# zhouzypaul/fql

Hardware: NVIDIA B200
Metric: fql_update_samples_per_sec (higher is better)
Workload: dtype bf16

## Files before the change

fql_b200/_lib.py:

```python
from __future__ import annotations

import ctypes as C
import os

_HERE = os.path.dirname(os.path.abspath(__file__))
LIB_PATH = os.path.join(_HERE, 'libfql_b200.so')

NUM_INFO = 13
NUM_RAW = 16
NET_NAMES = ('actor_bc_flow', 'actor_onestep_flow', 'critic', 'target_critic')
NET_ACTOR_BC_FLOW, NET_ACTOR_ONESTEP_FLOW, NET_CRITIC, NET_TARGET_CRITIC = 0, 1, 2, 3
LEAF_KINDS = ('kernel', 'bias', 'scale', 'bias', 'kernel', 'bias', 'kernel', 'bias')
PRECISION_FP32, PRECISION_BF16_TC, PRECISION_BF16_ENC = 0, 1, 2


class FqlDims(C.Structure):
    _fields_ = [(n, C.c_int32) for n in (
        'batch', 'global_batch', 'obs_dim', 'action_dim', 'hidden', 'num_hidden', 'critic_layer_norm', 'actor_layer_norm',
        'q_agg_min', 'normalize_q_loss', 'flow_steps', 'num_seeds', 'precision')] + [('reserved', C.c_int32 * 3)]


class FqlHparams(C.Structure):
    _fields_ = [(n, C.c_float) for n in ('lr', 'beta1', 'beta2', 'eps', 'discount', 'tau', 'alpha', 'one_minus_beta1',
                                         'one_minus_beta2', 'one_minus_tau')] + [('reserved', C.c_float * 2)]


class FqlLeaf(C.Structure):
    _fields_ = [('net', C.c_int32), ('layer', C.c_int32), ('kind', C.c_int32), ('ens', C.c_int32), ('rows', C.c_int32),
                ('cols', C.c_int32), ('offset', C.c_int64)]


class FqlBatch(C.Structure):
    _fields_ = [(n, C.c_void_p) for n in ('observations', 'actions', 'next_observations', 'rewards', 'masks', 'z_next', 'x0',
                                          't', 'z', 'z_metric')]


class FqlState(C.Structure):
    _fields_ = [(n, C.c_void_p) for n in ('params', 'mu', 'nu', 'grads', 'count', 'shadow')]


DP_MAX_RANKS = 8


class FqlDpComm(C.Structure):
    _fields_ = [('rank', C.c_int32), ('world', C.c_int32), ('base', C.c_void_p * DP_MAX_RANKS), ('base_mc', C.c_void_p)]


class FqlTestOperand(C.Structure):
    _fields_ = [('ptr', C.c_void_p), ('inner', C.c_int32), ('rows', C.c_int32), ('ld', C.c_int64), ('g0', C.c_int32), ('s0', C.c_int64),
                ('g1', C.c_int32), ('s1', C.c_int64)]


class FqlTestPtr(C.Structure):
    _fields_ = [('base', C.c_void_p), ('s0', C.c_int64), ('s1', C.c_int64), ('ld', C.c_int32)]


TEST_GEMM_PTRS = ('bias', 'out_f', 'out_h', 'out_z', 'zin', 'act', 'xb', 'target', 'ln_s', 'ln_b', 'dbias', 'wmaster', 'dln_s', 'dln_b')


class FqlTestGemm(C.Structure):
    _fields_ = ([(n, C.c_int32) for n in ('mode', 'M', 'N', 'K', 'G0', 'G1', 'a_mn', 'b_mn', 'ksplit')] +
                [('A', FqlTestOperand), ('B', FqlTestOperand)] + [(n, FqlTestPtr) for n in TEST_GEMM_PTRS] +
                [(n, C.c_int32) for n in ('F', 'Adim', 'step', 'n_steps', 'clip')])


TC_MODE_STORE_F32, TC_MODE_FWD_HIDDEN, TC_MODE_DGRAD_GELU, TC_MODE_EULER, TC_MODE_WGRAD_LN = 0, 1, 2, 3, 4


class FqlError(RuntimeError):
    pass


_lib = None

_SIGS = {
    'fql_version': (C.c_int, []),
    'fql_last_error': (C.c_char_p, []),
    'fql_info_name': (C.c_char_p, [C.c_int]),
    'fql_context_create': (C.c_int, [C.POINTER(C.c_void_p)]),
    'fql_context_destroy': (C.c_int, [C.c_void_p]),
    'fql_launch_count': (C.c_longlong, [C.c_void_p]),
    'fql_arena_floats': (C.c_int64, [C.POINTER(FqlDims)]),
    'fql_layout': (C.c_int, [C.POINTER(FqlDims), C.POINTER(FqlLeaf), C.c_int32, C.POINTER(C.c_int32)]),
    'fql_workspace_bytes': (C.c_size_t, [C.POINTER(FqlDims)]),
    'fql_shadow_bytes': (C.c_size_t, [C.POINTER(FqlDims)]),
    'fql_forward_workspace_bytes': (C.c_size_t, [C.POINTER(FqlDims), C.c_int32]),
    'fql_update_step': (C.c_int, [C.c_void_p, C.POINTER(FqlDims), C.POINTER(FqlHparams), C.POINTER(FqlBatch), C.POINTER(FqlState),
                                  C.c_void_p, C.c_void_p, C.c_size_t, C.c_void_p]),
    'fql_step_grads': (C.c_int, [C.c_void_p, C.POINTER(FqlDims), C.POINTER(FqlHparams), C.POINTER(FqlBatch), C.POINTER(FqlState),
                                 C.c_void_p, C.c_void_p, C.c_size_t, C.c_void_p]),
    'fql_step_apply': (C.c_int, [C.c_void_p, C.POINTER(FqlDims), C.POINTER(FqlHparams), C.POINTER(FqlState), C.c_void_p,
                                 C.c_void_p, C.c_void_p, C.c_size_t, C.c_void_p]),
    'fql_step_apply_gathered': (C.c_int, [C.c_void_p, C.POINTER(FqlDims), C.POINTER(FqlHparams), C.POINTER(FqlState), C.c_void_p, C.c_int32,
                                          C.c_void_p, C.c_void_p, C.c_size_t, C.c_void_p]),
    'fql_dp_symmetric_bytes': (C.c_size_t, [C.POINTER(FqlDims), C.c_int32]),
    'fql_dp_attach': (C.c_int, [C.c_void_p, C.POINTER(FqlDims), C.POINTER(FqlDpComm)]),
    'fql_dp_allreduce': (C.c_int, [C.c_void_p, C.c_int32, C.c_int64, C.c_int64, C.c_void_p]),
    'fql_conv3x3_workspace_bytes': (C.c_size_t, []),
    'fql_conv3x3_bf16': (C.c_int, [C.c_void_p, C.c_void_p, C.c_void_p, C.c_int32, C.c_int32, C.c_int32, C.c_int32, C.c_int32, C.c_int32,
                                   C.c_void_p, C.c_void_p, C.c_int32, C.c_void_p, C.c_void_p, C.c_size_t, C.c_void_p]),
    'fql_conv3x3_wgrad_bf16': (C.c_int, [C.c_void_p, C.c_void_p, C.c_int32, C.c_int32, C.c_int32, C.c_int32, C.c_int32, C.c_void_p,
                                         C.c_void_p, C.c_void_p, C.c_size_t, C.c_void_p]),
    'fql_test_tc_gemm': (C.c_int, [C.POINTER(FqlTestGemm), C.c_void_p]),
    'fql_test_act_ln_bf16': (C.c_int, [C.c_void_p, C.c_void_p, C.c_void_p, C.c_int64, C.c_int64, C.c_void_p, C.c_void_p, C.c_void_p,
                                       C.c_int32, C.c_int32, C.c_int32, C.c_int32, C.c_int32, C.c_void_p]),
    'fql_test_ln_bwd_bf16': (C.c_int, [C.c_void_p, C.c_void_p, C.c_void_p, C.c_int64, C.c_int64, C.c_void_p, C.c_void_p, C.c_int32,
                                       C.c_int32, C.c_int32, C.c_int32, C.c_int64, C.c_int64, C.c_void_p]),
    'fql_test_gelu_bwd_bf16': (C.c_int, [C.c_void_p, C.c_void_p, C.c_void_p, C.c_void_p, C.c_int32, C.c_int32, C.c_int32, C.c_int32,
                                         C.c_int64, C.c_int64, C.c_void_p]),
    'fql_test_colsum_bf16': (C.c_int, [C.c_void_p, C.c_int64, C.c_int64, C.c_int32, C.c_void_p, C.c_int64, C.c_int32, C.c_int64,
                                       C.c_void_p]),
    'fql_set_early_grads_event':(C.c_int, [C.c_void_p, C.c_void_p]),
    'fql_early_grads_floats': (C.c_int64, [C.POINTER(FqlDims)]),
    'fql_total_loss': (C.c_int, [C.c_void_p, C.POINTER(FqlDims), C.POINTER(FqlHparams), C.POINTER(FqlBatch), C.POINTER(FqlState),
                                 C.c_void_p, C.c_void_p, C.c_size_t, C.c_void_p]),
    'fql_sample_actions': (C.c_int, [C.c_void_p, C.POINTER(FqlDims), C.c_void_p, C.c_void_p, C.c_void_p, C.c_void_p, C.c_void_p,
                                     C.c_int32, C.c_void_p, C.c_size_t, C.c_void_p]),
    'fql_compute_flow_actions': (C.c_int, [C.c_void_p, C.POINTER(FqlDims), C.c_void_p, C.c_void_p, C.c_void_p, C.c_void_p,
                                           C.c_void_p, C.c_int32, C.c_void_p, C.c_size_t, C.c_void_p]),
    'fql_mlp_forward': (C.c_int, [C.c_void_p, C.POINTER(FqlDims), C.c_int32, C.c_void_p, C.c_void_p, C.c_void_p, C.c_int32,
                                  C.c_void_p, C.c_size_t, C.c_void_p]),
    'fql_target_update': (C.c_int, [C.POINTER(FqlDims), C.POINTER(FqlHparams), C.c_void_p, C.c_void_p, C.c_void_p]),
    'fql_debug_stamps': (C.c_int, [C.c_void_p, C.c_void_p, C.c_int]),
    'fql_refresh_shadow': (C.c_int, [C.POINTER(FqlDims), C.c_void_p, C.c_void_p, C.c_void_p]),
    'fql_gather_rows': (C.c_int, [C.c_void_p, C.c_void_p, C.c_void_p, C.c_int64, C.c_int64, C.c_void_p]),
    'fql_gather_frames': (C.c_int, [C.c_void_p, C.c_void_p, C.c_void_p, C.c_void_p, C.c_void_p, C.c_void_p, C.c_void_p, C.c_int64,
                                    C.c_int32, C.c_int32, C.c_int32, C.c_int32, C.c_int32, C.c_void_p]),
    'fql_fill_noise': (C.c_int, [C.POINTER(FqlDims), C.c_uint64, C.c_uint64, C.c_void_p, C.c_void_p, C.c_void_p, C.c_void_p,
                                 C.c_void_p, C.c_void_p]),
    'fql_fill_noise_rows': (C.c_int, [C.POINTER(FqlDims), C.c_uint64, C.c_uint64, C.c_int64, C.c_void_p, C.c_void_p, C.c_void_p,
                                      C.c_void_p, C.c_void_p, C.c_void_p]),
}
EXPORTS = tuple(_SIGS)


def lib():
    global _lib
    if _lib is None:
        if not os.path.exists(LIB_PATH):
            raise FqlError(f'{LIB_PATH} is missing: build it with `python -c "import __graft_entry__ as g; g.build()"` '
                           f'or `make -C fql_b200/csrc`. fql_b200 has no CPU or PyTorch fallback.')
        l = C.CDLL(LIB_PATH)
        for name, (res, args) in _SIGS.items():
            fn = getattr(l, name)
            fn.restype, fn.argtypes = res, args
        _lib = l
    return _lib


def check(rc, what=''):
    if rc != 0:
        raise FqlError(f'{what}: {lib().fql_last_error().decode()}')


def make_dims(batch, obs_dim, action_dim, *, global_batch=None, hidden=512, num_hidden=4, critic_layer_norm=True,
              actor_layer_norm=False, q_agg='mean', normalize_q_loss=False, flow_steps=10, num_seeds=1, precision=PRECISION_FP32,
              image=None):
    d = FqlDims()
    d.batch, d.global_batch = int(batch), int(global_batch if global_batch is not None else batch)
    d.obs_dim, d.action_dim, d.hidden, d.num_hidden = int(obs_dim), int(action_dim), int(hidden), int(num_hidden)
    d.critic_layer_norm, d.actor_layer_norm = int(bool(critic_layer_norm)), int(bool(actor_layer_norm))
    d.q_agg_min, d.normalize_q_loss = int(q_agg == 'min'), int(bool(normalize_q_loss))
    d.flow_steps, d.num_seeds, d.precision = int(flow_steps), int(num_seeds), int(precision)
    if image is not None:
        d.reserved[0], d.reserved[1], d.reserved[2] = int(image[0]), int(image[1]), int(image[2])
    return d


def make_hparams(lr=3e-4, discount=0.99, tau=0.005, alpha=300.0, beta1=0.9, beta2=0.999, eps=1e-8):
    h = FqlHparams()
    h.lr, h.beta1, h.beta2, h.eps, h.discount, h.tau, h.alpha = lr, beta1, beta2, eps, discount, tau, alpha
    h.one_minus_beta1, h.one_minus_beta2, h.one_minus_tau = 1.0 - beta1, 1.0 - beta2, 1.0 - tau
    return h


def layout(dims):
    l = lib()
    n = C.c_int32(0)
    check(l.fql_layout(C.byref(dims), None, 0, C.byref(n)), 'fql_layout')
    arr = (FqlLeaf * n.value)()
    check(l.fql_layout(C.byref(dims), arr, n.value, C.byref(n)), 'fql_layout')
    out = []
    for lf in arr:
        if lf.kind < 4:
            path = (('LayerNorm' if lf.kind >= 2 else 'Dense') + f'_{lf.layer}',)
        elif lf.kind < 6:
            path = ('encoder', f'stack_blocks_{lf.layer // 3}', f'Conv_{lf.layer % 3}')
        else:
            path = ('encoder', 'MLP_0', 'Dense_0')
        shape = None
        if lf.kind == 4:
            shape = (3, 3, lf.rows // 9, lf.cols)
        out.append(dict(net=NET_NAMES[lf.net], module=path[-1], path=path, name=LEAF_KINDS[lf.kind], ens=lf.ens, rows=lf.rows, cols=lf.cols,
                        offset=lf.offset, is_kernel=lf.kind in (0, 4, 6), shape=shape, kind=lf.kind))
    return out, int(l.fql_arena_floats(C.byref(dims)))
```

fql_b200/csrc/euler_cluster.cu:

```cuda
#include "step.cuh"
#include "tc_prims.cuh"

using namespace tc;

namespace {

constexpr int TILE_M = 128;
constexpr int KB = 64;
constexpr int A_BLK = TILE_M * 128;
constexpr int SUB = 32;
constexpr int A_SUB = TILE_M * SUB * 2;
constexpr int NSUB = 16;
constexpr int MAX_A = 32;
constexpr int NMMA = 4;
#ifndef FQL_EULER_NISS
#define FQL_EULER_NISS 2
#endif
constexpr int NISS = FQL_EULER_NISS;
static_assert(NISS == 1 || NISS == 2 || NISS == 4, "NISS");
constexpr int NEPI = 4;
constexpr int NTHREADS = 32 * (1 + NMMA + NEPI);
constexpr int EPI0 = 32 * (1 + NMMA);

struct EulerArgs {
  int H, K0, K0pad, A, F, n_steps, NL;
  int S, M, tiles;
  int x_rows_s;
  int x_row0;
  int w_row[FQL_MAXL];
  int w_rows_s;
  int wl_row, wl_rows_s;
  const float* params;
  long long arena;
  long long off_b[FQL_MAXL];
  const float* c0;
  const float* a0;
  float* target;
  __nv_bfloat16* hx;
  long long hx_buf_elems;
  float* state;
  __nv_bfloat16* Hsave[FQL_MAXL];
  __nv_bfloat16* Zsave[FQL_MAXL];
  float* out;
  int rows_cap, r0;
  float* Fsave[FQL_MAXL];
  int z_rows_cap, z_r0;
  unsigned long long* dbg;
  unsigned long long* t_start;
  int dbg_it;
};

struct HMaps {
  CUtensorMap m[4];
};
constexpr int MODE_EULER = 0, MODE_FWD = 1, MODE_DGRAD = 2;

__device__ __forceinline__ unsigned long long gtime() {
  unsigned long long t;
  asm volatile("mov.u64 %0, %globaltimer;" : "=l"(t));
  return t;
}

__device__ __forceinline__ float gelu_fast(float x) {
  const float u = FQL_GELU_C * (x + FQL_GELU_A * x * x * x);
  return 0.5f * x * (1.0f + tanh_approx(u));
}
__device__ __forceinline__ float gelu_grad_fast(float x) {
  const float x2 = x * x;
  const float u = FQL_GELU_C * (x + FQL_GELU_A * x2 * x);
  const float th = tanh_approx(u);
  const float du = FQL_GELU_C * (1.0f + 3.0f * FQL_GELU_A * x2);
  return 0.5f * (1.0f + th) + 0.5f * x * (1.0f - th * th) * du;
}
__device__ __forceinline__ uint32_t pack2(float a, float b) {
  __nv_bfloat162 v = __floats2bfloat162_rn(a, b);
  return *reinterpret_cast<uint32_t*>(&v);
}

template <int NC, int AMAX, int MODE>
__global__ void __launch_bounds__(NTHREADS, 1) euler_cluster_kernel(const __grid_constant__ CUtensorMap mapX,
                                                               const __grid_constant__ CUtensorMap mapW,
                                                               const __grid_constant__ CUtensorMap mapWL,
                                                               const __grid_constant__ HMaps mapsH, const EulerArgs a) {
  constexpr int NCOL = 512 / NC;
  constexpr int HALVES = NCOL / SUB;
  constexpr int B_ROWB = NCOL * 2;
  constexpr int B_BLK = KB * B_ROWB;
  constexpr int ACC_SET = NMMA * NCOL;
  constexpr uint16_t MASK = (uint16_t)((1u << NC) - 1u);
  extern __shared__ uint8_t smem_raw[];
  uint8_t* smem = reinterpret_cast<uint8_t*>((reinterpret_cast<uintptr_t>(smem_raw) + 1023) & ~(uintptr_t)1023);
  const int nkb = a.H / KB, nkb_x = a.K0pad / KB;
  uint8_t* sA = smem;
  uint8_t* sB = sA + NSUB * A_SUB;
  uint8_t* sX = sB + nkb * B_BLK;
  float* sBias = reinterpret_cast<float*>(sX + nkb_x * A_BLK);
  float* sT = sBias + a.NL * 64;
  uint64_t* bars = reinterpret_cast<uint64_t*>(sT + 64);
  uint64_t* full_a = bars;
  uint64_t* full_b = bars + 16;
  uint64_t* acc_full = bars + 17;
  uint64_t* free_a = bars + 18;
  uint64_t* a_ready = bars + 19;
  uint64_t* x_full = bars + 20;
  uint64_t* half_ready = bars + 21;
  uint32_t* tmem_slot = reinterpret_cast<uint32_t*>(bars + 24);

  const int warp = __shfl_sync(0xffffffffu, (int)(threadIdx.x >> 5), 0), lane = threadIdx.x & 31;
  const uint32_t j = __shfl_sync(0xffffffffu, cluster_ctarank(), 0);
  const int cl = blockIdx.x / NC;
  const int tile = cl % a.tiles, s = cl / a.tiles;
  const int NL = a.NL;
  const int total = a.n_steps * NL;
  const int hx_row = (s * a.tiles + tile) * TILE_M;
  unsigned long long* dbg = a.dbg ? a.dbg + blockIdx.x * 16 : nullptr;
  const int DBG_IT = a.dbg_it;

  if (warp == 0 && lane == 0) {
    tma_prefetch_desc(&mapX);
    tma_prefetch_desc(&mapW);
    tma_prefetch_desc(&mapWL);
    for (int i = 0; i < (MODE == MODE_EULER ? 1 : NL - 1); i++) tma_prefetch_desc(&mapsH.m[i]);
    for (int i = 0; i < NSUB; i++) mbar_init(&full_a[i], 1);
    mbar_init(&half_ready[0], NEPI);
    mbar_init(&half_ready[1], NEPI);
    mbar_init(full_b, 1);
    mbar_init(acc_full, NISS);
    mbar_init(free_a, NC * NISS);
    mbar_init(a_ready, NEPI);
    mbar_init(x_full, 1);
    fence_barrier_init();
  }
  if (warp == 1) tmem_alloc(tmem_slot, 2 * ACC_SET);
  for (int i = threadIdx.x; i < (MODE == MODE_DGRAD ? 0 : NL * 64); i += NTHREADS) {
    const int l = i >> 6, c = i & 63;
    const bool lastl = (l == NL - 1);
    const int N = lastl ? a.A : a.H;
    const int col = lastl ? c : (int)j * NCOL + c;
    sBias[i] = (c < NCOL && col < N && !(l == 0 && a.c0)) ? a.params[(int64_t)s * a.arena + a.off_b[l] + col] : 0.f;
  }
  if (threadIdx.x <= a.n_steps) sT[threadIdx.x] = (float)((double)threadIdx.x / (double)a.n_steps);
  tc_fence_before();
  __syncthreads();
  tc_fence_after();
  cluster_sync_all();
  const uint32_t tmem_base = *tmem_slot;
  if (a.t_start && blockIdx.x == 0 && threadIdx.x == 0) a.t_start[0] = gtime();

  if (warp == 0) {
    const bool el = elect_one();
    {
      if (el) mbar_expect_tx(x_full, nkb_x * A_BLK);
      const int xrow = s * a.x_rows_s + a.x_row0 + tile * TILE_M;
      for (int kb = 0; kb < nkb_x; kb++)
        if (el) tma_load_2d(sX + kb * A_BLK, &mapX, x_full, kb * KB, xrow);
      int n_pub = 0;
      int l = 0;
      for (int it = 0; it < total; it++, l = (l + 1 == NL) ? 0 : l + 1) {
        const bool last = (l == NL - 1);
        const int K = (l == 0) ? a.K0 : a.H;
        const int kblocks = (K + KB - 1) / KB;
        if (it > 0) mbar_wait_u(acc_full, (it - 1) & 1);
        if (el) mbar_expect_tx(full_b, kblocks * B_BLK);
        for (int kb = 0; kb < kblocks; kb++) {
          if (!el) continue;
          if constexpr (MODE == MODE_DGRAD) {
            if (l == 0) tma_load_2d(sB, &mapWL, full_b, 0, a.wl_row + s * a.wl_rows_s + (int)j * NCOL);
            else tma_load_2d(sB + kb * B_BLK, &mapW, full_b, kb * KB, a.w_row[l] + s * a.w_rows_s + (int)j * NCOL);
          } else {
            if (!last) tma_load_2d(sB + kb * B_BLK, &mapW, full_b, (int)j * NCOL, a.w_row[l] + s * a.w_rows_s + kb * KB);
            else tma_load_2d(sB + kb * B_BLK, &mapWL, full_b, 0, a.wl_row + s * a.wl_rows_s + kb * KB);
          }
        }
        if (l >= 1) {
          for (int sbk = 0; sbk < NSUB; sbk++)
            if (el) mbar_expect_tx(&full_a[sbk], A_SUB);
          const int buf = n_pub & 1;
          for (int h = 0; h < HALVES; h++) {
            mbar_wait_u(&half_ready[h], n_pub & 1);
            asm volatile("fence.proxy.async.global;" ::: "memory");
            if (h == 0) mbar_wait_cluster_u(free_a, (it - 1) & 1);
            if (dbg && el && it == DBG_IT) dbg[3 + h] = gtime();
            const int sbk = (int)j * HALVES + h;
            if (el)
              asm volatile(
                  "cp.async.bulk.tensor.2d.shared::cluster.global.mbarrier::complete_tx::bytes.multicast::cluster [%0], [%1, {%3, %4}], [%2], %5;"
                  ::"r"(smem_u32(sA + sbk * A_SUB)), "l"(reinterpret_cast<uint64_t>(MODE != MODE_EULER ? &mapsH.m[l - 1] : &mapsH.m[0])),
                  "r"(smem_u32(&full_a[sbk])), "r"(sbk * SUB),
                  "r"(MODE != MODE_EULER ? s * a.rows_cap + a.r0 + tile * TILE_M : buf * (a.S * a.tiles * TILE_M) + hx_row), "h"(MASK)
                  : "memory");
          }
          n_pub++;
        }
      }
    }
  } else if (warp <= NMMA) {
    const bool el = elect_one();
    if (warp <= NISS) {
      const int mw = warp - 1;
      const uint32_t tmem_u = __shfl_sync(0xffffffffu, tmem_base, 0);
      const uint32_t idesc = make_idesc_bf16(TILE_M, NCOL, false, MODE != MODE_DGRAD);
      const uint64_t ax_t = make_smem_desc(0, 16, 1024);
      const uint64_t a64_t0 = make_smem_desc_sw64(0, 16, 512);
      const uint64_t b_t0 = (MODE == MODE_DGRAD) ? make_smem_desc(0, 16, 1024)
                                                 : ((NC == 8) ? make_smem_desc(0, B_BLK, 1024) : make_smem_desc_sw64(0, B_BLK, 512));
      constexpr uint64_t B_KSTEP = (MODE == MODE_DGRAD) ? 2 : ((16 * B_ROWB) >> 4);
      constexpr uint64_t B_SUBH = (MODE == MODE_DGRAD) ? 4 : ((32 * B_ROWB) >> 4);
      const uint32_t sa0 = smem_u32(sA) >> 4, sx0 = smem_u32(sX) >> 4, sb0 = smem_u32(sB) >> 4;
      int n_a = 0;
      int n_step = 0;
      int l = 0;
      for (int it = 0; it < total; it++, l = (l + 1 == NL) ? 0 : l + 1) {
        const int K = (l == 0) ? a.K0 : a.H;
        const int kblocks = (K + KB - 1) / KB;
        const uint32_t tacc = tmem_u + (it & 1) * ACC_SET + mw * NCOL;
        if (l == 0) {
          if (it == 0) mbar_wait_u(x_full, 0);
          else { mbar_wait_u(a_ready, (n_step - 1) & 1); }
          n_step++;
          if (dbg && el && mw == 0 && it == DBG_IT) dbg[8] = gtime();
        }
        mbar_wait_u(full_b, it & 1);
        tc_fence_after();
        if (dbg && el && mw == 0 && it == DBG_IT && l == 0) dbg[9] = gtime();
        if (l >= 1) {
          constexpr int PER = NSUB / NISS;
          for (int i = 0; i < PER; i++) {
            const int sbk = (NC == 8) ? (mw * (PER / 2) + (i % (PER / 2))) * 2 + (i / (PER / 2)) : mw * PER + i;
            mbar_wait_u(&full_a[sbk], n_a & 1);
            tc_fence_after();
            if (dbg && el && mw == 0 && it == DBG_IT && i == 0) dbg[5] = gtime();
            if (dbg && el && mw == NISS - 1 && it == DBG_IT && i == PER - 1) dbg[6] = gtime();
            if (el)
              umma_bf16_x2(tacc, a64_t0 + (uint64_t)(sa0 + sbk * (A_SUB >> 4)),
                           b_t0 + (uint64_t)(sb0 + (sbk >> 1) * (B_BLK >> 4) + (sbk & 1) * B_SUBH), 2, B_KSTEP, idesc, i != 0);
          }
        } else {
          for (int kb = 0; kb < kblocks; kb++)
            for (int ks = mw; ks < 4; ks += NISS)
              if (el && ks < (a.K0 - kb * KB + 15) / 16)
                umma_bf16(tacc, ax_t + (uint64_t)(sx0 + kb * (A_BLK >> 4) + ks * 2), b_t0 + (uint64_t)(sb0 + kb * (B_BLK >> 4) + ks * B_KSTEP), idesc,
                          !(kb == 0 && ks == mw));
        }
        if (l >= 1) n_a++;
        if (dbg && el && mw == 0 && it == DBG_IT && l == 0) dbg[10] = gtime();
        if (el) {
          umma_commit(acc_full);
          asm volatile("tcgen05.commit.cta_group::1.mbarrier::arrive::one.shared::cluster.multicast::cluster.b64 [%0], %1;" ::"r"(smem_u32(free_a)),
                       "h"(MASK)
                       : "memory");
        }
      }
    }
  } else {
    const int q = warp & 3;
    const int row = q * 32 + lane;
    const int grow = tile * TILE_M + row;
    const bool valid = grow < a.M;
    const uint32_t t_lane0 = tmem_base + ((uint32_t)(q * 32) << 16);
    const int et = threadIdx.x - EPI0;
    float* st_row = a.state + (int64_t)blockIdx.x * MAX_A * TILE_M + row;
    int n_exch = 0;
    int l = 0, step = 0;
    for (int it = 0; it < total; it++, l = (l + 1 == NL) ? 0 : l + 1, step += (l == 0)) {
      const bool last = (l == NL - 1);
      const float* sb = sBias + l * 64;
      uint4 zq[4];
      if constexpr (MODE == MODE_DGRAD) {
        static_assert(MODE != MODE_DGRAD || HALVES == 1, "the dgrad chain is built for clusters of 16");
        if (valid) {
          const uint4* zp = reinterpret_cast<const uint4*>(a.Zsave[l] + ((int64_t)s * a.z_rows_cap + a.z_r0 + grow) * a.H + j * NCOL);
#pragma unroll
          for (int c = 0; c < 4; c++) zq[c] = __ldg(zp + c);
        }
      }
      float ac[AMAX];
      if (MODE == MODE_EULER && last) {
#pragma unroll
        for (int c = 0; c < AMAX; c++)
          if (c < a.A) ac[c] = (step == 0) ? (valid ? __ldg(a.a0 + ((int64_t)s * a.M + grow) * a.A + c) : 0.f) : __ldcg(st_row + c * TILE_M);
      }
      mbar_wait(acc_full, it & 1);
      tc_fence_after();
      if (dbg && et == 0 && it == DBG_IT - 1) dbg[0] = gtime();
      if (dbg && et == 0 && it == DBG_IT) dbg[7] = gtime();
      const int live = (l == 0 && (a.K0 + 15) / 16 < NISS) ? (a.K0 + 15) / 16 : NISS;
      const int buf = n_exch & 1;
      if (!last) n_exch++;
#pragma unroll 1
      for (int half = 0; half < HALVES; half++) {
        const uint32_t t_lane = t_lane0 + (it & 1) * ACC_SET + half * 32;
        uint32_t r0[32];
        if (!last || half == 0) {
          uint32_t t1[32];
          tmem_ld32(t_lane, r0);
          if (live > 1) tmem_ld32(t_lane + NCOL, t1);
          tmem_wait_ld();
          if (live > 1) {
#pragma unroll
            for (int i = 0; i < 32; i++) r0[i] = __float_as_uint(__uint_as_float(r0[i]) + __uint_as_float(t1[i]));
          }
          if (live > 2) {
            uint32_t t2[32];
            tmem_ld32(t_lane + 2 * NCOL, t1);
            if (live > 3) tmem_ld32(t_lane + 3 * NCOL, t2);
            tmem_wait_ld();
#pragma unroll
            for (int i = 0; i < 32; i++) {
              float v = __uint_as_float(r0[i]) + __uint_as_float(t1[i]);
              if (live > 3) v += __uint_as_float(t2[i]);
              r0[i] = __float_as_uint(v);
            }
          }
        }
        if constexpr (MODE == MODE_DGRAD) {
          if (valid) {
            const int64_t e0 = ((int64_t)s * a.rows_cap + a.r0 + grow) * a.H + j * NCOL;
            uint4* dh = reinterpret_cast<uint4*>(a.Hsave[l] + e0);
            float4* df = reinterpret_cast<float4*>(a.Fsave[l] + e0);
#pragma unroll
            for (int c = 0; c < 4; c++) {
              const uint32_t zw[4] = {zq[c].x, zq[c].y, zq[c].z, zq[c].w};
              float dv[8];
#pragma unroll
              for (int i = 0; i < 4; i++) {
                const __nv_bfloat162 zb = *reinterpret_cast<const __nv_bfloat162*>(&zw[i]);
                dv[2 * i] = __uint_as_float(r0[c * 8 + 2 * i]) * gelu_grad_fast(__low2float(zb));
                dv[2 * i + 1] = __uint_as_float(r0[c * 8 + 2 * i + 1]) * gelu_grad_fast(__high2float(zb));
              }
              dh[c] = make_uint4(pack2(dv[0], dv[1]), pack2(dv[2], dv[3]), pack2(dv[4], dv[5]), pack2(dv[6], dv[7]));
              df[2 * c] = make_float4(dv[0], dv[1], dv[2], dv[3]);
              df[2 * c + 1] = make_float4(dv[4], dv[5], dv[6], dv[7]);
            }
          }
          if (!last) {
            __syncwarp();
            if (lane == 0) mbar_arrive(&half_ready[half]);
          }
        } else if (!last) {
          if constexpr (MODE == MODE_EULER) {
            uint4* dst = reinterpret_cast<uint4*>(a.hx + (int64_t)buf * a.hx_buf_elems + (int64_t)(hx_row + row) * a.H + j * NCOL + half * 32);
            if (l == 0 && a.c0) {
              const float4* cp = reinterpret_cast<const float4*>(a.c0 + ((int64_t)s * a.M + (valid ? grow : 0)) * a.H + j * NCOL + half * 32);
#pragma unroll
              for (int c = 0; c < 8; c++) {
                const float4 cv = __ldg(cp + c);
                r0[c * 4 + 0] = __float_as_uint(__uint_as_float(r0[c * 4 + 0]) + cv.x);
                r0[c * 4 + 1] = __float_as_uint(__uint_as_float(r0[c * 4 + 1]) + cv.y);
                r0[c * 4 + 2] = __float_as_uint(__uint_as_float(r0[c * 4 + 2]) + cv.z);
                r0[c * 4 + 3] = __float_as_uint(__uint_as_float(r0[c * 4 + 3]) + cv.w);
              }
            }
#pragma unroll
            for (int c = 0; c < 4; c++) {
              float h[8];
#pragma unroll
              for (int i = 0; i < 8; i++) h[i] = gelu_fast(__uint_as_float(r0[c * 8 + i]) + sb[half * 32 + c * 8 + i]);
              dst[c] = make_uint4(pack2(h[0], h[1]), pack2(h[2], h[3]), pack2(h[4], h[5]), pack2(h[6], h[7]));
            }
          } else if (valid) {
            const int64_t e0 = ((int64_t)s * a.rows_cap + a.r0 + grow) * a.H + j * NCOL + half * 32;
            uint4* dh = reinterpret_cast<uint4*>(a.Hsave[l] + e0);
            uint4* dz = reinterpret_cast<uint4*>(a.Zsave[l] + e0);
#pragma unroll
            for (int c = 0; c < 4; c++) {
              float z[8], h[8];
#pragma unroll
              for (int i = 0; i < 8; i++) {
                z[i] = __uint_as_float(r0[c * 8 + i]) + sb[half * 32 + c * 8 + i];
                h[i] = gelu_fast(z[i]);
              }
              dh[c] = make_uint4(pack2(h[0], h[1]), pack2(h[2], h[3]), pack2(h[4], h[5]), pack2(h[6], h[7]));
              dz[c] = make_uint4(pack2(z[0], z[1]), pack2(z[2], z[3]), pack2(z[4], z[5]), pack2(z[6], z[7]));
            }
          }
          __syncwarp();
          if (lane == 0) mbar_arrive(&half_ready[half]);
          if (dbg && et == 0 && it == DBG_IT - 1) dbg[1 + half] = gtime();
        } else if (MODE == MODE_FWD) {
          if (half == 0 && j == 0 && valid) {
            float* o = a.out + ((int64_t)s * a.rows_cap + a.r0 + grow) * a.A;
#pragma unroll
            for (int c = 0; c < AMAX; c++)
              if (c < a.A) o[c] = __uint_as_float(r0[c]) + sb[c];
          }
        } else if (half == 0) {
          if (dbg && et == 0 && it == DBG_IT - 1) dbg[13] = gtime();
          const float inv = (float)a.n_steps;
          const bool final_step = (step == a.n_steps - 1);
#pragma unroll
          for (int c = 0; c < AMAX; c++)
            if (c < a.A) {
              ac[c] += (__uint_as_float(r0[c]) + sb[c]) / inv;
              const int col = a.F + c;
              *reinterpret_cast<__nv_bfloat16*>(sX + (col >> 6) * A_BLK + sw128_off(row, (col & 63) >> 3) + (col & 7) * 2) = __float2bfloat16(ac[c]);
            }
          {
            const int col = a.F + a.A;
            *reinterpret_cast<__nv_bfloat16*>(sX + (col >> 6) * A_BLK + sw128_off(row, (col & 63) >> 3) + (col & 7) * 2) =
                __float2bfloat16(sT[step + 1]);
          }
          if (dbg && et == 0 && it == DBG_IT - 1) dbg[11] = gtime();
          fence_proxy_async_smem();
          tc_fence_before();
          __syncwarp();
          if (lane == 0) mbar_arrive(a_ready);
          if (dbg && et == 0 && it == DBG_IT - 1) dbg[12] = gtime();
#pragma unroll
          for (int c = 0; c < AMAX; c++)
            if (c < a.A) {
              if (!final_step) __stcg(st_row + c * TILE_M, ac[c]);
              else if (valid && j == 0) a.target[((int64_t)s * a.M + grow) * a.A + c] = fminf(fmaxf(ac[c], -1.0f), 1.0f);
            }
        }
      }
      if (!last) tc_fence_before();
    }
  }
  tc_fence_before();
  __syncthreads();
  cluster_sync_all();
  if (a.t_start && blockIdx.x == 0 && threadIdx.x == 0) a.t_start[1] = gtime();
  if (warp == 1) tmem_dealloc(tmem_base, 2 * ACC_SET);
}

}

size_t tc_euler_scratch_elems(const FqlDims* d, int M) {
  const int tiles = (M + TILE_M - 1) / TILE_M;
  return (size_t)2 * d->num_seeds * tiles * TILE_M * d->hidden + (size_t)2 * d->num_seeds * tiles * 16 * MAX_A * TILE_M;
}

namespace {
template <int NC, int AMAX, int MODE>
int launch_euler(const EulerArgs& a, const TcEulerSpec& f, cudaStream_t st, bool query_only, int* max_clusters) {
  constexpr int NCOL = 512 / NC;
  const FqlDims* d = f.d;
  const int smem = NSUB * A_SUB + (a.H / KB) * (KB * NCOL * 2) + (a.K0pad / KB) * A_BLK + a.NL * 64 * 4 + 64 * 4 + 256 + 1024;
  FQL_REQUIRE(smem <= 232448, "euler_cluster_kernel: shared memory %d > 227 KB", smem);
  auto kern = euler_cluster_kernel<NC, AMAX, MODE>;
  static bool attr_set[FQL_MAX_DEVICES] = {};
  const int dev = fql_current_device();
  if (!attr_set[dev]) {
    FQL_CHECK_CUDA(cudaFuncSetAttribute(kern, cudaFuncAttributeMaxDynamicSharedMemorySize, 232448));
    if (NC > 8) FQL_CHECK_CUDA(cudaFuncSetAttribute(kern, cudaFuncAttributeNonPortableClusterSizeAllowed, 1));
    attr_set[dev] = true;
  }
  cudaLaunchConfig_t cfg;
  memset(&cfg, 0, sizeof(cfg));
  cfg.gridDim = dim3(NC * a.tiles * a.S);
  cfg.blockDim = dim3(NTHREADS);
  cfg.dynamicSmemBytes = smem;
  cfg.stream = st;
  cudaLaunchAttribute attr[1];
  attr[0].id = cudaLaunchAttributeClusterDimension;
  attr[0].val.clusterDim.x = NC;
  attr[0].val.clusterDim.y = 1;
  attr[0].val.clusterDim.z = 1;
  cfg.attrs = attr;
  cfg.numAttrs = 1;
  if (query_only) {
    cfg.stream = nullptr;
    if (cudaOccupancyMaxActiveClusters(max_clusters, kern, &cfg) != cudaSuccess) {
      cudaGetLastError();
      *max_clusters = 0;
    }
    return 0;
  }
  const CUtensorMapSwizzle wsw = (NC == 8 || MODE == MODE_DGRAD) ? CU_TENSOR_MAP_SWIZZLE_128B : CU_TENSOR_MAP_SWIZZLE_64B;
  CUtensorMap mapX, mapW, mapWL;
  HMaps mapsH;
  memset(&mapsH, 0, sizeof(mapsH));
  FQL_TRY(make_map_2d(&mapX, f.X0b, a.K0pad, (uint64_t)a.S * f.Mcap0, 64, TILE_M));
  if (MODE == MODE_DGRAD) {
    FQL_TRY(make_map_2d(&mapW, f.shadow, d->hidden, (uint64_t)a.S * a.w_rows_s, 64, NCOL, wsw));
    FQL_TRY(make_map_2d(&mapWL, f.shadow, 64, (uint64_t)a.S * a.wl_rows_s, 64, NCOL, wsw));
  } else {
    FQL_TRY(make_map_2d(&mapW, f.shadow, d->hidden, (uint64_t)a.S * a.w_rows_s, NCOL, KB, wsw));
    FQL_TRY(make_map_2d(&mapWL, f.shadow, 64, (uint64_t)a.S * a.wl_rows_s, NCOL, KB, wsw));
  }
  if (MODE == MODE_EULER) {
    FQL_TRY(make_map_2d(&mapsH.m[0], f.scratch, d->hidden, (uint64_t)2 * a.S * a.tiles * TILE_M, SUB, TILE_M, CU_TENSOR_MAP_SWIZZLE_64B));
  } else {
    for (int l = 0; l + 1 < a.NL; l++)
      FQL_TRY(make_map_2d(&mapsH.m[l], a.Hsave[l], d->hidden, (uint64_t)a.S * a.rows_cap, SUB, TILE_M, CU_TENSOR_MAP_SWIZZLE_64B));
  }
  FQL_CHECK_CUDA(cudaLaunchKernelEx(&cfg, kern, mapX, mapW, mapWL, mapsH, a));
  FQL_CHECK_LAUNCH();
  return 0;
}
}

namespace {
int fill_args(EulerArgs& a, const FqlDims* d, const Layout& L, int net, const float* params, int M, int Mcap0, int r0_in, bool hoisted = false) {
  FQL_TRY(tc_supported(d, !hoisted));
  FQL_REQUIRE(d->hidden == 512, "euler_cluster_kernel is built for hidden = 512 (16 exchange units of 32 columns)");
  const NetView& nv = L.net[net];
  memset(&a, 0, sizeof(a));
  a.H = d->hidden; a.K0 = nv.in_dim; a.K0pad = (int)round_up64(nv.in_dim, 64); a.A = nv.out_dim; a.F = d->obs_dim;
  a.n_steps = 1; a.NL = nv.n_layers;
  a.S = d->num_seeds; a.M = M; a.tiles = (M + TILE_M - 1) / TILE_M;
  a.x_rows_s = Mcap0; a.x_row0 = r0_in;
  const int64_t seed_elems = tc_shadow_seed_elems(d, L);
  a.w_rows_s = (int)(seed_elems / d->hidden);
  a.wl_rows_s = (int)(seed_elems / 64);
  for (int l = 0; l < nv.n_layers; l++) {
    a.w_row[l] = (int)(nv.off_w[l] / d->hidden);
    a.off_b[l] = nv.off_b[l];
  }
  int64_t wl = L.arena;
  for (int t = 0; t < net; t++) wl += (int64_t)L.net[t].ens * d->hidden * 64;
  a.wl_row = (int)(wl / 64);
  a.params = params; a.arena = L.arena;
  FQL_REQUIRE(a.A <= MAX_A, "euler_cluster_kernel: output width %d > %d", a.A, MAX_A);
  a.dbg_it = 7;
  return 0;
}
int max_clusters16(const EulerArgs& a, const TcEulerSpec& f) {
  static int max16_dev[FQL_MAX_DEVICES];
  static bool known[FQL_MAX_DEVICES] = {};
  const int dev = fql_current_device();
  int& max16 = max16_dev[dev];
  if (!known[dev]) {
    const char* e = getenv("FQL_B200_EULER_NC");
    if (e && atoi(e) == 8) max16 = 0;
    else if (launch_euler<16, 8, MODE_EULER>(a, f, nullptr, true, &max16)) max16 = 0;
    if (getenv("FQL_B200_VERBOSE")) fprintf(stderr, "fql_b200: clusters of 16 CTAs resident at once (device %d): %d\n", dev, max16);
    known[dev] = true;
  }
  return max16;
}
}

int tc_euler_cluster(const TcEulerSpec& f, cudaStream_t st) {
  const FqlDims* d = f.d;
  EulerArgs a;
  FQL_TRY(fill_args(a, d, *f.L, FQL_NET_ACTOR_BC_FLOW, f.params, f.M, f.Mcap0, f.r0_in, f.c0 != nullptr));
  a.A = d->action_dim; a.n_steps = d->flow_steps;
  if (f.c0) {
    a.c0 = f.c0;
    a.K0 = d->action_dim + 1; a.K0pad = 64; a.F = 0;
    a.w_row[0] += d->obs_dim;
  }
  a.a0 = f.a0; a.target = f.target;
  a.hx = reinterpret_cast<__nv_bfloat16*>(f.scratch);
  a.hx_buf_elems = (long long)a.S * a.tiles * TILE_M * a.H;
  a.state = reinterpret_cast<float*>(a.hx + 2 * a.hx_buf_elems);
  a.dbg = reinterpret_cast<unsigned long long*>(f.dbg);
  a.t_start = reinterpret_cast<unsigned long long*>(f.t_start);
  FQL_REQUIRE(f.scratch != nullptr && f.a0 && f.target, "tc_euler_cluster: NULL argument");
  FQL_REQUIRE(a.n_steps < 64, "euler_cluster_kernel: flow_steps %d >= 64", a.n_steps);
  const bool c16 = a.tiles * a.S <= max_clusters16(a, f);
  if (a.A <= 8) return c16 ? launch_euler<16, 8, MODE_EULER>(a, f, st, false, nullptr) : launch_euler<8, 8, MODE_EULER>(a, f, st, false, nullptr);
  if (a.A <= 16) return c16 ? launch_euler<16, 16, MODE_EULER>(a, f, st, false, nullptr) : launch_euler<8, 16, MODE_EULER>(a, f, st, false, nullptr);
  return c16 ? launch_euler<16, 32, MODE_EULER>(a, f, st, false, nullptr) : launch_euler<8, 32, MODE_EULER>(a, f, st, false, nullptr);
}

int tc_cluster_forward(const TcClusterFwdSpec& f, int other_clusters, cudaStream_t st) {
  const FqlDims* d = f.d;
  const NetView& nv = f.L->net[f.net];
  if (d->hidden != 512 || nv.ln || nv.n_layers > 5 || nv.n_layers < 2 || nv.out_dim > MAX_A || nv.in_dim > 128) return 1;
  EulerArgs a;
  if (fill_args(a, d, *f.L, f.net, f.params, f.M, f.rows_cap, f.r0)) return -1;
  TcEulerSpec e;
  memset(&e, 0, sizeof(e));
  e.d = d; e.L = f.L; e.params = f.params; e.shadow = f.shadow; e.X0b = f.X0b; e.Mcap0 = f.rows_cap; e.r0_in = f.r0; e.M = f.M;
  if (a.tiles * a.S + other_clusters > max_clusters16(a, e)) return 1;
  for (int l = 0; l + 1 < nv.n_layers; l++) {
    a.Hsave[l] = reinterpret_cast<__nv_bfloat16*>(f.Hb[l]);
    a.Zsave[l] = reinterpret_cast<__nv_bfloat16*>(f.Zb[l]);
    if (!a.Hsave[l] || !a.Zsave[l]) return 1;
  }
  a.out = f.out; a.rows_cap = f.rows_cap; a.r0 = f.r0;
  a.t_start = reinterpret_cast<unsigned long long*>(f.t_start);
  if (a.A <= 8) return launch_euler<16, 8, MODE_FWD>(a, e, st, false, nullptr) ? -1 : 0;
  if (a.A <= 16) return launch_euler<16, 16, MODE_FWD>(a, e, st, false, nullptr) ? -1 : 0;
  return launch_euler<16, 32, MODE_FWD>(a, e, st, false, nullptr) ? -1 : 0;
}

int tc_cluster_dgrad(const TcClusterBwdSpec& f, int other_clusters, cudaStream_t st) {
  const FqlDims* d = f.d;
  const NetView& nv = f.L->net[f.net];
  if (d->hidden != 512 || nv.ln || nv.n_layers > 5 || nv.n_layers < 3 || nv.out_dim > 64) return 1;
  EulerArgs a;
  if (fill_args(a, d, *f.L, f.net, nullptr, f.M, f.M, 0)) return -1;
  const int NLn = nv.n_layers;
  a.NL = NLn - 1;
  a.K0 = 64; a.K0pad = 64;
  for (int it = 1; it < a.NL; it++) a.w_row[it] = (int)(nv.off_w[NLn - 1 - it] / d->hidden);
  TcEulerSpec e;
  memset(&e, 0, sizeof(e));
  e.d = d; e.L = f.L; e.shadow = f.shadow; e.X0b = f.dOutb; e.Mcap0 = f.M; e.r0_in = 0; e.M = f.M;
  if (a.tiles * a.S + other_clusters > max_clusters16(a, e)) return 1;
  for (int it = 0; it < a.NL; it++) {
    const int lo = NLn - 2 - it;
    a.Hsave[it] = reinterpret_cast<__nv_bfloat16*>(f.dZb[lo]);
    a.Fsave[it] = f.dZf[lo];
    a.Zsave[it] = reinterpret_cast<__nv_bfloat16*>(f.Zb[lo]);
    if (!a.Hsave[it] || !a.Fsave[it] || !a.Zsave[it]) return 1;
  }
  a.rows_cap = f.M; a.r0 = 0; a.z_rows_cap = f.z_rows_cap; a.z_r0 = f.z_r0;
  a.t_start = reinterpret_cast<unsigned long long*>(f.t_start);
  return launch_euler<16, 8, MODE_DGRAD>(a, e, st, false, nullptr) ? -1 : 0;
}
```

fql_b200/csrc/step.cu:

```cuda
#include "step.cuh"
#include "dp_comm.cuh"

#include <cuda_bf16.h>
#include <stdarg.h>

#include <vector>

static thread_local char g_err[1024] = "";
thread_local long long g_fql_launches = 0;
void fql_set_error(const char* fmt, ...) {
  va_list ap;
  va_start(ap, fmt);
  vsnprintf(g_err, sizeof(g_err), fmt, ap);
  va_end(ap);
}

int fql_validate_dims(const FqlDims* d) {
  FQL_REQUIRE(d != nullptr, "dims is NULL");
  FQL_REQUIRE(d->batch >= 1 && d->global_batch >= d->batch, "batch=%d global_batch=%d", d->batch, d->global_batch);
  FQL_REQUIRE(d->obs_dim >= 1 && d->action_dim >= 1, "obs_dim=%d action_dim=%d", d->obs_dim, d->action_dim);
  FQL_REQUIRE(d->hidden >= 1 && d->num_hidden >= 1 && d->num_hidden + 1 <= FQL_MAXL, "hidden=%d num_hidden=%d", d->hidden, d->num_hidden);
  FQL_REQUIRE(d->num_seeds >= 1, "num_seeds=%d", d->num_seeds);
  FQL_REQUIRE(d->flow_steps >= 1, "flow_steps=%d", d->flow_steps);
  FQL_REQUIRE(d->precision == FQL_PRECISION_FP32 || d->precision == FQL_PRECISION_BF16_TC || d->precision == FQL_PRECISION_BF16_ENC,
              "precision=%d", d->precision);
  FQL_REQUIRE(d->precision != FQL_PRECISION_BF16_ENC || d->reserved[0] > 0, "FQL_PRECISION_BF16_ENC is a pixel-config mode (encoder='impala_small')");
  if (d->reserved[0] > 0) {
    FQL_REQUIRE(d->reserved[1] > 0 && d->reserved[2] > 0 && d->reserved[2] <= 32, "image dims %dx%dx%d", d->reserved[0], d->reserved[1], d->reserved[2]);
    FQL_REQUIRE(d->obs_dim == 512, "pixel configs: obs_dim is the encoder output width and must be 512 (got %d)", d->obs_dim);
    FQL_REQUIRE(d->num_seeds == 1, "pixel configs are built for num_seeds == 1");
  }
  return 0;
}

int fql_build_layout(const FqlDims* d, Layout* L) {
  FQL_TRY(fql_validate_dims(d));
  memset(L, 0, sizeof(*L));
  const int F = d->obs_dim, A = d->action_dim, H = d->hidden, NL = d->num_hidden + 1;
  int64_t off = 0;
  int nl = 0;
  auto add_leaf = [&](int net, int64_t n) {
    int64_t o = off;
    L->leaf_blk[nl] = (int)(off / FQL_LEAF_PAD);
    L->leaf_net[nl] = net;
    nl++;
    off += round_up64(n, FQL_LEAF_PAD);
    return o;
  };
  static const int kOrder[FQL_NUM_NETS] = {FQL_NET_ACTOR_BC_FLOW, FQL_NET_CRITIC, FQL_NET_ACTOR_ONESTEP_FLOW, FQL_NET_TARGET_CRITIC};
  for (int oi = 0; oi < FQL_NUM_NETS; oi++) {
    const int n = kOrder[oi];
    NetView& v = L->net[n];
    v.n_layers = NL;
    v.hidden = H;
    const bool critic = (n == FQL_NET_CRITIC || n == FQL_NET_TARGET_CRITIC);
    v.ens = critic ? 2 : 1;
    v.ln = critic ? d->critic_layer_norm : d->actor_layer_norm;
    v.in_dim = (n == FQL_NET_ACTOR_BC_FLOW) ? F + A + 1 : F + A;
    v.out_dim = critic ? 1 : A;
    v.begin = off;
    const int extra = v.ln ? 4 : 2;
    FQL_REQUIRE(nl + NL * extra + 20 <= FQL_MAX_LEAVES, "too many leaves");
    for (int l = 0; l < NL; l++) {
      const int64_t K = v.k_of(l), N = v.n_of(l);
      v.off_w[l] = add_leaf(n, v.ens * K * N);
      v.off_b[l] = add_leaf(n, v.ens * N);
      if (v.ln && l + 1 < NL) {
        v.off_lns[l] = add_leaf(n, v.ens * N);
        v.off_lnb[l] = add_leaf(n, v.ens * N);
      }
    }
    if (d->reserved[0] > 0) {
      v.has_enc = 1;
      static const int stacks[3] = {16, 32, 32};
      int c = d->reserved[2], h = d->reserved[0], w = d->reserved[1];
      for (int i = 0; i < 3; i++) {
        const int f = stacks[i];
        const int cin[3] = {c, f, f};
        for (int j = 0; j < 3; j++) {
          v.enc.off_cw[i][j] = add_leaf(n, 9 * cin[j] * f);
          v.enc.off_cb[i][j] = add_leaf(n, f);
        }
        c = f; h = (h + 1) / 2; w = (w + 1) / 2;
      }
      v.enc.off_dw = add_leaf(n, (int64_t)h * w * c * d->obs_dim);
      v.enc.off_db = add_leaf(n, d->obs_dim);
    }
    v.end = off;
  }
  L->arena = off;
  L->n_leaves = nl;
  L->leaf_blk[nl] = (int)(off / FQL_LEAF_PAD);
  return 0;
}

StepShape make_shape(const FqlDims* d) {
  StepShape s;
  s.S = d->num_seeds; s.B = d->batch; s.GB = d->global_batch; s.F = d->obs_dim; s.A = d->action_dim;
  s.H = d->hidden; s.NH = d->num_hidden;
  s.q_agg_min = d->q_agg_min; s.normalize_q_loss = d->normalize_q_loss; s.flow_steps = d->flow_steps;
  return s;
}

namespace {
struct Carver {
  char* base;
  size_t off = 0;
  float* take(int64_t nfloats) {
    off = (off + 255) & ~(size_t)255;
    float* p = base ? reinterpret_cast<float*>(base + off) : nullptr;
    off += (size_t)nfloats * sizeof(float);
    return p;
  }
};

void carve_pass(Carver& c, PassBuf* pb, int G, int Mcap, int H, int NH, int out_dim, bool ln, bool need_z) {
  pb->G = G;
  pb->Mcap = Mcap;
  for (int l = 0; l < NH; l++) {
    pb->Z[l] = (need_z || ln) ? c.take((int64_t)G * Mcap * H) : nullptr;
    pb->Hh[l] = c.take((int64_t)G * Mcap * H);
    pb->mu[l] = ln ? c.take((int64_t)G * Mcap) : nullptr;
    pb->rstd[l] = ln ? c.take((int64_t)G * Mcap) : nullptr;
  }
  pb->out = c.take((int64_t)G * Mcap * out_dim);
}
}

size_t carve_workspace(const FqlDims* d, const Layout& L, void* base, WsPtrs* w) {
  Carver c{reinterpret_cast<char*>(base)};
  const int64_t S = d->num_seeds, B = d->batch, F = d->obs_dim, A = d->action_dim, H = d->hidden;
  const int NH = d->num_hidden;
  memset(w, 0, sizeof(*w));
  w->XO = c.take(S * 3 * B * (F + A));
  w->XF = c.take(S * 2 * B * (F + A + 1));
  w->XC = c.take(3 * S * B * (F + A));
  w->vel = c.take(S * B * A);
  carve_pass(c, &w->pO, (int)S, (int)(3 * B), (int)H, NH, (int)A, d->actor_layer_norm, true);
  carve_pass(c, &w->pF, (int)S, (int)(2 * B), (int)H, NH, (int)A, d->actor_layer_norm, true);
  carve_pass(c, &w->pC, (int)(3 * S * 2), (int)B, (int)H, NH, 1, d->critic_layer_norm, true);
  w->O_out = w->pO.out;
  w->F_out = w->pF.out;
  w->C_out = w->pC.out;
  w->dq = c.take(S * 2 * B);
  w->dqs = c.take(S * 2 * B);
  w->dpred = c.take(S * B * A);
  w->dapi = c.take(S * B * A);
  w->target = c.take(S * B * A);
  w->dX0 = c.take(S * 2 * B * (F + A));
  w->raw_local = c.take(S * FQL_NUM_RAW);
  w->gstats = c.take(S * 4 + 4);
  w->partials = c.take(S * (int64_t)L.leaf_blk[L.n_leaves] * 4);
  w->cpost_part = c.take(2 * S * 64 * 4);
  w->cpost_ticket = reinterpret_cast<int*>(c.take(3 * S + 4));
  if (d->reserved[0] > 0) {
    for (int i = 0; i < 5; i++) w->feat[i] = c.take(S * B * F);
    for (int i = 0; i < 3; i++) w->dfeat[i] = c.take(S * B * F);
    w->dX0F = c.take(S * B * (F + A + 1));
    w->dX0O = c.take(S * B * (F + A));
    w->dX0C = c.take(S * 2 * B * (F + A));
    const bool bwd[5] = {false, true, false, true, true};
    for (int i = 0; i < 5; i++) {
      c.off = (c.off + 255) & ~(size_t)255;
      c.off += enc_carve(d, B, base ? c.base + c.off : nullptr, &w->enc[i], bwd[i]);
    }
  }
  if (d->precision == FQL_PRECISION_BF16_TC) {
    const int64_t kO = round_up64(F + A, 64), kF = round_up64(F + A + 1, 64);
    w->XOb = c.take((S * 3 * B * kO + 1) / 2);
    w->XFb = c.take((S * 2 * B * kF + 1) / 2);
    w->XCb = c.take((3 * S * B * kO + 1) / 2);
    for (int l = 0; l < NH; l++) {
      w->O_Hb[l] = c.take(S * 3 * B * H / 2);
      w->O_Zb[l] = c.take(S * 3 * B * H / 2);
      w->F_Hb[l] = c.take(S * 2 * B * H / 2);
      w->F_Zb[l] = c.take(S * 2 * B * H / 2);
      w->C_Hb[l] = c.take(3 * S * 2 * B * H / 2);
      w->C_XHb[l] = c.take(3 * S * 2 * B * H / 2);
      w->C_DGb[l] = c.take(3 * S * 2 * B * H / 2);
    }
    for (int i = 0; i < NH; i++) {
      w->O_dZb[i] = c.take(S * B * H / 2);
      w->F_dZb[i] = c.take(S * B * H / 2);
      w->O_dZf[i] = c.take(S * B * H);
      w->F_dZf[i] = c.take(S * B * H);
    }
    w->O_dOutb = c.take(S * B * 64 / 2);
    w->F_dOutb = c.take(S * B * 64 / 2);
    for (int i = 0; i < NH; i++) {
      w->C1_dZb[i] = c.take(S * 2 * B * H / 2);
      w->C2_dZb[i] = c.take(S * 2 * B * H / 2);
      w->C1_dZf[i] = c.take(S * 2 * B * H);
      w->C1_dHf[i] = c.take(S * 2 * B * H);
      w->C2_dZf[i] = c.take(S * 2 * B * H);
      w->C2_dHf[i] = c.take(S * 2 * B * H);
    }
    w->C1_dOutb = c.take(S * 2 * B * 64 / 2);
    w->C2_dOutb = c.take(S * 2 * B * 64 / 2);
    w->euler_a = c.take(S * B * A);
    for (int i = 0; i < 3; i++) w->cs_scratch[i] = c.take(65536);
    w->euler_hx = c.take((int64_t)(tc_euler_scratch_elems(d, (int)B) / 2 + 4));
  }
  for (int i = 0; i < 2; i++) {
    w->dC[i] = c.take(S * 2 * B * H);
    w->dCp[i] = c.take(S * 2 * B * H);
    w->dF[i] = c.take(S * B * H);
    w->dO[i] = c.take(S * B * H);
  }
  return c.off + 256;
}

namespace {

struct FwdSpec {
  int P;
  const NetView* nv[FQL_MAXP];
  const float* params;
  int64_t arena;
  int S, E, M, H;
  const float* X0;
  int Mcap0, r0_in;
  PassBuf* buf;
  int r0;
  int save_z;
};

int mlp_forward(const FwdSpec& f, cudaStream_t st) {
  const NetView& n0 = *f.nv[0];
  const int NL = n0.n_layers;
  const int64_t Mcap = f.buf->Mcap;
  for (int l = 0; l < NL; l++) {
    const int K = n0.k_of(l), N = n0.n_of(l);
    const bool last = (l == NL - 1);
    GemmArgs a;
    memset(&a, 0, sizeof(a));
    a.P = f.P; a.S = f.S; a.E = f.E; a.M = f.M; a.N = N; a.K = K;
    for (int p = 0; p < f.P; p++) {
      if (l == 0) a.A.base[p] = f.X0 + ((int64_t)p * f.S * f.Mcap0 + f.r0_in) * K;
      else a.A.base[p] = f.buf->Hh[l - 1] + ((int64_t)p * f.S * f.E * Mcap + f.r0) * f.H;
      a.B.base[p] = f.params + f.nv[p]->off_w[l];
      a.bias.base[p] = f.params + f.nv[p]->off_b[l];
    }
    if (l == 0) { a.A.stride_s = (int64_t)f.Mcap0 * K; a.A.stride_e = 0; a.lda = K; }
    else { a.A.stride_s = (int64_t)f.E * Mcap * f.H; a.A.stride_e = Mcap * f.H; a.lda = f.H; }
    a.B.stride_s = f.arena; a.B.stride_e = (int64_t)K * N; a.ldb = N;
    a.bias.stride_s = f.arena; a.bias.stride_e = N;
    a.out.stride_s = (int64_t)f.E * Mcap * N; a.out.stride_e = Mcap * N; a.ldo = N;
    a.out_pre.stride_s = a.out.stride_s; a.out_pre.stride_e = a.out.stride_e; a.ld_pre = N;
    for (int p = 0; p < f.P; p++) {
      const int64_t goff = ((int64_t)p * f.S * f.E * Mcap + f.r0) * N;
      if (last) a.out.base[p] = f.buf->out + goff;
      else if (n0.ln) a.out.base[p] = f.buf->Z[l] + goff;
      else {
        a.out.base[p] = f.buf->Hh[l] + goff;
        a.out_pre.base[p] = f.save_z ? f.buf->Z[l] + goff : nullptr;
      }
    }
    a.act_gelu = (!last && !n0.ln) ? 1 : 0;
    FQL_TRY(launch_gemm(a, st));
    if (!last && n0.ln) {
      ActLnArgs r;
      memset(&r, 0, sizeof(r));
      r.P = f.P; r.S = f.S; r.E = f.E; r.M = f.M; r.N = N; r.ld = N; r.ln = 1;
      for (int p = 0; p < f.P; p++) {
        const int64_t goff = ((int64_t)p * f.S * f.E * Mcap + f.r0);
        r.Z.base[p] = f.buf->Z[l] + goff * N;
        r.H.base[p] = f.buf->Hh[l] + goff * N;
        r.mu.base[p] = f.buf->mu[l] + goff;
        r.rstd.base[p] = f.buf->rstd[l] + goff;
        r.scale.base[p] = f.params + f.nv[p]->off_lns[l];
        r.lnbias.base[p] = f.params + f.nv[p]->off_lnb[l];
      }
      r.Z.stride_s = (int64_t)f.E * Mcap * N; r.Z.stride_e = Mcap * N;
      r.H.stride_s = r.Z.stride_s; r.H.stride_e = r.Z.stride_e;
      r.mu.stride_s = (int64_t)f.E * Mcap; r.mu.stride_e = Mcap;
      r.rstd.stride_s = r.mu.stride_s; r.rstd.stride_e = r.mu.stride_e;
      r.scale.stride_s = f.arena; r.scale.stride_e = N;
      r.lnbias.stride_s = f.arena; r.lnbias.stride_e = N;
      FQL_TRY(launch_act_ln_fwd(r, st));
    }
  }
  return 0;
}

struct BwdSpec {
  const NetView* nv;
  const float* params;
  float* grads;
  int64_t arena;
  int S, E, M, H;
  const float* X0;
  int Mcap0;
  const PassBuf* buf;
  int p, r0;
  const float* dOut;
  float* dpp[2];
  float* dX0;
};

int mlp_backward(const BwdSpec& b, cudaStream_t st) {
  const NetView& n = *b.nv;
  const int NL = n.n_layers;
  const int64_t Mcap = b.buf->Mcap;
  const int64_t goff_rows = ((int64_t)b.p * b.S * b.E * Mcap + b.r0);
  const float* dZ = b.dOut;
  int ldz = n.out_dim;
  int cur = 0;
  for (int l = NL - 1; l >= 0; l--) {
    const int K = n.k_of(l), N = n.n_of(l);
    const int64_t dz_ss = (int64_t)b.E * b.M * ldz, dz_se = (int64_t)b.M * ldz;
    if (b.grads) {
      GemmArgs a;
      memset(&a, 0, sizeof(a));
      a.P = 1; a.S = b.S; a.E = b.E; a.M = K; a.N = N; a.K = b.M;
      a.trans_a = 1;
      if (l == 0) { a.A.base[0] = b.X0; a.A.stride_s = (int64_t)b.Mcap0 * K; a.A.stride_e = 0; a.lda = K; }
      else { a.A.base[0] = b.buf->Hh[l - 1] + goff_rows * b.H; a.A.stride_s = (int64_t)b.E * Mcap * b.H; a.A.stride_e = Mcap * b.H; a.lda = b.H; }
      a.B.base[0] = dZ; a.B.stride_s = dz_ss; a.B.stride_e = dz_se; a.ldb = ldz;
      a.out.base[0] = b.grads + n.off_w[l]; a.out.stride_s = b.arena; a.out.stride_e = (int64_t)K * N; a.ldo = N;
      FQL_TRY(launch_gemm(a, st));
      ColSumArgs c;
      memset(&c, 0, sizeof(c));
      c.P = 1; c.S = b.S; c.E = b.E; c.M = b.M; c.N = N; c.ld = ldz;
      c.X.base[0] = dZ; c.X.stride_s = dz_ss; c.X.stride_e = dz_se;
      c.out.base[0] = b.grads + n.off_b[l]; c.out.stride_s = b.arena; c.out.stride_e = N;
      FQL_TRY(launch_colsum(c, st));
    }
    if (l == 0 && !b.dX0) break;
    GemmArgs a;
    memset(&a, 0, sizeof(a));
    a.P = 1; a.S = b.S; a.E = b.E; a.M = b.M; a.N = K; a.K = N;
    a.A.base[0] = dZ; a.A.stride_s = dz_ss; a.A.stride_e = dz_se; a.lda = ldz;
    a.trans_b = 1;
    a.B.base[0] = b.params + n.off_w[l]; a.B.stride_s = b.arena; a.B.stride_e = (int64_t)K * N; a.ldb = N;
    if (l == 0) {
      a.out.base[0] = b.dX0; a.out.stride_s = (int64_t)b.E * b.M * K; a.out.stride_e = (int64_t)b.M * K; a.ldo = K;
      FQL_TRY(launch_gemm(a, st));
      break;
    }
    float* dst = b.dpp[cur];
    a.out.base[0] = dst; a.out.stride_s = (int64_t)b.E * b.M * b.H; a.out.stride_e = (int64_t)b.M * b.H; a.ldo = b.H;
    const float* Zprev = b.buf->Z[l - 1] + goff_rows * b.H;
    const int64_t z_ss = (int64_t)b.E * Mcap * b.H, z_se = Mcap * b.H;
    if (!n.ln) {
      a.mulz.base[0] = Zprev; a.mulz.stride_s = z_ss; a.mulz.stride_e = z_se; a.ld_mulz = b.H;
      FQL_TRY(launch_gemm(a, st));
    } else {
      FQL_TRY(launch_gemm(a, st));
      if (b.grads) {
        ColSumArgs c;
        memset(&c, 0, sizeof(c));
        c.P = 1; c.S = b.S; c.E = b.E; c.M = b.M; c.N = b.H; c.ld = b.H;
        c.X.base[0] = dst; c.X.stride_s = a.out.stride_s; c.X.stride_e = a.out.stride_e;
        c.out.base[0] = b.grads + n.off_lnb[l - 1]; c.out.stride_s = b.arena; c.out.stride_e = b.H;
        FQL_TRY(launch_colsum(c, st));
        c.Z.base[0] = Zprev; c.Z.stride_s = z_ss; c.Z.stride_e = z_se;
        c.mu.base[0] = b.buf->mu[l - 1] + goff_rows; c.mu.stride_s = (int64_t)b.E * Mcap; c.mu.stride_e = Mcap;
        c.rstd.base[0] = b.buf->rstd[l - 1] + goff_rows; c.rstd.stride_s = c.mu.stride_s; c.rstd.stride_e = c.mu.stride_e;
        c.out.base[0] = b.grads + n.off_lns[l - 1];
        FQL_TRY(launch_colsum(c, st));
      }
      ActLnBwdArgs r;
      memset(&r, 0, sizeof(r));
      r.P = 1; r.S = b.S; r.E = b.E; r.M = b.M; r.N = b.H; r.ld = b.H;
      r.dH.base[0] = dst; r.dH.stride_s = a.out.stride_s; r.dH.stride_e = a.out.stride_e;
      r.dZ.base[0] = dst; r.dZ.stride_s = a.out.stride_s; r.dZ.stride_e = a.out.stride_e;
      r.Z.base[0] = Zprev; r.Z.stride_s = z_ss; r.Z.stride_e = z_se;
      r.scale.base[0] = b.params + n.off_lns[l - 1]; r.scale.stride_s = b.arena; r.scale.stride_e = b.H;
      FQL_TRY(launch_act_ln_bwd(r, st));
    }
    dZ = dst;
    ldz = b.H;
    cur ^= 1;
  }
  return 0;
}

}

struct GraphEntry {
  std::vector<unsigned char> key;
  cudaGraphExec_t exec;
  long long kernels;
};
struct FqlContext {
  cudaStream_t sc = nullptr;
  DpState dp;
  cudaStream_t s0 = nullptr, s1 = nullptr, s2 = nullptr, s3 = nullptr, s4 = nullptr, s5 = nullptr, s6 = nullptr, s7 = nullptr, s8 = nullptr, s9 = nullptr;
  cudaEvent_t ev[64] = {};
  std::vector<GraphEntry> graphs;
  int use_graph = 1;
  int use_euler_cluster = 1;
  int use_cluster_fwd = 1;
  int use_cluster_bwd = 1;
  unsigned long long* stamps = nullptr;
  int adam_done_blk = 0;
  int euler_hoist = 1;
  int enc_streams = 1;
  int dp_early_adam = 1;
  int dp_bc_late = 0;
  int use_big_bwd = 1;
  int chain_min_tiles = 48;
  cudaEvent_t early_event = nullptr;
  long long launches = 0;
};

extern "C" long long fql_launch_count(FqlContext* c) { return c ? c->launches : -1; }
extern "C" int fql_set_early_grads_event(FqlContext* c, void* event) {
  FQL_REQUIRE(c != nullptr, "context is NULL");
  c->early_event = reinterpret_cast<cudaEvent_t>(event);
  for (auto& g : c->graphs) if (g.exec) cudaGraphExecDestroy(g.exec);
  c->graphs.clear();
  return 0;
}
extern "C" int64_t fql_early_grads_floats(const FqlDims* d) {
  Layout L;
  if (fql_build_layout(d, &L)) return -1;
  return L.net[FQL_NET_ACTOR_ONESTEP_FLOW].begin;
}
extern "C" int fql_dp_allreduce(FqlContext* c, int32_t bucket, int64_t off, int64_t n, void* stream) {
  FQL_REQUIRE(c && c->dp.active, "fql_dp_allreduce: no communicator attached (fql_dp_attach)");
  const long long before = g_fql_launches;
  const int rc = dp_allreduce_range(c->dp, bucket, off, n, reinterpret_cast<cudaStream_t>(stream));
  c->launches += g_fql_launches - before;
  return rc;
}
extern "C" int fql_dp_attach(FqlContext* c, const FqlDims* d, const FqlDpComm* comm) {
  FQL_REQUIRE(c != nullptr, "context is NULL");
  for (auto& g : c->graphs) if (g.exec) cudaGraphExecDestroy(g.exec);
  c->graphs.clear();
  c->dp = DpState();
  if (!comm) return 0;
  Layout L;
  FQL_TRY(fql_build_layout(d, &L));
  FQL_REQUIRE(comm->world >= 2 && comm->world <= FQL_DP_MAX_RANKS && comm->rank >= 0 && comm->rank < comm->world, "fql_dp_attach: rank %d of %d",
              comm->rank, comm->world);
  for (int r = 0; r < comm->world; r++) FQL_REQUIRE(comm->base[r] != nullptr && ((uintptr_t)comm->base[r] & 15) == 0, "fql_dp_attach: base[%d] is NULL / unaligned", r);
  c->dp.comm = *comm;
  c->dp.S = d->num_seeds;
  c->dp.arena = L.arena;
  c->dp.lay = dp_layout(d->num_seeds, L.arena);
  c->dp.active = 1;
  return 0;
}

__global__ void stamp_kernel(unsigned long long* slot) {
  unsigned long long t;
  asm volatile("mov.u64 %0, %%globaltimer;" : "=l"(t));
  *slot = t;
}
static int stamp(FqlContext* ctx, int idx, cudaStream_t st) {
  if (!ctx->stamps) return 0;
  stamp_kernel<<<1, 1, 0, st>>>(ctx->stamps + idx);
  FQL_CHECK_LAUNCH();
  return 0;
}
extern "C" int fql_debug_stamps(FqlContext* c, unsigned long long* host_out, int n) {
  FQL_REQUIRE(c && c->stamps && n <= 576, "stamps are off (FQL_B200_STAMPS=1)");
  FQL_CHECK_CUDA(cudaMemcpy(host_out, c->stamps, n * sizeof(unsigned long long), cudaMemcpyDeviceToHost));
  return 0;
}
static int record_early(FqlContext* ctx, cudaStream_t st) {
  if (!ctx->early_event) return 0;
  cudaStreamCaptureStatus cap = cudaStreamCaptureStatusNone;
  FQL_CHECK_CUDA(cudaStreamIsCapturing(st, &cap));
  FQL_CHECK_CUDA(cudaEventRecordWithFlags(ctx->early_event, st, cap == cudaStreamCaptureStatusActive ? cudaEventRecordExternal : cudaEventRecordDefault));
  return 0;
}

extern "C" int fql_context_create(FqlContext** out) {
  FQL_REQUIRE(out != nullptr, "out is NULL");
  FqlContext* c = new FqlContext();
  int prio_lo = 0, prio_hi = 0;
  FQL_CHECK_CUDA(cudaDeviceGetStreamPriorityRange(&prio_lo, &prio_hi));
  const char* pr = getenv("FQL_B200_PRIO");
  if (pr && pr[0] == '0') prio_hi = prio_lo;
  FQL_CHECK_CUDA(cudaStreamCreateWithPriority(&c->s0, cudaStreamNonBlocking, prio_hi));
  FQL_CHECK_CUDA(cudaStreamCreateWithPriority(&c->s1, cudaStreamNonBlocking, prio_hi));
  FQL_CHECK_CUDA(cudaStreamCreateWithPriority(&c->s2, cudaStreamNonBlocking, prio_lo));
  FQL_CHECK_CUDA(cudaStreamCreateWithPriority(&c->s3, cudaStreamNonBlocking, prio_lo));
  FQL_CHECK_CUDA(cudaStreamCreateWithPriority(&c->s4, cudaStreamNonBlocking, prio_lo));
  FQL_CHECK_CUDA(cudaStreamCreateWithPriority(&c->s5, cudaStreamNonBlocking, prio_lo));
  FQL_CHECK_CUDA(cudaStreamCreateWithPriority(&c->s6, cudaStreamNonBlocking, prio_lo));
  FQL_CHECK_CUDA(cudaStreamCreateWithPriority(&c->s7, cudaStreamNonBlocking, prio_lo));
  FQL_CHECK_CUDA(cudaStreamCreateWithPriority(&c->s8, cudaStreamNonBlocking, prio_lo));
  FQL_CHECK_CUDA(cudaStreamCreateWithPriority(&c->s9, cudaStreamNonBlocking, prio_lo));
  FQL_CHECK_CUDA(cudaStreamCreateWithPriority(&c->sc, cudaStreamNonBlocking, prio_hi));
  for (auto& e : c->ev) FQL_CHECK_CUDA(cudaEventCreateWithFlags(&e, cudaEventDisableTiming));
  const char* g = getenv("FQL_B200_GRAPH");
  if (g && g[0] == '0') c->use_graph = 0;
  const char* ec = getenv("FQL_B200_EULER_CLUSTER");
  if (ec && ec[0] == '0') c->use_euler_cluster = 0;
  const char* cbw = getenv("FQL_B200_CLUSTER_BWD");
  if (cbw && cbw[0] == '0') c->use_cluster_bwd = 0;
  const char* cfw = getenv("FQL_B200_CLUSTER_FWD");
  if (cfw && cfw[0] == '0') c->use_cluster_fwd = 0;
  const char* stp = getenv("FQL_B200_STAMPS");
  if (stp && stp[0] == '1') {
    FQL_CHECK_CUDA(cudaMalloc(&c->stamps, 576 * sizeof(unsigned long long)));
    FQL_CHECK_CUDA(cudaMemset(c->stamps, 0, 576 * sizeof(unsigned long long)));
  }
  const char* ehs = getenv("FQL_B200_EULER_HOIST");
  if (ehs) c->euler_hoist = atoi(ehs);
  const char* ens = getenv("FQL_B200_ENC_STREAMS");
  if (ens) c->enc_streams = atoi(ens);
  const char* dea = getenv("FQL_B200_DP_EARLY_ADAM");
  if (dea) c->dp_early_adam = atoi(dea);
  const char* dbl = getenv("FQL_B200_DP_BC_LATE");
  if (dbl) c->dp_bc_late = atoi(dbl);
  const char* cm = getenv("FQL_B200_CHAIN_MIN_TILES");
  if (cm) c->chain_min_tiles = atoi(cm);
  const char* bb = getenv("FQL_B200_BIG_BWD");
  if (bb && bb[0] == '0') c->use_big_bwd = 0;
  *out = c;
  return 0;
}

extern "C" int fql_context_destroy(FqlContext* c) {
  if (!c) return 0;
  for (auto& g : c->graphs) if (g.exec) cudaGraphExecDestroy(g.exec);
  for (auto& e : c->ev) if (e) cudaEventDestroy(e);
  if (c->s0) cudaStreamDestroy(c->s0);
  if (c->s1) cudaStreamDestroy(c->s1);
  if (c->s2) cudaStreamDestroy(c->s2);
  if (c->s3) cudaStreamDestroy(c->s3);
  if (c->s4) cudaStreamDestroy(c->s4);
  if (c->s5) cudaStreamDestroy(c->s5);
  if (c->s6) cudaStreamDestroy(c->s6);
  if (c->s7) cudaStreamDestroy(c->s7);
  if (c->s8) cudaStreamDestroy(c->s8);
  if (c->s9) cudaStreamDestroy(c->s9);
  if (c->sc) cudaStreamDestroy(c->sc);
  if (c->stamps) cudaFree(c->stamps);
  delete c;
  return 0;
}

namespace {

struct StepCall {
  const FqlDims* d;
  const FqlHparams* hp;
  const FqlBatch* b;
  const FqlState* st;
  float* raw;
  float* info;
  void* ws;
  size_t ws_bytes;
  int do_grads, do_backward, do_apply;
  int raw_ranks;
};

int check_common(const FqlDims* d, const void* ws, size_t ws_bytes, Layout* L, WsPtrs* w) {
  FQL_TRY(fql_build_layout(d, L));
  const size_t need = carve_workspace(d, *L, nullptr, w);
  FQL_REQUIRE(ws != nullptr && ws_bytes >= need, "workspace too small: have %zu need %zu", ws_bytes, need);
  FQL_REQUIRE(((uintptr_t)ws & 255) == 0, "workspace must be 256-byte aligned");
  carve_workspace(d, *L, const_cast<void*>(ws), w);
  return 0;
}

int encode_observations(const StepCall& c, const Layout& L, WsPtrs& w, cudaStream_t st, FqlContext* ctx = nullptr) {
  const FqlBatch& b = *c.b;
  if (c.d->reserved[0] == 0) {
    w.src[0] = w.src[2] = b.next_observations;
    w.src[1] = w.src[3] = w.src[4] = b.observations;
    return 0;
  }
  const uint8_t* obs = reinterpret_cast<const uint8_t*>(b.observations);
  const uint8_t* nobs = reinterpret_cast<const uint8_t*>(b.next_observations);
  const float* P = c.st->params;
  const int64_t B = c.d->batch;
  cudaStream_t sa = st, sb = st;
  const bool fork = ctx && c.d->precision != FQL_PRECISION_FP32 && ctx->enc_streams;
  if (fork) {
    sa = ctx->s5; sb = ctx->s6;
    FQL_CHECK_CUDA(cudaEventRecord(ctx->ev[60], st));
    FQL_CHECK_CUDA(cudaStreamWaitEvent(sa, ctx->ev[60], 0));
    FQL_CHECK_CUDA(cudaStreamWaitEvent(sb, ctx->ev[60], 0));
  }
  FQL_TRY(enc_forward(c.d, L.net[FQL_NET_ACTOR_ONESTEP_FLOW].enc, P, nobs, B, w.enc[0], w.feat[0], st));
  FQL_TRY(enc_forward(c.d, L.net[FQL_NET_TARGET_CRITIC].enc, P, nobs, B, w.enc[2], w.feat[2], sa));
  FQL_TRY(enc_forward(c.d, L.net[FQL_NET_ACTOR_BC_FLOW].enc, P, obs, B, w.enc[4], w.feat[4], sb));
  FQL_TRY(enc_forward(c.d, L.net[FQL_NET_ACTOR_ONESTEP_FLOW].enc, P, obs, B, w.enc[1], w.feat[1], st));
  FQL_TRY(enc_forward(c.d, L.net[FQL_NET_CRITIC].enc, P, obs, B, w.enc[3], w.feat[3], sa));
  if (fork) {
    FQL_CHECK_CUDA(cudaEventRecord(ctx->ev[61], sa));
    FQL_CHECK_CUDA(cudaEventRecord(ctx->ev[62], sb));
    FQL_CHECK_CUDA(cudaStreamWaitEvent(st, ctx->ev[61], 0));
    FQL_CHECK_CUDA(cudaStreamWaitEvent(st, ctx->ev[62], 0));
  }
  for (int i = 0; i < 5; i++) w.src[i] = w.feat[i];
  return 0;
}

int encoder_grads(const StepCall& c, const Layout& L, const WsPtrs& w, int net, const float* dX0, int E, int K0, float* dfeat, int enc_idx,
                  cudaStream_t st) {
  const int64_t B = c.d->batch;
  FQL_TRY(launch_extract_feat_grad(dX0, dfeat, E, B, K0, c.d->obs_dim, st));
  return enc_backward(c.d, L.net[net].enc, c.st->params, c.st->grads, reinterpret_cast<const uint8_t*>(c.b->observations), B, w.enc[enc_idx],
                      dfeat, st);
}

int enqueue_grads_tc(FqlContext* ctx, const StepCall& c, const Layout& L, WsPtrs& w, const StepShape& sh, const FqlHparams& hp,
                     float* raw, cudaStream_t S0) {
  const FqlBatch& b = *c.b;
  const FqlDims* d = c.d;
  const int S = sh.S, B = sh.B, H = sh.H, NH = sh.NH;
  const float* P = c.st->params;
  const void* shadow = c.st->shadow;
  typedef __nv_bfloat16 bf16;
  cudaStream_t S1 = ctx->s1, S2 = ctx->s2;
  cudaEvent_t ev_prep = ctx->ev[0], ev_f0 = ctx->ev[1], ev_cpost = ctx->ev[2], ev_euler = ctx->ev[3], ev_s2 = ctx->ev[4], ev_pad = ctx->ev[5];
  const int kO = (int)round_up64(sh.F + sh.A, 64), kF = (int)round_up64(sh.F + sh.A + 1, 64);
  const bool dp_grads = ctx->dp.active && c.do_backward;
  const bool wide = tc_wide_input(d), pix = d->reserved[0] > 0;
  const bool dp_bucketed = dp_grads && !pix;
  bool bc_enc_forked = false;
  FQL_TRY(stamp(ctx, 0, S0));
  FQL_TRY(launch_zero_bc(raw, (int64_t)S * FQL_NUM_RAW, c.do_apply ? c.st->count : nullptr, hp, w.gstats + S * 4, S0, w.cpost_ticket, 3 * S));
  FQL_TRY(encode_observations(c, L, w, S0, ctx));
  FQL_TRY(launch_prep(sh, b, w, S0));
  FQL_TRY(stamp(ctx, 1, S0));
  FQL_CHECK_CUDA(cudaEventRecord(ev_prep, S0));
  FQL_CHECK_CUDA(cudaStreamWaitEvent(S1, ev_prep, 0));

  auto actor = [&](int net, const void* X0b, int K0pad, int rows_cap, int r0, int M, void* const* Hb, void* const* Zb, bool with_z) {
    TcActor t;
    memset(&t, 0, sizeof(t));
    t.d = d; t.L = &L; t.net = net; t.params = P; t.shadow = shadow; t.grads = c.st->grads; t.M = M;
    t.X0b = reinterpret_cast<const bf16*>(X0b) + (int64_t)r0 * K0pad; t.K0pad = K0pad; t.x_ss = (long long)rows_cap * K0pad;
    for (int l = 0; l < NH; l++) {
      t.Hb[l] = reinterpret_cast<bf16*>(Hb[l]) + (int64_t)r0 * H;
      t.Zb[l] = with_z ? reinterpret_cast<bf16*>(Zb[l]) + (int64_t)r0 * H : nullptr;
    }
    t.h_ss = (long long)rows_cap * H;
    t.cs_scratch = (net == FQL_NET_ACTOR_BC_FLOW) ? w.cs_scratch[0] : w.cs_scratch[1];
    return t;
  };

  FQL_TRY(tc_pad_bf16(w.XF, w.XFb, (int64_t)S * 2 * B, sh.F + sh.A + 1, kF, S1));
  FQL_CHECK_CUDA(cudaEventRecord(ev_pad, S1));
  const int row_tiles = S * ((B + 127) / 128);
  const bool many_tiles = row_tiles >= ctx->chain_min_tiles && !wide;
  const bool big_bwd = many_tiles && ctx->use_big_bwd && tc_mlp_chain2_supported(d) && d->critic_layer_norm && d->reserved[0] == 0;
  auto chain = [&](int net, const void* X0b, int rows_cap, int r0_in, int M, void* const* Hb, void* const* Zb, float* out, int n_steps,
                   cudaStream_t st) {
    TcChainSpec t;
    memset(&t, 0, sizeof(t));
    t.d = d; t.L = &L; t.P = 1; t.net[0] = net; t.params = P; t.shadow = shadow; t.M = M; t.X0b = X0b; t.Mcap0 = rows_cap; t.r0_in = r0_in;
    t.r0 = r0_in; t.Hb = Hb; t.Zb = Zb; t.Mcap_override = rows_cap; t.out_override = out; t.n_steps = n_steps;
    if (big_bwd && Zb) { t.DGb = Zb; t.Zb = nullptr; }
    if (n_steps > 1) { t.a0 = b.z; t.target = w.target; }
    return tc_mlp_chain(t, st);
  };
  if (many_tiles) {
    FQL_TRY(chain(FQL_NET_ACTOR_BC_FLOW, w.XFb, 2 * B, B, B, nullptr, nullptr, nullptr, sh.flow_steps, S1));
  } else if (H == 512 && ctx->use_euler_cluster && wide && S == 1 && ctx->euler_hoist) {
    const NetView& nb = L.net[FQL_NET_ACTOR_BC_FLOW];
    const bf16* sh16 = reinterpret_cast<const bf16*>(shadow);
    float* c0 = w.dF[0];
    TcGemmSpec g;
    memset(&g, 0, sizeof(g));
    g.M = B; g.N = H; g.K = sh.F; g.G0 = 1; g.G1 = 1; g.a_mn = 0; g.b_mn = 1;
    g.A.ptr = reinterpret_cast<const bf16*>(w.XFb) + (int64_t)B * kF; g.A.inner = sh.F; g.A.rows = B; g.A.ld = kF; g.A.g0 = 1; g.A.g1 = 1;
    g.B.ptr = sh16 + nb.off_w[0]; g.B.inner = H; g.B.rows = sh.F; g.B.ld = H; g.B.g0 = 1; g.B.g1 = 1;
    g.mode = TC_MODE_STORE_F32;
    g.bias.base = const_cast<float*>(P + nb.off_b[0]);
    g.out_f.base = c0; g.out_f.ld = H;
    FQL_TRY(tc_gemm(g, S1));
    float* xa = w.dF[1];
    void* xab = w.dO[0];
    FQL_TRY(launch_concat(b.z, sh.A, b.z, 0, 0.f, 1, xa, B, S1));
    FQL_TRY(tc_pad_bf16(xa, xab, B, sh.A + 1, 64, S1));
    TcEulerSpec e;
    memset(&e, 0, sizeof(e));
    e.d = d; e.L = &L; e.params = P; e.shadow = shadow; e.X0b = xab; e.Mcap0 = B; e.r0_in = 0; e.M = B;
    e.a0 = b.z; e.c0 = c0; e.target = w.target; e.scratch = w.euler_hx;
    FQL_TRY(tc_euler_cluster(e, S1));
  } else if (H == 512 && ctx->use_euler_cluster && !wide) {
    TcEulerSpec e;
    memset(&e, 0, sizeof(e));
    e.d = d; e.L = &L; e.params = P; e.shadow = shadow; e.X0b = w.XFb; e.Mcap0 = 2 * B; e.r0_in = B; e.M = B;
    e.a0 = b.z; e.target = w.target; e.scratch = w.euler_hx;
    e.t_start = ctx->stamps ? ctx->stamps + 13 : nullptr;
    e.dbg = (ctx->stamps && S * ((B + 127) / 128) <= 2) ? ctx->stamps + 64 : nullptr;
    FQL_TRY(tc_euler_cluster(e, S1));
  } else {
    TcActor e = actor(FQL_NET_ACTOR_BC_FLOW, w.XFb, kF, 2 * B, B, B, w.F_Hb, w.F_Zb, false);
    for (int i = 0; i < sh.flow_steps; i++) {
      TcEuler eu{w.euler_a, w.target, i, sh.flow_steps};
      FQL_TRY(tc_actor_forward(e, nullptr, 0, 0, &eu, S1));
    }
  }
  FQL_TRY(stamp(ctx, 2, S1));
  FQL_CHECK_CUDA(cudaEventRecord(ev_euler, S1));
  if (getenv("FQL_B200_EULER_ALONE")) {
    const int m = atoi(getenv("FQL_B200_EULER_ALONE"));
    if (m & 1) FQL_CHECK_CUDA(cudaStreamWaitEvent(S0, ev_euler, 0));
    if (m & 2) FQL_CHECK_CUDA(cudaStreamWaitEvent(S2, ev_euler, 0));
  }

  FQL_CHECK_CUDA(cudaStreamWaitEvent(S2, ev_pad, 0));
  TcActor fbc = actor(FQL_NET_ACTOR_BC_FLOW, w.XFb, kF, 2 * B, 0, B, w.F_Hb, w.F_Zb, true);
  if (many_tiles) FQL_TRY(chain(FQL_NET_ACTOR_BC_FLOW, w.XFb, 2 * B, 0, B, w.F_Hb, w.F_Zb, w.F_out, 1, S2));
  else FQL_TRY(tc_actor_forward(fbc, w.F_out, (long long)2 * B * sh.A, 0, nullptr, S2));
  FQL_TRY(launch_bc_post(sh, w, raw, S2));
  if (c.do_backward && big_bwd) {
    FQL_TRY(tc_actor_backward_big(fbc, w.dpred, w.F_dOutb, w.F_dZb, false, S2));
    FQL_CHECK_CUDA(cudaEventRecord(ctx->ev[16], S2));
    if (dp_bucketed && !ctx->dp_bc_late) {
      const NetView& nb = L.net[FQL_NET_ACTOR_BC_FLOW];
      FQL_CHECK_CUDA(cudaStreamWaitEvent(ctx->sc, ctx->ev[16], 0));
      FQL_TRY(dp_reduce_bucket(ctx->dp, 0, nb.begin, nb.end - nb.begin, nullptr, ctx->sc));
    }
    FQL_TRY(stamp(ctx, 4, S2));
  } else if (c.do_backward) {
    FQL_TRY(tc_actor_backward(fbc, w.dpred, w.F_dOutb, w.F_dZb, w.F_dZf, S2, ctx->s3, ctx->s7, &ctx->ev[8]));
    if (pix) {
      FQL_TRY(tc_actor_input_grad(fbc, w.F_dZb[0], w.dX0F, S2));
      FQL_CHECK_CUDA(cudaEventRecord(ctx->ev[63], S2));
      FQL_CHECK_CUDA(cudaStreamWaitEvent(ctx->sc, ctx->ev[63], 0));
      FQL_TRY(encoder_grads(c, L, w, FQL_NET_ACTOR_BC_FLOW, w.dX0F, 1, sh.F + sh.A + 1, w.dfeat[1], 4, ctx->sc));
      FQL_CHECK_CUDA(cudaEventRecord(ctx->ev[37], ctx->sc));
      bc_enc_forked = true;
    }
    FQL_CHECK_CUDA(cudaEventRecord(ctx->ev[53], ctx->s7));
    FQL_CHECK_CUDA(cudaStreamWaitEvent(ctx->s3, ctx->ev[53], 0));
    FQL_CHECK_CUDA(cudaEventRecord(ctx->ev[16], ctx->s3));
    if (dp_bucketed && !ctx->dp_bc_late) {
      const NetView& nb = L.net[FQL_NET_ACTOR_BC_FLOW];
      FQL_CHECK_CUDA(cudaStreamWaitEvent(ctx->sc, ctx->ev[16], 0));
      FQL_TRY(stamp(ctx, 20, ctx->sc));
      FQL_TRY(dp_reduce_bucket(ctx->dp, 0, nb.begin, nb.end - nb.begin, nullptr, ctx->sc));
      FQL_TRY(stamp(ctx, 21, ctx->sc));
    }
    FQL_TRY(stamp(ctx, 4, S2));
  }
  (void)ev_f0;

  FQL_TRY(tc_pad_bf16(w.XO, w.XOb, (int64_t)S * 3 * B, sh.F + sh.A, kO, S0));
  TcActor fo = actor(FQL_NET_ACTOR_ONESTEP_FLOW, w.XOb, kO, 3 * B, 0, 3 * B, w.O_Hb, w.O_Zb, true);
  bool split_metric = false;
  if (many_tiles) {
    FQL_TRY(chain(FQL_NET_ACTOR_ONESTEP_FLOW, w.XOb, 3 * B, 0, 3 * B, w.O_Hb, w.O_Zb, w.O_out, 1, S0));
  } else {
    int rc = 1;
    if (ctx->use_euler_cluster && ctx->use_cluster_fwd && !wide) {
      TcClusterFwdSpec cf;
      memset(&cf, 0, sizeof(cf));
      cf.d = d; cf.L = &L; cf.params = P; cf.shadow = shadow; cf.net = FQL_NET_ACTOR_ONESTEP_FLOW; cf.X0b = w.XOb; cf.rows_cap = 3 * B; cf.r0 = 0;
      cf.M = 2 * B; cf.Hb = w.O_Hb; cf.Zb = w.O_Zb; cf.out = w.O_out;
      cf.t_start = ctx->stamps ? ctx->stamps + 15 : nullptr;
      FQL_CHECK_CUDA(cudaEventRecord(ctx->ev[56], S0));
      rc = tc_cluster_forward(cf, row_tiles, S0);
      if (rc < 0) return -1;
      if (rc == 0) {
        FQL_CHECK_CUDA(cudaStreamWaitEvent(ctx->s9, ctx->ev[56], 0));
        TcActor fm = actor(FQL_NET_ACTOR_ONESTEP_FLOW, w.XOb, kO, 3 * B, 2 * B, B, w.O_Hb, w.O_Zb, true);
        FQL_TRY(tc_actor_forward(fm, w.O_out + (int64_t)2 * B * sh.A, (long long)3 * B * sh.A, 0, nullptr, ctx->s9));
        FQL_TRY(launch_post_onestep(sh, b, w, raw, ctx->s9, 2));
        FQL_CHECK_CUDA(cudaEventRecord(ctx->ev[57], ctx->s9));
        split_metric = true;
      }
    }
    if (rc == 1) FQL_TRY(tc_actor_forward(fo, w.O_out, (long long)3 * B * sh.A, 0, nullptr, S0));
  }
  FQL_TRY(stamp(ctx, 3, S0));
  FQL_TRY(launch_post_onestep(sh, b, w, raw, S0, split_metric ? 1 : 3));
  FQL_TRY(tc_pad_bf16(w.XC, w.XCb, (int64_t)3 * S * B, sh.F + sh.A, kO, S0));
  TcCritic cr;
  memset(&cr, 0, sizeof(cr));
  cr.d = d; cr.L = &L; cr.params = P; cr.shadow = shadow; cr.M = B; cr.K0pad = kO; cr.x_ss = (long long)B * kO; cr.buf = &w.pC; cr.Hb = w.C_Hb;
  cr.cs_scratch = w.cs_scratch[2];
  bool split_cpost = false;
  if (many_tiles) {
    TcChainSpec t;
    memset(&t, 0, sizeof(t));
    t.d = d; t.L = &L; t.P = 3; t.net[0] = FQL_NET_TARGET_CRITIC; t.net[1] = FQL_NET_CRITIC; t.net[2] = FQL_NET_CRITIC;
    t.params = P; t.shadow = shadow; t.M = B; t.X0b = w.XCb; t.Mcap0 = B; t.buf = &w.pC; t.save = 1; t.n_steps = 1; t.Hb = w.C_Hb;
    if (big_bwd) { t.DGb = w.C_DGb; t.XHb = w.C_XHb; t.save_mask = 6; }
    FQL_TRY(tc_mlp_chain(t, S0));
  } else {
    FQL_CHECK_CUDA(cudaEventRecord(ctx->ev[40], S0));
    cudaStream_t cs[3] = {ctx->s6, ctx->s5, S0};
    const int nets[3] = {FQL_NET_TARGET_CRITIC, FQL_NET_CRITIC, FQL_NET_CRITIC};
    for (int p = 0; p < 3; p++) {
      if (cs[p] != S0) FQL_CHECK_CUDA(cudaStreamWaitEvent(cs[p], ctx->ev[40], 0));
      TcCritic f = cr;
      f.p = p; f.X0b = reinterpret_cast<const bf16*>(w.XCb) + (int64_t)p * S * B * kO;
      FQL_TRY(tc_critic_forward(f, nets[p], w.C_out, cs[p]));
      if (cs[p] != S0) FQL_CHECK_CUDA(cudaEventRecord(ctx->ev[41 + p], cs[p]));
    }
    FQL_CHECK_CUDA(cudaStreamWaitEvent(ctx->s5, ctx->ev[41], 0));
    FQL_TRY(launch_critic_post(sh, hp, b, w, raw, ctx->s5, 1));
    FQL_CHECK_CUDA(cudaEventRecord(ev_cpost, ctx->s5));
    split_cpost = true;
  }
  FQL_TRY(stamp(ctx, 5, S0));
  const DpLamArgs dpl = dp_lam_args(ctx->dp);
  FQL_TRY(launch_critic_post(sh, hp, b, w, raw, S0, split_cpost ? 2 : 3, &dpl));
  if (!split_cpost) FQL_CHECK_CUDA(cudaEventRecord(ev_cpost, S0));

  if (c.do_backward) {
    FQL_CHECK_CUDA(cudaStreamWaitEvent(S2, ev_cpost, 0));
    TcCritic t = cr;
    t.grads = c.st->grads; t.p = 1; t.X0b = reinterpret_cast<const bf16*>(w.XCb) + (int64_t)1 * S * B * kO;
    t.dOut = w.dq; t.dOutb = w.C1_dOutb;
    for (int l = 0; l < NH; l++) { t.dZb[l] = w.C1_dZb[l]; t.dZf[l] = w.C1_dZf[l]; t.dHf[l] = w.C1_dHf[l]; }
    if (pix) t.dX0 = w.dX0C;
    if (big_bwd) {
      FQL_TRY(tc_critic_backward_big(t, w.C_XHb, w.C_DGb, S2));
      FQL_CHECK_CUDA(cudaEventRecord(ctx->ev[36], S2));
    } else {
      FQL_TRY(tc_critic_backward(t, S2, ctx->s5, ctx->s8, &ctx->ev[28]));
      if (pix) FQL_TRY(encoder_grads(c, L, w, FQL_NET_CRITIC, w.dX0C, 2, sh.F + sh.A, w.dfeat[0], 3, S2));
      FQL_CHECK_CUDA(cudaEventRecord(ctx->ev[54], ctx->s8));
      FQL_CHECK_CUDA(cudaStreamWaitEvent(ctx->s5, ctx->ev[54], 0));
      FQL_CHECK_CUDA(cudaEventRecord(ctx->ev[36], ctx->s5));
    }
    if (dp_bucketed) {
      const NetView& nc = L.net[FQL_NET_CRITIC];
      FQL_CHECK_CUDA(cudaStreamWaitEvent(ctx->sc, ctx->ev[36], 0));
      int64_t b0 = nc.begin;
      if (ctx->dp_bc_late) {
        FQL_CHECK_CUDA(cudaStreamWaitEvent(ctx->sc, ctx->ev[16], 0));
        b0 = L.net[FQL_NET_ACTOR_BC_FLOW].begin;
        FQL_REQUIRE(L.net[FQL_NET_ACTOR_BC_FLOW].end == nc.begin, "arena order: bc-flow is not followed by the critic");
      }
      FQL_TRY(stamp(ctx, 22, ctx->sc));
      FQL_TRY(dp_reduce_bucket(ctx->dp, 1, b0, nc.end - b0, nullptr, ctx->sc));
      FQL_TRY(stamp(ctx, 23, ctx->sc));
      FQL_CHECK_CUDA(cudaEventRecord(ctx->ev[59], ctx->sc));
    }
    FQL_CHECK_CUDA(cudaStreamWaitEvent(S2, ctx->ev[36], 0));
    FQL_CHECK_CUDA(cudaStreamWaitEvent(S2, ctx->ev[16], 0));
    FQL_TRY(stamp(ctx, 8, S2));
    FQL_TRY(record_early(ctx, S2));
    TcCritic q = cr;
    q.grads = nullptr; q.p = 2; q.X0b = reinterpret_cast<const bf16*>(w.XCb) + (int64_t)2 * S * B * kO;
    q.dOut = w.dqs; q.dOutb = w.C2_dOutb; q.dX0 = w.dX0;
    for (int l = 0; l < NH; l++) { q.dZb[l] = w.C2_dZb[l]; q.dZf[l] = w.C2_dZf[l]; q.dHf[l] = w.C2_dHf[l]; }
    if (big_bwd) FQL_TRY(tc_critic_backward_big(q, w.C_XHb, w.C_DGb, S0));
    else FQL_TRY(tc_critic_backward(q, S0, nullptr, nullptr, &ctx->ev[44]));
    FQL_TRY(stamp(ctx, 6, S0));
    if (dp_bucketed && c.do_apply && ctx->dp_early_adam) {
      const int blk1 = (int)(L.net[FQL_NET_ACTOR_ONESTEP_FLOW].begin / FQL_LEAF_PAD);
      FQL_CHECK_CUDA(cudaEventRecord(ctx->ev[52], S0));
      FQL_CHECK_CUDA(cudaStreamWaitEvent(ctx->sc, ctx->ev[52], 0));
      FQL_CHECK_CUDA(cudaStreamWaitEvent(ctx->sc, ev_euler, 0));
      FQL_TRY(launch_adam_polyak_stats(L, hp, S, c.st->params, c.st->mu, c.st->nu, c.st->grads, w.gstats + S * 4, w.partials, c.st->shadow,
                                       tc_shadow_seed_elems(d, L), ctx->sc, 0, blk1));
      FQL_TRY(stamp(ctx, 9, ctx->sc));
      FQL_CHECK_CUDA(cudaEventRecord(ctx->ev[59], ctx->sc));
      ctx->adam_done_blk = blk1;
    }
  }
  if (bc_enc_forked) FQL_CHECK_CUDA(cudaStreamWaitEvent(S2, ctx->ev[37], 0));
  FQL_CHECK_CUDA(cudaEventRecord(ev_s2, S2));
  FQL_CHECK_CUDA(cudaStreamWaitEvent(S0, ev_euler, 0));
  if (split_metric) FQL_CHECK_CUDA(cudaStreamWaitEvent(S0, ctx->ev[57], 0));
  if (split_cpost) FQL_CHECK_CUDA(cudaStreamWaitEvent(S0, ev_cpost, 0));
  FQL_TRY(launch_actor_grad(sh, hp, w, raw, S0, w.O_dOutb));
  FQL_TRY(stamp(ctx, 7, S0));
  if (c.do_backward) {
    TcActor bo = actor(FQL_NET_ACTOR_ONESTEP_FLOW, w.XOb, kO, 3 * B, B, B, w.O_Hb, w.O_Zb, true);
    int rc = 1;
    if (!many_tiles && ctx->use_euler_cluster && ctx->use_cluster_bwd && !wide) {
      TcClusterBwdSpec cb;
      memset(&cb, 0, sizeof(cb));
      cb.d = d; cb.L = &L; cb.shadow = shadow; cb.net = FQL_NET_ACTOR_ONESTEP_FLOW; cb.dOutb = w.O_dOutb; cb.M = B;
      cb.Zb = w.O_Zb; cb.z_rows_cap = 3 * B; cb.z_r0 = B; cb.dZb = w.O_dZb; cb.dZf = w.O_dZf;
      cb.t_start = ctx->stamps ? ctx->stamps + 17 : nullptr;
      rc = tc_cluster_dgrad(cb, 0, S0);
      if (rc < 0) return -1;
      if (rc == 0) {
        cudaStream_t ss[5] = {ctx->s4, ctx->s9, ctx->s3, ctx->s7, ctx->s1};
        FQL_CHECK_CUDA(cudaEventRecord(ctx->ev[18], S0));
        for (int i = 0; i < 5; i++) FQL_CHECK_CUDA(cudaStreamWaitEvent(ss[i], ctx->ev[18], 0));
        FQL_TRY(tc_actor_param_grads(bo, w.dapi, w.O_dOutb, w.O_dZb, w.O_dZf, ss, 5));
        for (int i = 0; i < 5; i++) {
          FQL_CHECK_CUDA(cudaEventRecord(ctx->ev[19 + i], ss[i]));
          FQL_CHECK_CUDA(cudaStreamWaitEvent(S0, ctx->ev[19 + i], 0));
        }
      }
    }
    if (rc == 1 && big_bwd) {
      FQL_TRY(tc_actor_backward_big(bo, w.dapi, w.O_dOutb, w.O_dZb, true, S0));
    } else if (rc == 1) {
      FQL_TRY(tc_actor_backward(bo, w.dapi, w.O_dOutb, w.O_dZb, w.O_dZf, S0, ctx->s4, ctx->s9, &ctx->ev[18], true));
      if (pix) {
        FQL_TRY(tc_actor_input_grad(bo, w.O_dZb[0], w.dX0O, S0));
        FQL_TRY(encoder_grads(c, L, w, FQL_NET_ACTOR_ONESTEP_FLOW, w.dX0O, 1, sh.F + sh.A, w.dfeat[2], 1, S0));
      }
      FQL_CHECK_CUDA(cudaEventRecord(ctx->ev[55], ctx->s9));
      FQL_CHECK_CUDA(cudaStreamWaitEvent(ctx->s4, ctx->ev[55], 0));
      FQL_CHECK_CUDA(cudaEventRecord(ctx->ev[26], ctx->s4));
      FQL_CHECK_CUDA(cudaStreamWaitEvent(S0, ctx->ev[26], 0));
    }
    FQL_CHECK_CUDA(cudaStreamWaitEvent(S0, ctx->ev[16], 0));
    FQL_TRY(stamp(ctx, 10, S0));
  }
  FQL_CHECK_CUDA(cudaStreamWaitEvent(S0, ev_s2, 0));
  if (dp_grads && !dp_bucketed) {
    const int64_t t0 = L.net[FQL_NET_TARGET_CRITIC].begin;
    FQL_TRY(dp_reduce_bucket(ctx->dp, 3, 0, t0, raw, S0));
  }
  if (dp_bucketed) {
    const NetView& no = L.net[FQL_NET_ACTOR_ONESTEP_FLOW];
    FQL_TRY(stamp(ctx, 24, S0));
    FQL_TRY(dp_reduce_bucket(ctx->dp, 2, no.begin, no.end - no.begin, raw, S0));
    FQL_TRY(stamp(ctx, 25, S0));
    FQL_CHECK_CUDA(cudaStreamWaitEvent(S0, ctx->ev[59], 0));
  }
  return 0;
}

int enqueue_step(FqlContext* ctx, const StepCall& c, cudaStream_t S0) {
  Layout L;
  WsPtrs w;
  FQL_TRY(check_common(c.d, c.ws, c.ws_bytes, &L, &w));
  const bool tcm = c.d->precision == FQL_PRECISION_BF16_TC;
  if (tcm) {
    FQL_TRY(tc_supported(c.d, false));
    FQL_REQUIRE(c.st->shadow != nullptr, "FQL_PRECISION_BF16_TC needs FqlState.shadow (fql_shadow_bytes() bytes, kept by fql_refresh_shadow)");
  }
  const StepShape sh = make_shape(c.d);
  const FqlHparams hp = *c.hp;
  const int S = sh.S, B = sh.B, H = sh.H;
  FQL_REQUIRE(!(c.d->normalize_q_loss && c.d->global_batch != c.d->batch) || ctx->dp.active,
              "normalize_q_loss with a data-parallel split needs the global mean|q| inside the step (agents/fql.py:74-76): attach a peer-memory "
              "communicator (fql_dp_attach); the fql_step_grads / fql_step_apply split cannot provide it");
  if (ctx->dp.active && c.do_grads) {
    FQL_REQUIRE(c.st->grads == ctx->dp.comm.base[ctx->dp.comm.rank], "data parallel: FqlState.grads must be this rank's symmetric buffer (base[rank])");
    FQL_REQUIRE(c.d->global_batch == (int64_t)c.d->batch * ctx->dp.comm.world && ctx->dp.S == S && !c.raw,
                "data parallel: global_batch must be world x batch (%d x %d), seeds as attached, and the raw accumulators internal", ctx->dp.comm.world, c.d->batch);
  }
  float* raw = c.raw ? c.raw : w.raw_local;
  const float* P = c.st->params;

  if (c.do_grads && !tcm) {
    const FqlBatch& b = *c.b;
    cudaStream_t S1 = ctx->s1, S2 = ctx->s2;
    cudaEvent_t ev_prep = ctx->ev[0], ev_f0 = ctx->ev[1], ev_cpost = ctx->ev[2], ev_euler = ctx->ev[3], ev_s2 = ctx->ev[4];
    FQL_TRY(launch_zero_bc(raw, (int64_t)S * FQL_NUM_RAW, c.do_apply ? c.st->count : nullptr, hp, w.gstats + S * 4, S0, w.cpost_ticket, 3 * S));
    FQL_TRY(encode_observations(c, L, w, S0, ctx));
    FQL_TRY(launch_prep(sh, b, w, S0));
    const bool pix = c.d->reserved[0] > 0;
    FQL_CHECK_CUDA(cudaEventRecord(ev_prep, S0));
    FQL_CHECK_CUDA(cudaStreamWaitEvent(S1, ev_prep, 0));
    FQL_CHECK_CUDA(cudaStreamWaitEvent(S2, ev_prep, 0));

    FwdSpec fF;
    memset(&fF, 0, sizeof(fF));
    fF.P = 1; fF.nv[0] = &L.net[FQL_NET_ACTOR_BC_FLOW]; fF.params = P; fF.arena = L.arena;
    fF.S = S; fF.E = 1; fF.M = 2 * B; fF.H = H; fF.X0 = w.XF; fF.Mcap0 = 2 * B; fF.r0_in = 0;
    fF.buf = &w.pF; fF.r0 = 0; fF.save_z = 1;
    {
      FQL_TRY(mlp_forward(fF, S1));
      FQL_CHECK_CUDA(cudaEventRecord(ev_f0, S1));
      fF.M = B; fF.r0_in = B; fF.r0 = B; fF.save_z = 0;
      for (int i = 0; i < sh.flow_steps; i++) {
        FQL_TRY(launch_euler_update(sh, w, i, S1));
        if (i + 1 < sh.flow_steps) FQL_TRY(mlp_forward(fF, S1));
      }
    }
    FQL_CHECK_CUDA(cudaEventRecord(ev_euler, S1));

    FwdSpec fO;
    memset(&fO, 0, sizeof(fO));
    fO.P = 1; fO.nv[0] = &L.net[FQL_NET_ACTOR_ONESTEP_FLOW]; fO.params = P; fO.arena = L.arena;
    fO.S = S; fO.E = 1; fO.M = 3 * B; fO.H = H; fO.X0 = w.XO; fO.Mcap0 = 3 * B; fO.r0_in = 0;
    fO.buf = &w.pO; fO.r0 = 0; fO.save_z = 1;
    FQL_TRY(mlp_forward(fO, S0));
    FQL_TRY(launch_post_onestep(sh, b, w, raw, S0));
    FwdSpec fC;
    memset(&fC, 0, sizeof(fC));
    fC.P = 3; fC.nv[0] = &L.net[FQL_NET_TARGET_CRITIC]; fC.nv[1] = &L.net[FQL_NET_CRITIC]; fC.nv[2] = &L.net[FQL_NET_CRITIC];
    fC.params = P; fC.arena = L.arena; fC.S = S; fC.E = 2; fC.M = B; fC.H = H; fC.X0 = w.XC; fC.Mcap0 = B; fC.r0_in = 0;
    fC.buf = &w.pC; fC.r0 = 0; fC.save_z = 1;
    FQL_TRY(mlp_forward(fC, S0));
    {
      const DpLamArgs dpl = dp_lam_args(ctx->dp);
      FQL_TRY(launch_critic_post(sh, hp, b, w, raw, S0, 3, &dpl));
    }
    FQL_CHECK_CUDA(cudaEventRecord(ev_cpost, S0));

    FQL_CHECK_CUDA(cudaStreamWaitEvent(S2, ev_f0, 0));
    FQL_TRY(launch_bc_post(sh, w, raw, S2));
    if (c.do_backward) {
      BwdSpec bF;
      memset(&bF, 0, sizeof(bF));
      bF.nv = &L.net[FQL_NET_ACTOR_BC_FLOW]; bF.params = P; bF.grads = c.st->grads; bF.arena = L.arena;
      bF.S = S; bF.E = 1; bF.M = B; bF.H = H; bF.X0 = w.XF; bF.Mcap0 = 2 * B; bF.buf = &w.pF; bF.p = 0; bF.r0 = 0;
      bF.dOut = w.dpred; bF.dpp[0] = w.dF[0]; bF.dpp[1] = w.dF[1];
      if (pix) bF.dX0 = w.dX0F;
      FQL_TRY(mlp_backward(bF, S2));
      if (pix) FQL_TRY(encoder_grads(c, L, w, FQL_NET_ACTOR_BC_FLOW, w.dX0F, 1, sh.F + sh.A + 1, w.dfeat[1], 4, S2));
      FQL_CHECK_CUDA(cudaStreamWaitEvent(S2, ev_cpost, 0));
      BwdSpec bC;
      memset(&bC, 0, sizeof(bC));
      bC.nv = &L.net[FQL_NET_CRITIC]; bC.params = P; bC.grads = c.st->grads; bC.arena = L.arena;
      bC.S = S; bC.E = 2; bC.M = B; bC.H = H; bC.X0 = w.XC + (int64_t)1 * S * B * (sh.F + sh.A); bC.Mcap0 = B;
      bC.buf = &w.pC; bC.p = 1; bC.r0 = 0; bC.dOut = w.dq; bC.dpp[0] = w.dC[0]; bC.dpp[1] = w.dC[1];
      if (pix) bC.dX0 = w.dX0C;
      FQL_TRY(mlp_backward(bC, S2));
      if (pix) FQL_TRY(encoder_grads(c, L, w, FQL_NET_CRITIC, w.dX0C, 2, sh.F + sh.A, w.dfeat[0], 3, S2));
      FQL_TRY(record_early(ctx, S2));
    }
    FQL_CHECK_CUDA(cudaEventRecord(ev_s2, S2));

    if (c.do_backward) {
      BwdSpec bQ;
      memset(&bQ, 0, sizeof(bQ));
      bQ.nv = &L.net[FQL_NET_CRITIC]; bQ.params = P; bQ.grads = nullptr; bQ.arena = L.arena;
      bQ.S = S; bQ.E = 2; bQ.M = B; bQ.H = H; bQ.X0 = w.XC + (int64_t)2 * S * B * (sh.F + sh.A); bQ.Mcap0 = B;
      bQ.buf = &w.pC; bQ.p = 2; bQ.r0 = 0; bQ.dOut = w.dqs; bQ.dpp[0] = w.dCp[0]; bQ.dpp[1] = w.dCp[1]; bQ.dX0 = w.dX0;
      FQL_TRY(mlp_backward(bQ, S0));
    }
    FQL_CHECK_CUDA(cudaStreamWaitEvent(S0, ev_euler, 0));
    FQL_TRY(launch_actor_grad(sh, hp, w, raw, S0));
    if (c.do_backward) {
      BwdSpec bO;
      memset(&bO, 0, sizeof(bO));
      bO.nv = &L.net[FQL_NET_ACTOR_ONESTEP_FLOW]; bO.params = P; bO.grads = c.st->grads; bO.arena = L.arena;
      bO.S = S; bO.E = 1; bO.M = B; bO.H = H; bO.X0 = w.XO + (int64_t)B * (sh.F + sh.A); bO.Mcap0 = 3 * B;
      bO.buf = &w.pO; bO.p = 0; bO.r0 = B; bO.dOut = w.dapi; bO.dpp[0] = w.dO[0]; bO.dpp[1] = w.dO[1];
      if (pix) bO.dX0 = w.dX0O;
      FQL_TRY(mlp_backward(bO, S0));
      if (pix) FQL_TRY(encoder_grads(c, L, w, FQL_NET_ACTOR_ONESTEP_FLOW, w.dX0O, 1, sh.F + sh.A, w.dfeat[2], 1, S0));
    }
    FQL_CHECK_CUDA(cudaStreamWaitEvent(S0, ev_s2, 0));
    if (ctx->dp.active && c.do_backward) {
      const int64_t t0 = L.net[FQL_NET_TARGET_CRITIC].begin;
      FQL_TRY(dp_reduce_bucket(ctx->dp, 3, 0, t0, raw, S0));
    }
  }

  ctx->adam_done_blk = 0;
  if (c.do_grads && tcm) FQL_TRY(enqueue_grads_tc(ctx, c, L, w, sh, hp, raw, S0));
  int raw_ranks = c.raw_ranks > 1 ? c.raw_ranks : 1;
  const float* raw_fin = raw;
  if (ctx->dp.active && c.do_grads) {
    if (!c.do_backward) FQL_TRY(dp_reduce_bucket(ctx->dp, 2, 0, 0, raw, S0));
    raw_fin = dp_raw_all(ctx->dp);
    raw_ranks = ctx->dp.comm.world;
  }
  if (c.do_apply) {
    if (!c.do_grads) FQL_TRY(launch_zero_bc(nullptr, 0, c.st->count, hp, w.gstats + S * 4, S0));
    const int blk0 = ctx->adam_done_blk;
    const int blk1 = blk0 ? (int)(L.net[FQL_NET_TARGET_CRITIC].begin / FQL_LEAF_PAD) : -1;
    FQL_TRY(launch_adam_polyak_stats(L, hp, S, c.st->params, c.st->mu, c.st->nu, c.st->grads, w.gstats + S * 4, w.partials,
                                     tcm ? c.st->shadow : nullptr, tcm ? tc_shadow_seed_elems(c.d, L) : 0, S0, blk0, blk1));
    FQL_TRY(stamp(ctx, 11, S0));
    if (tcm) {
      FQL_CHECK_CUDA(cudaEventRecord(ctx->ev[50], S0));
      FQL_CHECK_CUDA(cudaStreamWaitEvent(ctx->s1, ctx->ev[50], 0));
      FQL_TRY(tc_refresh_shadow_lastlayer(c.d, L, c.st->params, c.st->shadow, ctx->s1));
      FQL_CHECK_CUDA(cudaEventRecord(ctx->ev[51], ctx->s1));
    }
    FinArgs fin;
    memset(&fin, 0, sizeof(fin));
    fin.sh = sh; fin.hp = hp; fin.raw = raw_fin; fin.ranks = raw_ranks; fin.info = c.info;
    FQL_TRY(launch_grad_stats_final(L, S, w.partials, w.gstats, c.st->count, S0, c.info ? &fin : nullptr));
    if (tcm) FQL_CHECK_CUDA(cudaStreamWaitEvent(S0, ctx->ev[51], 0));
  }
  if (c.info && !c.do_apply) FQL_TRY(launch_finalize_info(sh, hp, raw_fin, raw_ranks, w.gstats, c.info, 0, S0));
  FQL_TRY(stamp(ctx, 12, S0));
  return 0;
}

int run_step_on(FqlContext* ctx, const StepCall& c, cudaStream_t S0) {
  cudaStreamCaptureStatus cap = cudaStreamCaptureStatusNone;
  FQL_CHECK_CUDA(cudaStreamIsCapturing(S0, &cap));
  if (!ctx->use_graph || cap != cudaStreamCaptureStatusNone) {
    const long long before = g_fql_launches;
    const int rc0 = enqueue_step(ctx, c, S0);
    ctx->launches += g_fql_launches - before;
    return rc0;
  }

  std::vector<unsigned char> key;
  auto push = [&](const void* p, size_t n) { key.insert(key.end(), (const unsigned char*)p, (const unsigned char*)p + n); };
  push(c.d, sizeof(FqlDims));
  push(c.hp, sizeof(FqlHparams));
  if (c.b) push(c.b, sizeof(FqlBatch));
  push(c.st, sizeof(FqlState));
  push(&c.raw, sizeof(void*)); push(&c.info, sizeof(void*)); push(&c.ws, sizeof(void*)); push(&c.ws_bytes, sizeof(size_t));
  int flags[4] = {c.do_grads, c.do_backward, c.do_apply, c.raw_ranks};
  push(flags, sizeof(flags));
  push(&S0, sizeof(S0));
  GraphEntry* seen = nullptr;
  for (auto& g : ctx->graphs)
    if (g.key == key) {
      if (g.exec) {
        FQL_CHECK_CUDA(cudaGraphLaunch(g.exec, S0));
        ctx->launches += g.kernels;
        return 0;
      }
      seen = &g;
    }
  if (!seen) {
    if (ctx->graphs.size() >= 16) {
      if (ctx->graphs.front().exec) cudaGraphExecDestroy(ctx->graphs.front().exec);
      ctx->graphs.erase(ctx->graphs.begin());
    }
    ctx->graphs.push_back({key, nullptr, 0});
    const long long before = g_fql_launches;
    const int rc0 = enqueue_step(ctx, c, S0);
    ctx->launches += g_fql_launches - before;
    return rc0;
  }
  {
    Layout L;
    WsPtrs w;
    FQL_TRY(check_common(c.d, c.ws, c.ws_bytes, &L, &w));
    if (c.d->precision == FQL_PRECISION_BF16_TC) {
      FQL_TRY(tc_supported(c.d, false));
      FQL_REQUIRE(c.st->shadow != nullptr, "FQL_PRECISION_BF16_TC needs FqlState.shadow");
    }
  }
  FQL_CHECK_CUDA(cudaStreamBeginCapture(S0, cudaStreamCaptureModeThreadLocal));
  const long long before = g_fql_launches;
  int rc = enqueue_step(ctx, c, S0);
  const long long nk = g_fql_launches - before;
  cudaGraph_t graph = nullptr;
  cudaError_t e = cudaStreamEndCapture(S0, &graph);
  if (rc) {
    if (graph) cudaGraphDestroy(graph);
    return rc;
  }
  FQL_CHECK_CUDA(e);
  cudaGraphExec_t exec = nullptr;
  FQL_CHECK_CUDA(cudaGraphInstantiate(&exec, graph, 0));
  cudaGraphDestroy(graph);
  seen->exec = exec;
  seen->kernels = nk;
  FQL_CHECK_CUDA(cudaGraphLaunch(exec, S0));
  ctx->launches += nk;
  return 0;
}


int run_step(FqlContext* ctx, const StepCall& c, void* stream) {
  FQL_REQUIRE(ctx != nullptr, "context is NULL");
  FQL_REQUIRE(c.d && c.hp && c.st, "NULL argument");
  cudaStream_t user = reinterpret_cast<cudaStream_t>(stream);
  if (user != nullptr && user != cudaStreamLegacy) return run_step_on(ctx, c, user);
  FQL_CHECK_CUDA(cudaEventRecord(ctx->ev[6], user));
  FQL_CHECK_CUDA(cudaStreamWaitEvent(ctx->s0, ctx->ev[6], 0));
  const int rc = run_step_on(ctx, c, ctx->s0);
  FQL_CHECK_CUDA(cudaEventRecord(ctx->ev[7], ctx->s0));
  FQL_CHECK_CUDA(cudaStreamWaitEvent(user, ctx->ev[7], 0));
  return rc;
}

}

extern "C" int fql_update_step(FqlContext* ctx, const FqlDims* d, const FqlHparams* hp, const FqlBatch* batch,
                               const FqlState* st, float* info, void* workspace, size_t ws_bytes, void* stream) {
  FQL_REQUIRE(batch != nullptr, "batch is NULL");
  StepCall c{d, hp, batch, st, nullptr, info, workspace, ws_bytes, 1, 1, 1, 1};
  return run_step(ctx, c, stream);
}

extern "C" int fql_step_grads(FqlContext* ctx, const FqlDims* d, const FqlHparams* hp, const FqlBatch* batch,
                              const FqlState* st, float* raw, void* workspace, size_t ws_bytes, void* stream) {
  FQL_REQUIRE(batch != nullptr && raw != nullptr, "batch/raw is NULL");
  StepCall c{d, hp, batch, st, raw, nullptr, workspace, ws_bytes, 1, 1, 0, 1};
  return run_step(ctx, c, stream);
}

extern "C" int fql_step_apply(FqlContext* ctx, const FqlDims* d, const FqlHparams* hp, const FqlState* st, const float* raw,
                              float* info, void* workspace, size_t ws_bytes, void* stream) {
  FQL_REQUIRE(raw != nullptr, "raw is NULL");
  StepCall c{d, hp, nullptr, st, const_cast<float*>(raw), info, workspace, ws_bytes, 0, 0, 1, 1};
  return run_step(ctx, c, stream);
}

extern "C" int fql_step_apply_gathered(FqlContext* ctx, const FqlDims* d, const FqlHparams* hp, const FqlState* st, const float* raw_all,
                                       int32_t ranks, float* info, void* workspace, size_t ws_bytes, void* stream) {
  FQL_REQUIRE(raw_all != nullptr && ranks >= 1, "raw_all is NULL / ranks < 1");
  StepCall c{d, hp, nullptr, st, const_cast<float*>(raw_all), info, workspace, ws_bytes, 0, 0, 1, ranks};
  return run_step(ctx, c, stream);
}

extern "C" int fql_total_loss(FqlContext* ctx, const FqlDims* d, const FqlHparams* hp, const FqlBatch* batch,
                              const FqlState* st, float* info, void* workspace, size_t ws_bytes, void* stream) {
  FQL_REQUIRE(batch != nullptr && info != nullptr, "batch/info is NULL");
  StepCall c{d, hp, batch, st, nullptr, info, workspace, ws_bytes, 1, 0, 0, 1};
  return run_step(ctx, c, stream);
}

namespace {
size_t carve_forward(const FqlDims* d, int rows, int ens, int in_dim, int out_dim, bool ln, void* base, float** X, PassBuf* pb,
                     void** Xb = nullptr, void** Hx = nullptr, float** feat = nullptr, EncBuf* eb = nullptr) {
  Carver c{reinterpret_cast<char*>(base)};
  *X = c.take((int64_t)d->num_seeds * rows * in_dim);
  void* xb = c.take((int64_t)d->num_seeds * rows * 128 / 2 + 4);
  if (Xb) *Xb = xb;
  void* hx = (d->precision == FQL_PRECISION_BF16_TC && d->hidden == 512) ? c.take((int64_t)(tc_euler_scratch_elems(d, rows) / 2 + 4)) : nullptr;
  if (Hx) *Hx = hx;
  if (d->reserved[0] > 0) {
    float* ft = c.take((int64_t)rows * d->obs_dim);
    if (feat) *feat = ft;
    c.off = (c.off + 255) & ~(size_t)255;
    EncBuf tmp;
    c.off += enc_carve(d, rows, base ? c.base + c.off : nullptr, eb ? eb : &tmp, false);
  }
  carve_pass(c, pb, d->num_seeds * ens, rows, d->hidden, d->num_hidden, out_dim, ln, false);
  return c.off + 256;
}
}

extern "C" size_t fql_forward_workspace_bytes(const FqlDims* d, int32_t rows) {
  if (fql_validate_dims(d)) return 0;
  float* X;
  PassBuf pb;
  return carve_forward(d, rows, 2, d->obs_dim + d->action_dim + 1, d->action_dim > 1 ? d->action_dim : 1, true, nullptr, &X, &pb);
}

static int forward_net(const FqlDims* d, const Layout& L, int net, const float* params, const float* X, PassBuf* pb, int rows,
                       cudaStream_t st) {
  FwdSpec f;
  memset(&f, 0, sizeof(f));
  f.P = 1; f.nv[0] = &L.net[net]; f.params = params; f.arena = L.arena;
  f.S = d->num_seeds; f.E = L.net[net].ens; f.M = rows; f.H = d->hidden; f.X0 = X; f.Mcap0 = rows; f.buf = pb;
  return mlp_forward(f, st);
}

extern "C" int fql_mlp_forward(FqlContext*, const FqlDims* d, int32_t net, const float* params, const float* x, float* y,
                               int32_t rows, void* workspace, size_t ws_bytes, void* stream) {
  Layout L;
  FQL_TRY(fql_build_layout(d, &L));
  FQL_REQUIRE(net >= 0 && net < FQL_NUM_NETS && rows >= 1, "bad net/rows");
  FQL_REQUIRE(d->precision == FQL_PRECISION_FP32, "fql_mlp_forward: FP32 only");
  const NetView& nv = L.net[net];
  float* X;
  PassBuf pb;
  const size_t need = carve_forward(d, rows, nv.ens, nv.in_dim, nv.out_dim, nv.ln, nullptr, &X, &pb);
  FQL_REQUIRE(workspace && ws_bytes >= need, "workspace too small: have %zu need %zu", ws_bytes, need);
  carve_forward(d, rows, nv.ens, nv.in_dim, nv.out_dim, nv.ln, workspace, &X, &pb);
  cudaStream_t st = reinterpret_cast<cudaStream_t>(stream);
  FQL_TRY(forward_net(d, L, net, params, x, &pb, rows, st));
  FQL_CHECK_CUDA(cudaMemcpyAsync(y, pb.out, sizeof(float) * (size_t)d->num_seeds * nv.ens * rows * nv.out_dim,
                                 cudaMemcpyDeviceToDevice, st));
  return 0;
}

extern "C" int fql_sample_actions(FqlContext*, const FqlDims* d, const float* params, const void* shadow, const float* obs,
                                  const float* noise, float* actions_out, int32_t rows, void* workspace, size_t ws_bytes,
                                  void* stream) {
  Layout L;
  FQL_TRY(fql_build_layout(d, &L));
  FQL_REQUIRE(rows >= 1, "rows=%d", rows);
  const NetView& nv = L.net[FQL_NET_ACTOR_ONESTEP_FLOW];
  float* X;
  void* Xb;
  PassBuf pb;
  const size_t need = carve_forward(d, rows, 1, nv.in_dim, nv.out_dim, nv.ln, nullptr, &X, &pb);
  FQL_REQUIRE(workspace && ws_bytes >= need, "workspace too small: have %zu need %zu", ws_bytes, need);
  float* feat = nullptr;
  EncBuf eb;
  carve_forward(d, rows, 1, nv.in_dim, nv.out_dim, nv.ln, workspace, &X, &pb, &Xb, nullptr, &feat, &eb);
  cudaStream_t st = reinterpret_cast<cudaStream_t>(stream);
  const int64_t R = (int64_t)d->num_seeds * rows;
  if (d->reserved[0] > 0) {
    FQL_TRY(enc_forward(d, nv.enc, params, reinterpret_cast<const uint8_t*>(obs), rows, eb, feat, st));
    obs = feat;
  }
  FQL_TRY(launch_concat(obs, d->obs_dim, noise, d->action_dim, 0.f, 0, X, R, st));
  if (d->precision == FQL_PRECISION_BF16_TC && !tc_wide_input(d)) {
    FQL_REQUIRE(shadow != nullptr, "FQL_PRECISION_BF16_TC needs the bf16 shadow");
    const int kp = (int)round_up64(nv.in_dim, 64);
    FQL_TRY(tc_pad_bf16(X, Xb, R, nv.in_dim, kp, st));
    TcChainSpec t;
    memset(&t, 0, sizeof(t));
    t.d = d; t.L = &L; t.P = 1; t.net[0] = FQL_NET_ACTOR_ONESTEP_FLOW; t.params = params; t.shadow = shadow;
    t.M = rows; t.X0b = Xb; t.Mcap0 = rows; t.n_steps = 1; t.out_override = actions_out; t.clip_out = 1;
    return tc_mlp_chain(t, st);
  }
  FQL_TRY(forward_net(d, L, FQL_NET_ACTOR_ONESTEP_FLOW, params, X, &pb, rows, st));
  FQL_TRY(launch_clip(pb.out, actions_out, R * d->action_dim, st));
  return 0;
}

extern "C" int fql_compute_flow_actions(FqlContext*, const FqlDims* d, const float* params, const void* shadow, const float* obs,
                                        const float* noise, float* actions_out, int32_t rows, void* workspace, size_t ws_bytes,
                                        void* stream) {
  Layout L;
  FQL_TRY(fql_build_layout(d, &L));
  FQL_REQUIRE(rows >= 1, "rows=%d", rows);
  const NetView& nv = L.net[FQL_NET_ACTOR_BC_FLOW];
  float* X;
  void* Xb;
  void* Hx = nullptr;
  PassBuf pb;
  const size_t need = carve_forward(d, rows, 1, nv.in_dim, nv.out_dim, nv.ln, nullptr, &X, &pb);
  FQL_REQUIRE(workspace && ws_bytes >= need, "workspace too small: have %zu need %zu", ws_bytes, need);
  float* feat = nullptr;
  EncBuf eb;
  carve_forward(d, rows, 1, nv.in_dim, nv.out_dim, nv.ln, workspace, &X, &pb, &Xb, &Hx, &feat, &eb);
  cudaStream_t st = reinterpret_cast<cudaStream_t>(stream);
  const int64_t R = (int64_t)d->num_seeds * rows;
  if (d->reserved[0] > 0) {
    FQL_TRY(enc_forward(d, nv.enc, params, reinterpret_cast<const uint8_t*>(obs), rows, eb, feat, st));
    obs = feat;
  }
  FQL_TRY(launch_concat(obs, d->obs_dim, noise, d->action_dim, 0.f, 1, X, R, st));
  if (d->precision == FQL_PRECISION_BF16_TC && !tc_wide_input(d)) {
    FQL_REQUIRE(shadow != nullptr, "FQL_PRECISION_BF16_TC needs the bf16 shadow");
    const int kp = (int)round_up64(nv.in_dim, 64);
    FQL_TRY(tc_pad_bf16(X, Xb, R, nv.in_dim, kp, st));
    if (d->hidden == 512 && Hx) {
      TcEulerSpec e;
      memset(&e, 0, sizeof(e));
      e.d = d; e.L = &L; e.params = params; e.shadow = shadow; e.X0b = Xb; e.Mcap0 = rows; e.r0_in = 0; e.M = rows;
      e.a0 = noise; e.target = actions_out; e.scratch = Hx;
      return tc_euler_cluster(e, st);
    }
    TcChainSpec t;
    memset(&t, 0, sizeof(t));
    t.d = d; t.L = &L; t.P = 1; t.net[0] = FQL_NET_ACTOR_BC_FLOW; t.params = params; t.shadow = shadow;
    t.M = rows; t.X0b = Xb; t.Mcap0 = rows; t.n_steps = d->flow_steps; t.a0 = noise; t.target = actions_out;
    return tc_mlp_chain(t, st);
  }
  for (int i = 0; i < d->flow_steps; i++) {
    FQL_TRY(forward_net(d, L, FQL_NET_ACTOR_BC_FLOW, params, X, &pb, rows, st));
    FQL_TRY(launch_euler_inplace(X, pb.out, d->obs_dim, d->action_dim, R, i, d->flow_steps, actions_out, st));
  }
  return 0;
}

extern "C" int fql_version(void) { return FQL_ABI_VERSION; }
extern "C" const char* fql_last_error(void) { return g_err; }
extern "C" const char* fql_info_name(int i) {
  static const char* names[FQL_NUM_INFO] = {
      "critic/critic_loss", "critic/q_mean", "critic/q_max", "critic/q_min", "actor/actor_loss", "actor/bc_flow_loss",
      "actor/distill_loss", "actor/q_loss", "actor/q", "actor/mse", "grad/max", "grad/min", "grad/norm"};
  return (i >= 0 && i < FQL_NUM_INFO) ? names[i] : nullptr;
}
extern "C" int64_t fql_arena_floats(const FqlDims* d) {
  Layout L;
  if (fql_build_layout(d, &L)) return -1;
  return L.arena;
}
extern "C" size_t fql_workspace_bytes(const FqlDims* d) {
  Layout L;
  if (fql_build_layout(d, &L)) return 0;
  WsPtrs w;
  return carve_workspace(d, L, nullptr, &w);
}
extern "C" size_t fql_shadow_bytes(const FqlDims* d) {
  Layout L;
  if (fql_build_layout(d, &L)) return 0;
  if (d->precision != FQL_PRECISION_BF16_TC) return 0;
  return (size_t)d->num_seeds * (size_t)tc_shadow_seed_elems(d, L) * 2;
}
extern "C" int fql_refresh_shadow(const FqlDims* d, const float* params, void* shadow, void* stream) {
  Layout L;
  FQL_TRY(fql_build_layout(d, &L));
  if (d->precision != FQL_PRECISION_BF16_TC) return 0;
  return tc_refresh_shadow(d, L, params, shadow, reinterpret_cast<cudaStream_t>(stream));
}

extern "C" int fql_layout(const FqlDims* d, FqlLeaf* leaves, int32_t cap, int32_t* n_leaves) {
  Layout L;
  FQL_TRY(fql_build_layout(d, &L));
  int n = 0;
  auto put = [&](int net, int layer, int kind, int ens, int rows, int cols, int64_t off) {
    if (leaves && n < cap) leaves[n] = FqlLeaf{net, layer, kind, ens, rows, cols, off};
    n++;
  };
  static const int kOrder[FQL_NUM_NETS] = {FQL_NET_ACTOR_BC_FLOW, FQL_NET_CRITIC, FQL_NET_ACTOR_ONESTEP_FLOW, FQL_NET_TARGET_CRITIC};
  for (int oi = 0; oi < FQL_NUM_NETS; oi++) {
    const int t = kOrder[oi];
    const NetView& v = L.net[t];
    for (int l = 0; l < v.n_layers; l++) {
      put(t, l, FQL_LEAF_KERNEL, v.ens, v.k_of(l), v.n_of(l), v.off_w[l]);
      put(t, l, FQL_LEAF_BIAS, v.ens, 1, v.n_of(l), v.off_b[l]);
      if (v.ln && l + 1 < v.n_layers) {
        put(t, l, FQL_LEAF_LN_SCALE, v.ens, 1, v.n_of(l), v.off_lns[l]);
        put(t, l, FQL_LEAF_LN_BIAS, v.ens, 1, v.n_of(l), v.off_lnb[l]);
      }
    }
    if (v.has_enc) {
      static const int stacks[3] = {16, 32, 32};
      int c = d->reserved[2], h = d->reserved[0], w = d->reserved[1];
      for (int i = 0; i < 3; i++) {
        const int f = stacks[i];
        const int cin[3] = {c, f, f};
        for (int j = 0; j < 3; j++) {
          put(t, 3 * i + j, FQL_LEAF_CONV_KERNEL, 1, 9 * cin[j], f, v.enc.off_cw[i][j]);
          put(t, 3 * i + j, FQL_LEAF_CONV_BIAS, 1, 1, f, v.enc.off_cb[i][j]);
        }
        c = f; h = (h + 1) / 2; w = (w + 1) / 2;
      }
      put(t, 0, FQL_LEAF_ENC_DENSE_KERNEL, 1, h * w * c, d->obs_dim, v.enc.off_dw);
      put(t, 0, FQL_LEAF_ENC_DENSE_BIAS, 1, 1, d->obs_dim, v.enc.off_db);
    }
  }
  if (n_leaves) *n_leaves = n;
  FQL_REQUIRE(!leaves || n <= cap, "leaf table too small: need %d", n);
  return 0;
}
```

fql_b200/csrc/step.cuh:

```cuda
#pragma once
#include "common.cuh"

#include <cudaTypedefs.h>

enum {
  RAW_CRITIC_SQ = 0, RAW_Q_SUM = 1, RAW_BC_SQ = 2, RAW_DISTILL_SQ = 3, RAW_QPI_SUM = 4, RAW_QPI_ABS = 5, RAW_MSE = 6,
  RAW_Q_MAX = 9, RAW_Q_NEGMIN = 10,
};

struct StepShape {
  int S, B, GB, F, A, H, NH;
  int q_agg_min, normalize_q_loss, flow_steps;
};

struct PassBuf {
  float* Z[FQL_MAXL];
  float* Hh[FQL_MAXL];
  float* mu[FQL_MAXL];
  float* rstd[FQL_MAXL];
  float* out;
  int G, Mcap;
};

struct EncTc {
  void *img, *y0, *p[3], *r1[3], *r2[3], *xs[3], *flat;
  void *wf, *wd, *wdense;
  void *dzb, *da, *db, *dc;
};
struct EncBuf {
  EncTc tc;
  float *pl[3], *c1[3], *x[3];
  uint8_t* arg[3];
  float *flat, *z, *scratch;
  float *dz, *dflat, *da, *db, *dc, *partial;
  int flat_dim;
};

struct WsPtrs {
  float *XO, *XF, *XC, *vel;
  float *O_out, *F_out, *C_out;
  float *dq, *dqs, *dpred, *dapi, *target, *dX0;
  float *raw_local;
  float *gstats;
  float *partials;
  float *cpost_part;
  int *cpost_ticket;
  PassBuf pO, pF, pC;
  float *dC[2], *dCp[2], *dF[2], *dO[2];
  void *XOb, *XFb, *XCb;
  void *O_Hb[FQL_MAXL], *O_Zb[FQL_MAXL], *F_Hb[FQL_MAXL], *F_Zb[FQL_MAXL], *E_Hb[FQL_MAXL];
  void *C_Hb[FQL_MAXL];
  void *C_XHb[FQL_MAXL], *C_DGb[FQL_MAXL];
  void *O_dZb[FQL_MAXL], *F_dZb[FQL_MAXL], *O_dOutb, *F_dOutb;
  float *O_dZf[FQL_MAXL], *F_dZf[FQL_MAXL];
  void *C1_dZb[FQL_MAXL], *C1_dOutb, *C2_dZb[FQL_MAXL], *C2_dOutb;
  float *C1_dZf[FQL_MAXL], *C1_dHf[FQL_MAXL], *C2_dZf[FQL_MAXL], *C2_dHf[FQL_MAXL];
  float *euler_a;
  float *cs_scratch[3];
  float *feat[5];
  float *dfeat[3];
  float *dX0F, *dX0O, *dX0C;
  EncBuf enc[5];
  const float *src[5];
  void *euler_hx;
};

StepShape make_shape(const FqlDims* d);
size_t carve_workspace(const FqlDims* d, const Layout& L, void* base, WsPtrs* w);

int launch_prep(const StepShape& sh, const FqlBatch& b, const WsPtrs& w, cudaStream_t st);
int launch_post_onestep(const StepShape& sh, const FqlBatch& b, const WsPtrs& w, float* raw, cudaStream_t st, int parts = 3);
struct DpLamArgs;
int launch_critic_post(const StepShape& sh, const FqlHparams& hp, const FqlBatch& b, const WsPtrs& w, float* raw, cudaStream_t st, int parts = 3,
                       const DpLamArgs* dpl = nullptr);
int launch_bc_post(const StepShape& sh, const WsPtrs& w, float* raw, cudaStream_t st);
int launch_euler_update(const StepShape& sh, const WsPtrs& w, int step, cudaStream_t st);
int launch_actor_grad(const StepShape& sh, const FqlHparams& hp, const WsPtrs& w, float* raw, cudaStream_t st, void* dapib = nullptr);
int launch_finalize_info(const StepShape& sh, const FqlHparams& hp, const float* raw, int ranks, const float* gstats, float* info,
                         int with_grad_stats, cudaStream_t st);
int launch_clip(const float* in, float* out, int64_t n, cudaStream_t st);
int launch_concat(const float* x0, int k0, const float* x1, int k1, float c2, int k2, float* out, int64_t rows, cudaStream_t st);
int launch_euler_inplace(float* X, const float* v, int F, int A, int64_t rows, int step, int nsteps, float* out, cudaStream_t st);

int launch_adam_polyak_stats(const Layout& L, const FqlHparams& hp, int S, float* params, float* mu, float* nu,
                             const float* grads, const float* bc, float* partials, void* shadow, int64_t shadow_seed, cudaStream_t st,
                             int blk0 = 0, int blk1 = -1);
struct FinArgs {
  StepShape sh;
  FqlHparams hp;
  const float* raw;
  int ranks;
  float* info;
};
int launch_grad_stats_final(const Layout& L, int S, const float* partials, float* gstats, int32_t* count_inc, cudaStream_t st,
                            const FinArgs* fin = nullptr);

#ifdef __CUDACC__
__device__ __forceinline__ void fql_finalize_info_seed(const StepShape& sh, const FqlHparams& hp, const float* raw, int ranks, const float* gstats,
                                                       float* info, int s, int with_grad_stats) {
  float rw[FQL_NUM_RAW];
  for (int i = 0; i < FQL_NUM_RAW; i++) rw[i] = raw[s * FQL_NUM_RAW + i];
  for (int r = 1; r < ranks; r++) {
    const float* o = raw + ((int64_t)r * sh.S + s) * FQL_NUM_RAW;
    for (int i = 0; i < 9; i++) rw[i] += o[i];
    rw[RAW_Q_MAX] = fmaxf(rw[RAW_Q_MAX], o[RAW_Q_MAX]);
    rw[RAW_Q_NEGMIN] = fmaxf(rw[RAW_Q_NEGMIN], o[RAW_Q_NEGMIN]);
  }
  float* o = info + s * FQL_NUM_INFO;
  const float gb = (float)sh.GB, A = (float)sh.A;
  const float critic_loss = rw[RAW_CRITIC_SQ] / (2.0f * gb);
  const float bc = rw[RAW_BC_SQ] / (gb * A);
  const float distill = rw[RAW_DISTILL_SQ] / (gb * A);
  const float q = rw[RAW_QPI_SUM] / gb;
  float q_loss = -q;
  if (sh.normalize_q_loss) q_loss = (1.0f / (rw[RAW_QPI_ABS] / gb)) * q_loss;
  o[0] = critic_loss;
  o[1] = rw[RAW_Q_SUM] / (2.0f * gb);
  o[2] = rw[RAW_Q_MAX];
  o[3] = -rw[RAW_Q_NEGMIN];
  o[4] = bc + hp.alpha * distill + q_loss;
  o[5] = bc;
  o[6] = distill;
  o[7] = q_loss;
  o[8] = q;
  o[9] = rw[RAW_MSE] / (gb * A);
  if (with_grad_stats) {
    o[10] = gstats[s * 4 + 0];
    o[11] = gstats[s * 4 + 1];
    o[12] = gstats[s * 4 + 2];
  } else {
    o[10] = o[11] = o[12] = 0.f;
  }
}
#endif
int launch_zero(float* p, int64_t n, cudaStream_t st);
int launch_zero_bc(float* p, int64_t n, const int32_t* count, const FqlHparams& hp, float* bc, cudaStream_t st, int* tickets = nullptr,
                   int n_tickets = 0);

struct TcChainSpec {
  const FqlDims* d;
  const Layout* L;
  int P;
  int net[FQL_MAXP];
  const float* params;
  const void* shadow;
  int M;
  const void* X0b;
  int Mcap0, r0_in;
  PassBuf* buf;
  int r0, save;
  float* out_override;
  void* const* Hb;
  void* const* Zb;
  int Mcap_override;
  int n_steps;
  const float* a0;
  float* target;
  int clip_out;
  void* const* DGb;
  void* const* XHb;
  int save_mask;
};
struct TcChain2BwdSpec {
  const FqlDims* d;
  const Layout* L;
  int net;
  const float* params;
  const void* shadow;
  const void* dOutb;
  int M, Mcap, r0;
  int Mcap_dz;
  void* const* DGb;
  void* const* XHb;
  float* const* rstd;
  void* const* dZb;
  float* dX0;
};
int tc_mlp_chain2_backward(const TcChain2BwdSpec& f, cudaStream_t st);
int tc_supported(const FqlDims* d, bool fused_kernels = true);
inline bool tc_wide_input(const FqlDims* d) { return d->obs_dim + d->action_dim + 1 > 128; }
int64_t tc_shadow_seed_elems(const FqlDims* d, const Layout& L);
int tc_refresh_shadow(const FqlDims* d, const Layout& L, const float* params, void* shadow, cudaStream_t st);
int tc_refresh_shadow_lastlayer(const FqlDims* d, const Layout& L, const float* params, void* shadow, cudaStream_t st);
int tc_pad_bf16(const float* x, void* y, int64_t rows, int K0, int K0pad, cudaStream_t st);
int tc_mlp_chain(const TcChainSpec& f, cudaStream_t st);
int tc_mlp_chain2_supported(const FqlDims* d);
int tc_mlp_chain2(const TcChainSpec& f, cudaStream_t st);
PFN_cuTensorMapEncodeTiled_v12000 get_encode();
int make_map_2d(CUtensorMap* m, const void* base, uint64_t inner, uint64_t rows, uint32_t box_inner, uint32_t box_rows,
                CUtensorMapSwizzle swz = CU_TENSOR_MAP_SWIZZLE_128B);

enum { TC_MODE_STORE_F32 = 0, TC_MODE_FWD_HIDDEN = 1, TC_MODE_DGRAD_GELU = 2, TC_MODE_EULER = 3, TC_MODE_WGRAD_LN = 4 };
struct TcOperand {
  const void* ptr;
  int inner, rows;
  long long ld;
  int g0;
  long long s0;
  int g1;
  long long s1;
};
struct TcPtr {
  void* base;
  long long s0, s1;
  int ld;
};
struct TcGemmSpec {
  int M, N, K, G0, G1;
  int a_mn, b_mn;
  TcOperand A, B;
  int mode;
  TcPtr bias, out_f, out_h, out_z, zin, act, xb, target;
  int F, Adim, step, n_steps, clip;
  int ksplit;
  TcPtr ln_s, ln_b, dbias, wmaster, dln_s, dln_b;
  void* dbg;
};
int launch_colsum_bf16(const void* X, int64_t G, int64_t M, int N, float* out, int64_t out_stride_g0, int G0, int64_t out_stride_g1, cudaStream_t st);
int tc_gemm(const TcGemmSpec& s, cudaStream_t st);
struct TcActor;
int tc_actor_input_grad(const TcActor& t, const void* dZ0b, float* dX0, cudaStream_t st);

struct TcActor {
  const FqlDims* d;
  const Layout* L;
  int net;
  const float* params;
  const void* shadow;
  float* grads;
  int M;
  const void* X0b;
  int K0pad;
  long long x_ss;
  void* Hb[FQL_MAXL];
  void* Zb[FQL_MAXL];
  long long h_ss;
  float* cs_scratch;
};
struct TcEuler {
  float* act;
  float* target;
  int step, n_steps;
};
struct TcCritic {
  const FqlDims* d;
  const Layout* L;
  const float* params;
  const void* shadow;
  float* grads;
  int M, p;
  const void* X0b;
  int K0pad;
  long long x_ss;
  const PassBuf* buf;
  void* const* Hb;
  const float* dOut;
  void* dOutb;
  void* dZb[FQL_MAXL];
  float* dZf[FQL_MAXL];
  float* dHf[FQL_MAXL];
  float* dX0;
  float* cs_scratch;
};
int tc_actor_forward(const TcActor& t, float* out, long long out_ss, int clip, const TcEuler* eu, cudaStream_t st);
int tc_actor_backward(const TcActor& t, const float* dOut, void* dOutb, void* const dZb[FQL_MAXL], float* const dZf[FQL_MAXL],
                      cudaStream_t st, cudaStream_t side, cudaStream_t side2, cudaEvent_t* ev, bool dOutb_ready = false);
int tc_critic_backward(const TcCritic& t, cudaStream_t st, cudaStream_t side, cudaStream_t side2, cudaEvent_t* ev);
int tc_critic_forward(const TcCritic& t, int net, float* out, cudaStream_t st);
int tc_actor_backward_big(const TcActor& t, const float* dOut, void* dOutb, void* const dZb[FQL_MAXL], bool dOutb_ready, cudaStream_t st);
int tc_critic_backward_big(const TcCritic& t, void* const* XHb, void* const* DGb, cudaStream_t st);

struct TcEulerSpec {
  const FqlDims* d;
  const Layout* L;
  const float* params;
  const void* shadow;
  const void* X0b;
  int Mcap0, r0_in, M;
  const float* a0;
  const float* c0;
  float* target;
  void* scratch;
  void* dbg;
  void* t_start;
};
size_t tc_euler_scratch_elems(const FqlDims* d, int M);
struct TcClusterFwdSpec {
  const FqlDims* d;
  const Layout* L;
  const float* params;
  const void* shadow;
  int net;
  const void* X0b;
  int rows_cap, r0, M;
  void* const* Hb;
  void* const* Zb;
  float* out;
  void* t_start;
};
int tc_cluster_forward(const TcClusterFwdSpec& f, int other_clusters, cudaStream_t st);
struct TcClusterBwdSpec {
  const FqlDims* d;
  const Layout* L;
  const void* shadow;
  int net;
  const void* dOutb;
  int M;
  void* const* Zb;
  int z_rows_cap, z_r0;
  void* const* dZb;
  float* const* dZf;
  void* t_start;
};
int tc_cluster_dgrad(const TcClusterBwdSpec& f, int other_clusters, cudaStream_t st);
int tc_actor_param_grads(const TcActor& t, const float* dOut, const void* dOutb, void* const dZb[FQL_MAXL], float* const dZf[FQL_MAXL],
                         cudaStream_t* streams, int n_streams);
int tc_euler_cluster(const TcEulerSpec& f, cudaStream_t st);

size_t enc_carve(const FqlDims* d, int64_t B, void* base, EncBuf* e, bool for_backward);
int enc_forward(const FqlDims* d, const EncView& v, const float* params, const uint8_t* obs, int64_t B, const EncBuf& e, float* feat,
                cudaStream_t st);
int enc_backward(const FqlDims* d, const EncView& v, const float* params, float* grads, const uint8_t* obs, int64_t B, const EncBuf& e,
                 const float* dfeat, cudaStream_t st);
size_t enc_tc_carve(const FqlDims* d, int64_t B, void* base, EncBuf* e, bool for_backward);
int enc_tc_forward(const FqlDims* d, const EncView& v, const float* params, const uint8_t* obs, int64_t B, const EncBuf& e, float* feat,
                   cudaStream_t st);
int enc_tc_backward(const FqlDims* d, const EncView& v, const float* params, float* grads, const uint8_t* obs, int64_t B, const EncBuf& e,
                    const float* dfeat, cudaStream_t st);
int launch_extract_feat_grad(const float* dX0, float* out, int E, int64_t M, int K0, int F, cudaStream_t st);
```

fql_b200/csrc/tc_prims.cuh:

```cuda
#pragma once
#include <cuda.h>
#include <cuda_bf16.h>
#include <stdint.h>

namespace tc {

__device__ __forceinline__ uint32_t smem_u32(const void* p) { return (uint32_t)__cvta_generic_to_shared(p); }
__device__ __forceinline__ bool elect_one() {
  uint32_t pred = 0;
  asm volatile(
      "{\n\t.reg .pred P;\n\telect.sync _|P, 0xffffffff;\n\tselp.u32 %0, 1, 0, P;\n\t}\n"
      : "=r"(pred));
  return pred != 0;
}

__device__ __forceinline__ void mbar_init(uint64_t* bar, uint32_t count) {
  asm volatile("mbarrier.init.shared::cta.b64 [%0], %1;" ::"r"(smem_u32(bar)), "r"(count));
}
__device__ __forceinline__ void fence_barrier_init() { asm volatile("fence.mbarrier_init.release.cluster;" ::: "memory"); }
__device__ __forceinline__ void mbar_expect_tx(uint64_t* bar, uint32_t bytes) {
  asm volatile("mbarrier.arrive.expect_tx.shared::cta.b64 _, [%0], %1;" ::"r"(smem_u32(bar)), "r"(bytes) : "memory");
}
__device__ __forceinline__ void mbar_arrive(uint64_t* bar) {
  asm volatile("mbarrier.arrive.shared::cta.b64 _, [%0];" ::"r"(smem_u32(bar)) : "memory");
}
__device__ __forceinline__ bool mbar_try_wait(uint64_t* bar, uint32_t parity) {
  uint32_t ok;
  asm volatile(
      "{\n\t.reg .pred P;\n\tmbarrier.try_wait.parity.shared::cta.b64 P, [%1], %2;\n\tselp.u32 %0, 1, 0, P;\n\t}\n"
      : "=r"(ok)
      : "r"(smem_u32(bar)), "r"(parity)
      : "memory");
  return ok != 0;
}
static __device__ __noinline__ void mbar_timeout(uint64_t* bar, uint32_t parity) {
  printf("fql_b200: mbarrier timeout (block %d thread %d bar %p parity %u)\n", blockIdx.x, threadIdx.x, (void*)bar, parity);
  __trap();
}
__device__ __forceinline__ void mbar_wait_u(uint64_t* bar, uint32_t parity) {
  asm volatile(
      "{\n\t.reg .pred P1, P2;\n\t.reg .u32 c;\n\tmov.u32 c, 0;\n"
      "W_LOOP:\n\tmbarrier.try_wait.parity.shared::cta.b64 P1, [%0], %1;\n\t@P1 bra W_DONE;\n\t"
      "add.u32 c, c, 1;\n\tsetp.lt.u32 P2, c, 0x4000000;\n\t@P2 bra W_LOOP;\n\ttrap;\n"
      "W_DONE:\n\t}\n" ::"r"(smem_u32(bar)), "r"(parity)
      : "memory");
}
__device__ __forceinline__ void mbar_wait(uint64_t* bar, uint32_t parity) {
  uint32_t spins = 0;
  while (!mbar_try_wait(bar, parity)) {
    if (++spins > (1u << 26)) mbar_timeout(bar, parity);
  }
}

__device__ __forceinline__ uint32_t cluster_ctarank() {
  uint32_t r;
  asm volatile("mov.u32 %0, %%cluster_ctarank;" : "=r"(r));
  return r;
}
__device__ __forceinline__ void cluster_sync_all() {
  asm volatile("barrier.cluster.arrive.release;" ::: "memory");
  asm volatile("barrier.cluster.wait.acquire;" ::: "memory");
}
__device__ __forceinline__ void mbar_wait_cluster_u(uint64_t* bar, uint32_t parity) {
  asm volatile(
      "{\n\t.reg .pred P1, P2;\n\t.reg .u32 c;\n\tmov.u32 c, 0;\n"
      "WC_LOOP:\n\tmbarrier.try_wait.parity.acquire.cluster.shared::cta.b64 P1, [%0], %1;\n\t@P1 bra WC_DONE;\n\t"
      "add.u32 c, c, 1;\n\tsetp.lt.u32 P2, c, 0x4000000;\n\t@P2 bra WC_LOOP;\n\ttrap;\n"
      "WC_DONE:\n\t}\n" ::"r"(smem_u32(bar)), "r"(parity)
      : "memory");
}

__device__ __forceinline__ void tma_prefetch_desc(const CUtensorMap* m) {
  asm volatile("prefetch.tensormap [%0];" ::"l"(reinterpret_cast<uint64_t>(m)) : "memory");
}
__device__ __forceinline__ void tma_prefetch_2d(const CUtensorMap* m, int c0, int c1) {
  asm volatile("cp.async.bulk.prefetch.tensor.2d.L2.global.tile [%0, {%1, %2}];" ::"l"(reinterpret_cast<uint64_t>(m)), "r"(c0), "r"(c1) : "memory");
}
__device__ __forceinline__ void tma_load_2d(void* dst, const CUtensorMap* m, uint64_t* bar, int c0, int c1) {
  asm volatile(
      "cp.async.bulk.tensor.2d.shared::cluster.global.mbarrier::complete_tx::bytes [%0], [%1, {%3, %4}], [%2];"
      ::"r"(smem_u32(dst)), "l"(reinterpret_cast<uint64_t>(m)), "r"(smem_u32(bar)), "r"(c0), "r"(c1)
      : "memory");
}
__device__ __forceinline__ void fence_proxy_async_smem() { asm volatile("fence.proxy.async.shared::cta;" ::: "memory"); }

__device__ __forceinline__ void tmem_alloc(uint32_t* dst_smem, uint32_t cols) {
  asm volatile("tcgen05.alloc.cta_group::1.sync.aligned.shared::cta.b32 [%0], %1;" ::"r"(smem_u32(dst_smem)), "r"(cols) : "memory");
  asm volatile("tcgen05.relinquish_alloc_permit.cta_group::1.sync.aligned;" ::: "memory");
}
__device__ __forceinline__ void tmem_dealloc(uint32_t taddr, uint32_t cols) {
  asm volatile("tcgen05.dealloc.cta_group::1.sync.aligned.b32 %0, %1;" ::"r"(taddr), "r"(cols) : "memory");
}
__device__ __forceinline__ void tc_fence_before() { asm volatile("tcgen05.fence::before_thread_sync;" ::: "memory"); }
__device__ __forceinline__ void tc_fence_after() { asm volatile("tcgen05.fence::after_thread_sync;" ::: "memory"); }
__device__ __forceinline__ void umma_bf16(uint32_t d_tmem, uint64_t a_desc, uint64_t b_desc, uint32_t idesc, uint32_t accumulate) {
  asm volatile(
      "{\n\t.reg .pred p;\n\tsetp.ne.b32 p, %4, 0;\n\t"
      "tcgen05.mma.cta_group::1.kind::f16 [%0], %1, %2, %3, p;\n\t}\n"
      ::"r"(d_tmem), "l"(a_desc), "l"(b_desc), "r"(idesc), "r"(accumulate)
      : "memory");
}
__device__ __forceinline__ void umma_bf16_x4(uint32_t d_tmem, uint64_t a_desc, uint64_t b_desc, uint64_t a_step, uint64_t b_step,
                                             uint32_t idesc, uint32_t accumulate_first) {
  asm volatile(
      "{\n\t.reg .pred p, q;\n\t.reg .b64 a1, a2, a3, b1, b2, b3;\n\t"
      "setp.ne.b32 p, %4, 0;\n\t"
      "setp.eq.b32 q, 0, 0;\n\t"
      "add.u64 a1, %1, %5;\n\tadd.u64 b1, %2, %6;\n\t"
      "add.u64 a2, a1, %5;\n\tadd.u64 b2, b1, %6;\n\t"
      "add.u64 a3, a2, %5;\n\tadd.u64 b3, b2, %6;\n\t"
      "tcgen05.mma.cta_group::1.kind::f16 [%0], %1, %2, %3, p;\n\t"
      "tcgen05.mma.cta_group::1.kind::f16 [%0], a1, b1, %3, q;\n\t"
      "tcgen05.mma.cta_group::1.kind::f16 [%0], a2, b2, %3, q;\n\t"
      "tcgen05.mma.cta_group::1.kind::f16 [%0], a3, b3, %3, q;\n\t}\n"
      ::"r"(d_tmem), "l"(a_desc), "l"(b_desc), "r"(idesc), "r"(accumulate_first), "l"(a_step), "l"(b_step)
      : "memory");
}
__device__ __forceinline__ void umma_bf16_x2(uint32_t d_tmem, uint64_t a_desc, uint64_t b_desc, uint64_t a_step, uint64_t b_step,
                                             uint32_t idesc, uint32_t accumulate_first) {
  asm volatile(
      "{\n\t.reg .pred p, q;\n\t.reg .b64 a1, b1;\n\t"
      "setp.ne.b32 p, %4, 0;\n\t"
      "setp.eq.b32 q, 0, 0;\n\t"
      "add.u64 a1, %1, %5;\n\tadd.u64 b1, %2, %6;\n\t"
      "tcgen05.mma.cta_group::1.kind::f16 [%0], %1, %2, %3, p;\n\t"
      "tcgen05.mma.cta_group::1.kind::f16 [%0], a1, b1, %3, q;\n\t}\n"
      ::"r"(d_tmem), "l"(a_desc), "l"(b_desc), "r"(idesc), "r"(accumulate_first), "l"(a_step), "l"(b_step)
      : "memory");
}
__device__ __forceinline__ void umma_commit(uint64_t* bar) {
  asm volatile("tcgen05.commit.cta_group::1.mbarrier::arrive::one.shared::cluster.b64 [%0];" ::"r"(smem_u32(bar)) : "memory");
}
__device__ __forceinline__ void tmem_ld32(uint32_t taddr, uint32_t (&r)[32]) {
  asm volatile(
      "tcgen05.ld.sync.aligned.32x32b.x32.b32 "
      "{%0, %1, %2, %3, %4, %5, %6, %7, %8, %9, %10, %11, %12, %13, %14, %15, "
      "%16, %17, %18, %19, %20, %21, %22, %23, %24, %25, %26, %27, %28, %29, %30, %31}, [%32];"
      : "=r"(r[0]), "=r"(r[1]), "=r"(r[2]), "=r"(r[3]), "=r"(r[4]), "=r"(r[5]), "=r"(r[6]), "=r"(r[7]), "=r"(r[8]), "=r"(r[9]),
        "=r"(r[10]), "=r"(r[11]), "=r"(r[12]), "=r"(r[13]), "=r"(r[14]), "=r"(r[15]), "=r"(r[16]), "=r"(r[17]), "=r"(r[18]),
        "=r"(r[19]), "=r"(r[20]), "=r"(r[21]), "=r"(r[22]), "=r"(r[23]), "=r"(r[24]), "=r"(r[25]), "=r"(r[26]), "=r"(r[27]),
        "=r"(r[28]), "=r"(r[29]), "=r"(r[30]), "=r"(r[31])
      : "r"(taddr)
      : "memory");
}
__device__ __forceinline__ void tmem_st32(uint32_t taddr, const uint32_t (&r)[32]) {
  asm volatile(
      "tcgen05.st.sync.aligned.32x32b.x32.b32 [%0], "
      "{%1, %2, %3, %4, %5, %6, %7, %8, %9, %10, %11, %12, %13, %14, %15, %16, "
      "%17, %18, %19, %20, %21, %22, %23, %24, %25, %26, %27, %28, %29, %30, %31, %32};"
      ::"r"(taddr), "r"(r[0]), "r"(r[1]), "r"(r[2]), "r"(r[3]), "r"(r[4]), "r"(r[5]), "r"(r[6]), "r"(r[7]), "r"(r[8]), "r"(r[9]),
        "r"(r[10]), "r"(r[11]), "r"(r[12]), "r"(r[13]), "r"(r[14]), "r"(r[15]), "r"(r[16]), "r"(r[17]), "r"(r[18]), "r"(r[19]),
        "r"(r[20]), "r"(r[21]), "r"(r[22]), "r"(r[23]), "r"(r[24]), "r"(r[25]), "r"(r[26]), "r"(r[27]), "r"(r[28]), "r"(r[29]),
        "r"(r[30]), "r"(r[31])
      : "memory");
}
__device__ __forceinline__ void tmem_wait_ld() { asm volatile("tcgen05.wait::ld.sync.aligned;" ::: "memory"); }
__device__ __forceinline__ void tmem_wait_st() { asm volatile("tcgen05.wait::st.sync.aligned;" ::: "memory"); }

__device__ __forceinline__ uint64_t make_smem_desc(uint32_t saddr, uint32_t lbo, uint32_t sbo) {
  uint64_t d = 0;
  d |= (uint64_t)((saddr >> 4) & 0x3FFF);
  d |= (uint64_t)((lbo >> 4) & 0x3FFF) << 16;
  d |= (uint64_t)((sbo >> 4) & 0x3FFF) << 32;
  d |= (uint64_t)1 << 46;
  d |= (uint64_t)2 << 61;
  return d;
}
__device__ __forceinline__ uint64_t make_smem_desc_sw64(uint32_t saddr, uint32_t lbo, uint32_t sbo) {
  uint64_t d = 0;
  d |= (uint64_t)((saddr >> 4) & 0x3FFF);
  d |= (uint64_t)((lbo >> 4) & 0x3FFF) << 16;
  d |= (uint64_t)((sbo >> 4) & 0x3FFF) << 32;
  d |= (uint64_t)1 << 46;
  d |= (uint64_t)4 << 61;
  return d;
}
__host__ __device__ constexpr uint32_t make_idesc_bf16(uint32_t M, uint32_t N, bool a_mn, bool b_mn) {
  return (1u << 4)
         | (1u << 7)
         | (1u << 10)
         | ((a_mn ? 1u : 0u) << 15)
         | ((b_mn ? 1u : 0u) << 16)
         | ((N >> 3) << 17)
         | ((M >> 4) << 24);
}

__device__ __forceinline__ uint32_t sw128_off(uint32_t r, uint32_t c) { return r * 128u + ((c ^ (r & 7u)) << 4); }

__device__ __forceinline__ float tanh_approx(float x) {
  float y;
  asm("tanh.approx.f32 %0, %1;" : "=f"(y) : "f"(x));
  return y;
}

}
```

include/fql_b200.h:

```cpp
#ifndef FQL_B200_H_
#define FQL_B200_H_

#include <stddef.h>
#include <stdint.h>

#ifdef __cplusplus
extern "C" {
#endif

#define FQL_ABI_VERSION 1

enum { FQL_NET_ACTOR_BC_FLOW = 0, FQL_NET_ACTOR_ONESTEP_FLOW = 1, FQL_NET_CRITIC = 2, FQL_NET_TARGET_CRITIC = 3, FQL_NUM_NETS = 4 };
enum { FQL_LEAF_KERNEL = 0, FQL_LEAF_BIAS = 1, FQL_LEAF_LN_SCALE = 2, FQL_LEAF_LN_BIAS = 3,
       FQL_LEAF_CONV_KERNEL = 4, FQL_LEAF_CONV_BIAS = 5, FQL_LEAF_ENC_DENSE_KERNEL = 6, FQL_LEAF_ENC_DENSE_BIAS = 7 };
enum { FQL_PRECISION_FP32 = 0,
       FQL_PRECISION_BF16_TC = 1,
       FQL_PRECISION_BF16_ENC = 2 };

typedef struct FqlDims {
  int32_t batch;
  int32_t global_batch;
  int32_t obs_dim;
  int32_t action_dim;
  int32_t hidden;
  int32_t num_hidden;
  int32_t critic_layer_norm;
  int32_t actor_layer_norm;
  int32_t q_agg_min;
  int32_t normalize_q_loss;
  int32_t flow_steps;
  int32_t num_seeds;
  int32_t precision;
  int32_t reserved[3];
} FqlDims;

typedef struct FqlHparams {
  float lr, beta1, beta2, eps;
  float discount, tau, alpha;
  float one_minus_beta1, one_minus_beta2, one_minus_tau;
  float reserved[2];
} FqlHparams;

typedef struct FqlLeaf {
  int32_t net;
  int32_t layer;
  int32_t kind;
  int32_t ens;
  int32_t rows, cols;
  int64_t offset;
} FqlLeaf;

typedef struct FqlBatch {
  const float* observations;
  const float* actions;
  const float* next_observations;
  const float* rewards;
  const float* masks;
  const float* z_next;
  const float* x0;
  const float* t;
  const float* z;
  const float* z_metric;
} FqlBatch;

typedef struct FqlState {
  float* params;
  float* mu;
  float* nu;
  float* grads;
  int32_t* count;
  void* shadow;
} FqlState;

#define FQL_NUM_INFO 13
#define FQL_NUM_RAW 16

typedef struct FqlContext FqlContext;

int fql_version(void);
const char* fql_last_error(void);
const char* fql_info_name(int i);
int fql_context_create(FqlContext** out);
int fql_context_destroy(FqlContext* ctx);
long long fql_launch_count(FqlContext* ctx);

int64_t fql_arena_floats(const FqlDims* d);
int fql_layout(const FqlDims* d, FqlLeaf* leaves, int32_t cap, int32_t* n_leaves);
size_t fql_workspace_bytes(const FqlDims* d);
size_t fql_shadow_bytes(const FqlDims* d);
size_t fql_forward_workspace_bytes(const FqlDims* d, int32_t rows);

int fql_update_step(FqlContext* ctx, const FqlDims* d, const FqlHparams* hp, const FqlBatch* batch,
                    const FqlState* st, float* info, void* workspace, size_t ws_bytes, void* stream);
int fql_step_grads(FqlContext* ctx, const FqlDims* d, const FqlHparams* hp, const FqlBatch* batch,
                   const FqlState* st, float* raw, void* workspace, size_t ws_bytes, void* stream);
int fql_step_apply(FqlContext* ctx, const FqlDims* d, const FqlHparams* hp, const FqlState* st, const float* raw,
                   float* info, void* workspace, size_t ws_bytes, void* stream);
int fql_step_apply_gathered(FqlContext* ctx, const FqlDims* d, const FqlHparams* hp, const FqlState* st, const float* raw_all,
                            int32_t ranks, float* info, void* workspace, size_t ws_bytes, void* stream);
int fql_set_early_grads_event(FqlContext* ctx, void* event);
int64_t fql_early_grads_floats(const FqlDims* d);
#define FQL_DP_MAX_RANKS 8
typedef struct FqlDpComm {
  int32_t rank, world;
  void* base[FQL_DP_MAX_RANKS];
  void* base_mc;
} FqlDpComm;
size_t fql_dp_symmetric_bytes(const FqlDims* d, int32_t world);
int fql_dp_attach(FqlContext* ctx, const FqlDims* d, const FqlDpComm* comm);
int fql_dp_allreduce(FqlContext* ctx, int32_t bucket, int64_t off, int64_t n, void* stream);

int fql_total_loss(FqlContext* ctx, const FqlDims* d, const FqlHparams* hp, const FqlBatch* batch,
                   const FqlState* st, float* info, void* workspace, size_t ws_bytes, void* stream);

int fql_sample_actions(FqlContext* ctx, const FqlDims* d, const float* params, const void* shadow, const float* obs,
                       const float* noise, float* actions_out, int32_t rows, void* workspace, size_t ws_bytes, void* stream);
int fql_compute_flow_actions(FqlContext* ctx, const FqlDims* d, const float* params, const void* shadow, const float* obs,
                             const float* noise, float* actions_out, int32_t rows, void* workspace, size_t ws_bytes, void* stream);
int fql_mlp_forward(FqlContext* ctx, const FqlDims* d, int32_t net, const float* params, const float* x, float* y,
                    int32_t rows, void* workspace, size_t ws_bytes, void* stream);
int fql_target_update(const FqlDims* d, const FqlHparams* hp, float* params, void* shadow, void* stream);
int fql_refresh_shadow(const FqlDims* d, const float* params, void* shadow, void* stream);

int fql_gather_rows(const void* src, void* dst, const int64_t* idxs, int64_t n_idx, int64_t row_bytes, void* stream);
int fql_gather_frames(const uint8_t* obs_src, const uint8_t* next_src, uint8_t* obs_out, uint8_t* next_out,
                      const int64_t* idxs, const int64_t* init_idxs, const int64_t* crop_from, int64_t n_idx,
                      int32_t img_h, int32_t img_w, int32_t img_c, int32_t frame_stack, int32_t pad, void* stream);
int fql_fill_noise(const FqlDims* d, uint64_t seed, uint64_t step, float* z_next, float* x0, float* t, float* z,
                   float* z_metric, void* stream);
int fql_fill_noise_rows(const FqlDims* d, uint64_t seed, uint64_t step, int64_t row_offset, float* z_next, float* x0, float* t,
                        float* z, float* z_metric, void* stream);


int fql_debug_stamps(FqlContext* ctx, unsigned long long* host_out, int n);

size_t fql_conv3x3_workspace_bytes(void);
int fql_conv3x3_bf16(const void* x, const float* w_hwio, const float* bias, int32_t B, int32_t H, int32_t W, int32_t cin, int32_t cout,
                     int32_t input_gradient, const void* mask, const void* add, int32_t relu_out, void* out, void* workspace,
                     size_t ws_bytes, void* stream);
int fql_conv3x3_wgrad_bf16(const void* x, const void* dy, int32_t B, int32_t H, int32_t W, int32_t cin, int32_t cout, float* gw, float* gb,
                           void* workspace, size_t ws_bytes, void* stream);

typedef struct FqlTestOperand {
  const void* ptr;
  int32_t inner, rows;
  int64_t ld;
  int32_t g0;
  int64_t s0;
  int32_t g1;
  int64_t s1;
} FqlTestOperand;
typedef struct FqlTestPtr {
  void* base;
  int64_t s0, s1;
  int32_t ld;
} FqlTestPtr;
typedef struct FqlTestGemm {
  int32_t mode, M, N, K, G0, G1, a_mn, b_mn, ksplit;
  FqlTestOperand A, B;
  FqlTestPtr bias, out_f, out_h, out_z, zin, act, xb, target, ln_s, ln_b, dbias, wmaster, dln_s, dln_b;
  int32_t F, Adim, step, n_steps, clip;
} FqlTestGemm;
int fql_test_tc_gemm(const FqlTestGemm* g, void* stream);
int fql_test_act_ln_bf16(const float* Z, const float* scale, const float* bias, int64_t par_s, int64_t par_e, void* Hb, float* mu,
                         float* rstd, int32_t M, int32_t N, int32_t S, int32_t E, int32_t ln, void* stream);
int fql_test_ln_bwd_bf16(const float* dH, const float* Z, const float* scale, int64_t scale_s, int64_t scale_e, float* dZ, void* dZb,
                         int32_t M, int32_t N, int32_t S, int32_t E, int64_t z_rows_e, int64_t z_rows_s, void* stream);
int fql_test_gelu_bwd_bf16(const float* dH, const float* Z, float* dZ, void* dZb, int32_t M, int32_t N, int32_t S, int32_t E,
                           int64_t z_rows_e, int64_t z_rows_s, void* stream);
int fql_test_colsum_bf16(const void* X, int64_t G, int64_t M, int32_t N, float* out, int64_t out_stride_g0, int32_t G0,
                         int64_t out_stride_g1, void* stream);

#ifdef __cplusplus
}
#endif
#endif
```

Measured before the change: 1.145 million.

## Fuse critic forward with LayerNorm into cluster kernel and split Adam across streams

Adds a MODE_FWD_LN variant of the cluster Euler kernel. It runs the whole critic ensemble MLP forward in one persistent launch and computes the LayerNorm statistics across the 16-CTA cluster, exchanging them with st.async to distributed shared memory. One of the critic forward passes uses it when it fits, replacing the per-layer tc_critic_forward path. It also splits the Adam/Polyak update into three parameter ranges launched on different streams so parts of the optimizer overlap with remaining backward work. This adds cluster-barrier synchronisation and more stream and event dependencies.

```diff
diff --git a/fql_b200/_lib.py b/fql_b200/_lib.py
--- a/fql_b200/_lib.py
+++ b/fql_b200/_lib.py
@@ -110,6 +110,8 @@
                                          C.c_int64, C.c_int64, C.c_void_p]),
     'fql_test_colsum_bf16': (C.c_int, [C.c_void_p, C.c_int64, C.c_int64, C.c_int32, C.c_void_p, C.c_int64, C.c_int32, C.c_int64,
                                        C.c_void_p]),
+    'fql_test_critic_cluster_forward': (C.c_int, [C.POINTER(FqlDims), C.c_void_p, C.c_void_p, C.c_void_p, C.c_int32, C.c_void_p, C.c_void_p,
+                                                  C.c_void_p, C.c_void_p, C.c_void_p, C.c_void_p]),
     'fql_set_early_grads_event':(C.c_int, [C.c_void_p, C.c_void_p]),
     'fql_early_grads_floats': (C.c_int64, [C.POINTER(FqlDims)]),
     'fql_total_loss': (C.c_int, [C.c_void_p, C.POINTER(FqlDims), C.POINTER(FqlHparams), C.POINTER(FqlBatch), C.POINTER(FqlState),
diff --git a/fql_b200/csrc/euler_cluster.cu b/fql_b200/csrc/euler_cluster.cu
--- a/fql_b200/csrc/euler_cluster.cu
+++ b/fql_b200/csrc/euler_cluster.cu
@@ -48,12 +48,18 @@
   unsigned long long* dbg;
   unsigned long long* t_start;
   int dbg_it;
+  float* mu[FQL_MAXL];
+  float* rstd[FQL_MAXL];
+  long long off_lns[FQL_MAXL], off_lnb[FQL_MAXL];
+  int w_row_e[FQL_MAXL];
+  int wl_row_e;
 };
 
 struct HMaps {
   CUtensorMap m[4];
 };
-constexpr int MODE_EULER = 0, MODE_FWD = 1, MODE_DGRAD = 2;
+constexpr int MODE_EULER = 0, MODE_FWD = 1, MODE_DGRAD = 2, MODE_FWD_LN = 3;
+constexpr int CRIT_E = 2;
 
 __device__ __forceinline__ unsigned long long gtime() {
   unsigned long long t;
@@ -105,11 +111,15 @@
   uint64_t* x_full = bars + 20;
   uint64_t* half_ready = bars + 21;
   uint32_t* tmem_slot = reinterpret_cast<uint32_t*>(bars + 24);
+  uint64_t* stat_full = bars + 26;
+  float2* sStat = reinterpret_cast<float2*>(bars + 32);
+  float* sLn = reinterpret_cast<float*>(sStat + NC * TILE_M);
 
   const int warp = __shfl_sync(0xffffffffu, (int)(threadIdx.x >> 5), 0), lane = threadIdx.x & 31;
   const uint32_t j = __shfl_sync(0xffffffffu, cluster_ctarank(), 0);
   const int cl = blockIdx.x / NC;
-  const int tile = cl % a.tiles, s = cl / a.tiles;
+  const int tile = cl % a.tiles, sr = cl / a.tiles;
+  const int s = (MODE == MODE_FWD_LN) ? sr / CRIT_E : sr, e = (MODE == MODE_FWD_LN) ? sr % CRIT_E : 0;
   const int NL = a.NL;
   const int total = a.n_steps * NL;
   const int hx_row = (s * a.tiles + tile) * TILE_M;
@@ -129,6 +139,7 @@
     mbar_init(free_a, NC * NISS);
     mbar_init(a_ready, NEPI);
     mbar_init(x_full, 1);
+    if (MODE == MODE_FWD_LN) mbar_init(stat_full, 1);
     fence_barrier_init();
   }
   if (warp == 1) tmem_alloc(tmem_slot, 2 * ACC_SET);
@@ -137,7 +148,14 @@
     const bool lastl = (l == NL - 1);
     const int N = lastl ? a.A : a.H;
     const int col = lastl ? c : (int)j * NCOL + c;
-    sBias[i] = (c < NCOL && col < N && !(l == 0 && a.c0)) ? a.params[(int64_t)s * a.arena + a.off_b[l] + col] : 0.f;
+    sBias[i] = (c < NCOL && col < N && !(l == 0 && a.c0)) ? a.params[(int64_t)s * a.arena + a.off_b[l] + e * N + col] : 0.f;
+  }
+  if constexpr (MODE == MODE_FWD_LN) {
+    static_assert(MODE != MODE_FWD_LN || NCOL == 32, "the LayerNorm chain is built for clusters of 16");
+    for (int i = threadIdx.x; i < (NL - 1) * 64; i += NTHREADS) {
+      const int l = i >> 6, c = i & 63;
+      sLn[i] = a.params[(int64_t)s * a.arena + (c < 32 ? a.off_lns[l] : a.off_lnb[l]) + e * a.H + (int)j * NCOL + (c & 31)];
+    }
   }
   if (threadIdx.x <= a.n_steps) sT[threadIdx.x] = (float)((double)threadIdx.x / (double)a.n_steps);
   tc_fence_before();
@@ -168,8 +186,8 @@
             if (l == 0) tma_load_2d(sB, &mapWL, full_b, 0, a.wl_row + s * a.wl_rows_s + (int)j * NCOL);
             else tma_load_2d(sB + kb * B_BLK, &mapW, full_b, kb * KB, a.w_row[l] + s * a.w_rows_s + (int)j * NCOL);
           } else {
-            if (!last) tma_load_2d(sB + kb * B_BLK, &mapW, full_b, (int)j * NCOL, a.w_row[l] + s * a.w_rows_s + kb * KB);
-            else tma_load_2d(sB + kb * B_BLK, &mapWL, full_b, 0, a.wl_row + s * a.wl_rows_s + kb * KB);
+            if (!last) tma_load_2d(sB + kb * B_BLK, &mapW, full_b, (int)j * NCOL, a.w_row[l] + s * a.w_rows_s + e * a.w_row_e[l] + kb * KB);
+            else tma_load_2d(sB + kb * B_BLK, &mapWL, full_b, 0, a.wl_row + s * a.wl_rows_s + e * a.wl_row_e + kb * KB);
           }
         }
         if (l >= 1) {
@@ -187,7 +205,7 @@
                   "cp.async.bulk.tensor.2d.shared::cluster.global.mbarrier::complete_tx::bytes.multicast::cluster [%0], [%1, {%3, %4}], [%2], %5;"
                   ::"r"(smem_u32(sA + sbk * A_SUB)), "l"(reinterpret_cast<uint64_t>(MODE != MODE_EULER ? &mapsH.m[l - 1] : &mapsH.m[0])),
                   "r"(smem_u32(&full_a[sbk])), "r"(sbk * SUB),
-                  "r"(MODE != MODE_EULER ? s * a.rows_cap + a.r0 + tile * TILE_M : buf * (a.S * a.tiles * TILE_M) + hx_row), "h"(MASK)
+                  "r"(MODE != MODE_EULER ? sr * a.rows_cap + a.r0 + tile * TILE_M : buf * (a.S * a.tiles * TILE_M) + hx_row), "h"(MASK)
                   : "memory");
           }
           n_pub++;
@@ -261,6 +279,7 @@
     const int et = threadIdx.x - EPI0;
     float* st_row = a.state + (int64_t)blockIdx.x * MAX_A * TILE_M + row;
     int n_exch = 0;
+    int n_ln = 0;
     int l = 0, step = 0;
     for (int it = 0; it < total; it++, l = (l + 1 == NL) ? 0 : l + 1, step += (l == 0)) {
       const bool last = (l == NL - 1);
@@ -358,6 +377,55 @@
               for (int i = 0; i < 8; i++) h[i] = gelu_fast(__uint_as_float(r0[c * 8 + i]) + sb[half * 32 + c * 8 + i]);
               dst[c] = make_uint4(pack2(h[0], h[1]), pack2(h[2], h[3]), pack2(h[4], h[5]), pack2(h[6], h[7]));
             }
+          } else if constexpr (MODE == MODE_FWD_LN) {
+            const int64_t e0 = ((int64_t)sr * a.rows_cap + a.r0 + grow) * a.H + j * NCOL;
+            float4* zf = reinterpret_cast<float4*>(a.Fsave[l] + e0);
+            float s1 = 0.f, s2 = 0.f;
+#pragma unroll
+            for (int c = 0; c < 8; c++) {
+              float z[4];
+#pragma unroll
+              for (int i = 0; i < 4; i++) z[i] = __uint_as_float(r0[c * 4 + i]) + sb[c * 4 + i];
+              if (valid) zf[c] = make_float4(z[0], z[1], z[2], z[3]);
+#pragma unroll
+              for (int i = 0; i < 4; i++) {
+                const float g = gelu_fast(z[i]);
+                r0[c * 4 + i] = __float_as_uint(g);
+                s1 += g;
+                s2 += g * g;
+              }
+            }
+            if (et == 0) mbar_expect_tx(stat_full, NC * TILE_M * 8);
+            const uint32_t slot = smem_u32(sStat + j * TILE_M + row), bar = smem_u32(stat_full);
+#pragma unroll 4
+            for (int p = 0; p < NC; p++) st_async_v2(mapa_shared(slot, p), s1, s2, mapa_shared(bar, p));
+            mbar_wait_cluster_u(stat_full, n_ln & 1);
+            n_ln++;
+            float t1 = 0.f, t2 = 0.f;
+#pragma unroll
+            for (int p = 0; p < NC; p++) {
+              const float2 v = sStat[p * TILE_M + row];
+              t1 += v.x;
+              t2 += v.y;
+            }
+            constexpr float inv_n = 1.0f / (float)(NC * NCOL);
+            const float mu = t1 * inv_n;
+            const float rstd = rsqrtf(fmaxf(0.f, t2 * inv_n - mu * mu) + FQL_LN_EPS);
+            const float* ln = sLn + l * 64;
+            if (valid) {
+              uint4* dh = reinterpret_cast<uint4*>(a.Hsave[l] + e0);
+#pragma unroll
+              for (int c = 0; c < 4; c++) {
+                float h[8];
+#pragma unroll
+                for (int i = 0; i < 8; i++) h[i] = (__uint_as_float(r0[c * 8 + i]) - mu) * rstd * ln[c * 8 + i] + ln[32 + c * 8 + i];
+                dh[c] = make_uint4(pack2(h[0], h[1]), pack2(h[2], h[3]), pack2(h[4], h[5]), pack2(h[6], h[7]));
+              }
+              if (j == 0) {
+                a.mu[l][(int64_t)sr * a.rows_cap + a.r0 + grow] = mu;
+                a.rstd[l][(int64_t)sr * a.rows_cap + a.r0 + grow] = rstd;
+              }
+            }
           } else if (valid) {
             const int64_t e0 = ((int64_t)s * a.rows_cap + a.r0 + grow) * a.H + j * NCOL + half * 32;
             uint4* dh = reinterpret_cast<uint4*>(a.Hsave[l] + e0);
@@ -377,9 +445,9 @@
           __syncwarp();
           if (lane == 0) mbar_arrive(&half_ready[half]);
           if (dbg && et == 0 && it == DBG_IT - 1) dbg[1 + half] = gtime();
-        } else if (MODE == MODE_FWD) {
+        } else if (MODE == MODE_FWD || MODE == MODE_FWD_LN) {
           if (half == 0 && j == 0 && valid) {
-            float* o = a.out + ((int64_t)s * a.rows_cap + a.r0 + grow) * a.A;
+            float* o = a.out + ((int64_t)sr * a.rows_cap + a.r0 + grow) * a.A;
 #pragma unroll
             for (int c = 0; c < AMAX; c++)
               if (c < a.A) o[c] = __uint_as_float(r0[c]) + sb[c];
@@ -436,7 +504,9 @@
 int launch_euler(const EulerArgs& a, const TcEulerSpec& f, cudaStream_t st, bool query_only, int* max_clusters) {
   constexpr int NCOL = 512 / NC;
   const FqlDims* d = f.d;
-  const int smem = NSUB * A_SUB + (a.H / KB) * (KB * NCOL * 2) + (a.K0pad / KB) * A_BLK + a.NL * 64 * 4 + 64 * 4 + 256 + 1024;
+  const int groups = a.S * (MODE == MODE_FWD_LN ? CRIT_E : 1);
+  const int smem = NSUB * A_SUB + (a.H / KB) * (KB * NCOL * 2) + (a.K0pad / KB) * A_BLK + a.NL * 64 * 4 + 64 * 4 + 256 + 1024 +
+                   (MODE == MODE_FWD_LN ? NC * TILE_M * 8 + a.NL * 64 * 4 : 0);
   FQL_REQUIRE(smem <= 232448, "euler_cluster_kernel: shared memory %d > 227 KB", smem);
   auto kern = euler_cluster_kernel<NC, AMAX, MODE>;
   static bool attr_set[FQL_MAX_DEVICES] = {};
@@ -448,7 +518,7 @@
   }
   cudaLaunchConfig_t cfg;
   memset(&cfg, 0, sizeof(cfg));
-  cfg.gridDim = dim3(NC * a.tiles * a.S);
+  cfg.gridDim = dim3(NC * a.tiles * groups);
   cfg.blockDim = dim3(NTHREADS);
   cfg.dynamicSmemBytes = smem;
   cfg.stream = st;
@@ -483,7 +553,7 @@
     FQL_TRY(make_map_2d(&mapsH.m[0], f.scratch, d->hidden, (uint64_t)2 * a.S * a.tiles * TILE_M, SUB, TILE_M, CU_TENSOR_MAP_SWIZZLE_64B));
   } else {
     for (int l = 0; l + 1 < a.NL; l++)
-      FQL_TRY(make_map_2d(&mapsH.m[l], a.Hsave[l], d->hidden, (uint64_t)a.S * a.rows_cap, SUB, TILE_M, CU_TENSOR_MAP_SWIZZLE_64B));
+      FQL_TRY(make_map_2d(&mapsH.m[l], a.Hsave[l], d->hidden, (uint64_t)groups * a.rows_cap, SUB, TILE_M, CU_TENSOR_MAP_SWIZZLE_64B));
   }
   FQL_CHECK_CUDA(cudaLaunchKernelEx(&cfg, kern, mapX, mapW, mapWL, mapsH, a));
   FQL_CHECK_LAUNCH();
@@ -576,6 +646,36 @@
   if (a.A <= 8) return launch_euler<16, 8, MODE_FWD>(a, e, st, false, nullptr) ? -1 : 0;
   if (a.A <= 16) return launch_euler<16, 16, MODE_FWD>(a, e, st, false, nullptr) ? -1 : 0;
   return launch_euler<16, 32, MODE_FWD>(a, e, st, false, nullptr) ? -1 : 0;
+}
+
+int tc_cluster_critic_forward(const TcCritic& t, int net, float* out, int other_clusters, cudaStream_t st) {
+  const FqlDims* d = t.d;
+  const NetView& nv = t.L->net[net];
+  if (d->hidden != 512 || !nv.ln || nv.ens != CRIT_E || nv.n_layers > 5 || nv.n_layers < 2 || nv.out_dim > 8 || nv.in_dim > 128) return 1;
+  const int64_t Mcap = t.buf->Mcap;
+  FQL_REQUIRE(Mcap == t.M && t.K0pad == (int)round_up64(nv.in_dim, 64) && t.x_ss % t.K0pad == 0,
+              "tc_cluster_critic_forward: dense pass buffers and a [S][rows][K0pad] operand expected (M %d Mcap %lld K0pad %d)", t.M,
+              (long long)Mcap, t.K0pad);
+  EulerArgs a;
+  const int x_rows = (int)(t.x_ss / t.K0pad);
+  if (fill_args(a, d, *t.L, net, t.params, t.M, x_rows, 0)) return -1;
+  TcEulerSpec e;
+  memset(&e, 0, sizeof(e));
+  e.d = d; e.L = t.L; e.params = t.params; e.shadow = t.shadow; e.X0b = t.X0b; e.Mcap0 = x_rows; e.r0_in = 0; e.M = t.M;
+  if (a.tiles * a.S * CRIT_E + other_clusters > max_clusters16(a, e)) return 1;
+  const int64_t prow = (int64_t)t.p * a.S * CRIT_E * Mcap;
+  for (int l = 0; l + 1 < nv.n_layers; l++) {
+    a.Hsave[l] = reinterpret_cast<__nv_bfloat16*>(t.Hb[l]) + prow * a.H;
+    a.Fsave[l] = t.buf->Z[l] + prow * a.H;
+    a.mu[l] = t.buf->mu[l] + prow;
+    a.rstd[l] = t.buf->rstd[l] + prow;
+    a.off_lns[l] = nv.off_lns[l];
+    a.off_lnb[l] = nv.off_lnb[l];
+    a.w_row_e[l] = nv.k_of(l);
+  }
+  a.wl_row_e = a.H;
+  a.out = out + prow; a.rows_cap = (int)Mcap; a.r0 = 0;
+  return launch_euler<16, 8, MODE_FWD_LN>(a, e, st, false, nullptr) ? -1 : 0;
 }
 
 int tc_cluster_dgrad(const TcClusterBwdSpec& f, int other_clusters, cudaStream_t st) {
@@ -603,3 +703,26 @@
   a.t_start = reinterpret_cast<unsigned long long*>(f.t_start);
   return launch_euler<16, 8, MODE_DGRAD>(a, e, st, false, nullptr) ? -1 : 0;
 }
+
+extern "C" int fql_test_critic_cluster_forward(const FqlDims* d, const float* params, const void* shadow, const void* X0b, int32_t M,
+                                               void* const* Hb, float* const* Z, float* const* mu, float* const* rstd, float* out,
+                                               void* stream) {
+  FQL_REQUIRE(d && params && shadow && X0b && Hb && Z && mu && rstd && out && M >= 1, "fql_test_critic_cluster_forward: NULL argument or M=%d", M);
+  Layout L;
+  FQL_TRY(fql_build_layout(d, &L));
+  const NetView& nv = L.net[FQL_NET_CRITIC];
+  PassBuf buf;
+  memset(&buf, 0, sizeof(buf));
+  for (int l = 0; l + 1 < nv.n_layers; l++) {
+    buf.Z[l] = Z[l]; buf.mu[l] = mu[l]; buf.rstd[l] = rstd[l];
+  }
+  buf.Mcap = M;
+  TcCritic t;
+  memset(&t, 0, sizeof(t));
+  t.d = d; t.L = &L; t.params = params; t.shadow = shadow; t.M = M; t.p = 0; t.X0b = X0b;
+  t.K0pad = (int)round_up64(nv.in_dim, 64); t.x_ss = (long long)M * t.K0pad; t.buf = &buf; t.Hb = Hb;
+  const int rc = tc_cluster_critic_forward(t, FQL_NET_CRITIC, out, 0, reinterpret_cast<cudaStream_t>(stream));
+  FQL_REQUIRE(rc != 1, "fql_test_critic_cluster_forward: the cluster kernel does not take this critic (hidden %d, seeds %d, M %d)", d->hidden,
+              d->num_seeds, M);
+  return rc;
+}
diff --git a/fql_b200/csrc/step.cu b/fql_b200/csrc/step.cu
--- a/fql_b200/csrc/step.cu
+++ b/fql_b200/csrc/step.cu
@@ -393,6 +393,7 @@
   int use_euler_cluster = 1;
   int use_cluster_fwd = 1;
   int use_cluster_bwd = 1;
+  int use_cluster_critic = 1;
   unsigned long long* stamps = nullptr;
   int adam_done_blk = 0;
   int euler_hoist = 1;
@@ -495,6 +496,8 @@
   if (cbw && cbw[0] == '0') c->use_cluster_bwd = 0;
   const char* cfw = getenv("FQL_B200_CLUSTER_FWD");
   if (cfw && cfw[0] == '0') c->use_cluster_fwd = 0;
+  const char* ccr = getenv("FQL_B200_CLUSTER_CRITIC");
+  if (ccr && ccr[0] == '0') c->use_cluster_critic = 0;
   const char* stp = getenv("FQL_B200_STAMPS");
   if (stp && stp[0] == '1') {
     FQL_CHECK_CUDA(cudaMalloc(&c->stamps, 576 * sizeof(unsigned long long)));
@@ -644,6 +647,13 @@
   const int row_tiles = S * ((B + 127) / 128);
   const bool many_tiles = row_tiles >= ctx->chain_min_tiles && !wide;
   const bool big_bwd = many_tiles && ctx->use_big_bwd && tc_mlp_chain2_supported(d) && d->critic_layer_norm && d->reserved[0] == 0;
+  const bool split_opt = c.do_apply && c.do_backward && !dp_grads && !many_tiles && !pix;
+  const int blk_critic = (int)(L.net[FQL_NET_CRITIC].begin / FQL_LEAF_PAD), blk_onestep = (int)(L.net[FQL_NET_ACTOR_ONESTEP_FLOW].begin / FQL_LEAF_PAD);
+  const int blk_target = (int)(L.net[FQL_NET_TARGET_CRITIC].begin / FQL_LEAF_PAD);
+  auto adam_range = [&](int blk0, int blk1, cudaStream_t st) {
+    return launch_adam_polyak_stats(L, hp, S, c.st->params, c.st->mu, c.st->nu, c.st->grads, w.gstats + S * 4, w.partials, c.st->shadow,
+                                    tc_shadow_seed_elems(d, L), st, blk0, blk1);
+  };
   auto chain = [&](int net, const void* X0b, int rows_cap, int r0_in, int M, void* const* Hb, void* const* Zb, float* out, int n_steps,
                    cudaStream_t st) {
     TcChainSpec t;
@@ -738,6 +748,15 @@
     FQL_TRY(stamp(ctx, 4, S2));
   }
   (void)ev_f0;
+  if (split_opt) {
+    FQL_REQUIRE(L.net[FQL_NET_ACTOR_BC_FLOW].begin == 0 && L.net[FQL_NET_ACTOR_BC_FLOW].end == L.net[FQL_NET_CRITIC].begin &&
+                    L.net[FQL_NET_CRITIC].end == L.net[FQL_NET_ACTOR_ONESTEP_FLOW].begin,
+                "arena order: bc-flow | critic | one-step actor expected");
+    FQL_CHECK_CUDA(cudaStreamWaitEvent(ctx->s6, ctx->ev[16], 0));
+    FQL_CHECK_CUDA(cudaStreamWaitEvent(ctx->s6, ev_euler, 0));
+    FQL_TRY(adam_range(0, blk_critic, ctx->s6));
+    FQL_CHECK_CUDA(cudaEventRecord(ctx->ev[38], ctx->s6));
+  }
 
   FQL_TRY(tc_pad_bf16(w.XO, w.XOb, (int64_t)S * 3 * B, sh.F + sh.A, kO, S0));
   TcActor fo = actor(FQL_NET_ACTOR_ONESTEP_FLOW, w.XOb, kO, 3 * B, 0, 3 * B, w.O_Hb, w.O_Zb, true);
@@ -789,7 +808,10 @@
       if (cs[p] != S0) FQL_CHECK_CUDA(cudaStreamWaitEvent(cs[p], ctx->ev[40], 0));
       TcCritic f = cr;
       f.p = p; f.X0b = reinterpret_cast<const bf16*>(w.XCb) + (int64_t)p * S * B * kO;
-      FQL_TRY(tc_critic_forward(f, nets[p], w.C_out, cs[p]));
+      int rc = 1;
+      if (p == 2 && ctx->use_euler_cluster && ctx->use_cluster_critic && !wide) rc = tc_cluster_critic_forward(f, nets[p], w.C_out, row_tiles, cs[p]);
+      if (rc < 0) return -1;
+      if (rc == 1) FQL_TRY(tc_critic_forward(f, nets[p], w.C_out, cs[p]));
       if (cs[p] != S0) FQL_CHECK_CUDA(cudaEventRecord(ctx->ev[41 + p], cs[p]));
     }
     FQL_CHECK_CUDA(cudaStreamWaitEvent(ctx->s5, ctx->ev[41], 0));
@@ -855,6 +877,12 @@
       FQL_CHECK_CUDA(cudaEventRecord(ctx->ev[59], ctx->sc));
       ctx->adam_done_blk = blk1;
     }
+  }
+  if (split_opt) {
+    FQL_CHECK_CUDA(cudaEventRecord(ctx->ev[39], S0));
+    FQL_CHECK_CUDA(cudaStreamWaitEvent(S2, ctx->ev[39], 0));
+    FQL_TRY(adam_range(blk_critic, blk_onestep, S2));
+    FQL_CHECK_CUDA(cudaStreamWaitEvent(S2, ctx->ev[38], 0));
   }
   if (bc_enc_forked) FQL_CHECK_CUDA(cudaStreamWaitEvent(S2, ctx->ev[37], 0));
   FQL_CHECK_CUDA(cudaEventRecord(ev_s2, S2));
@@ -901,6 +929,10 @@
     FQL_CHECK_CUDA(cudaStreamWaitEvent(S0, ctx->ev[16], 0));
     FQL_TRY(stamp(ctx, 10, S0));
   }
+  if (split_opt) {
+    FQL_TRY(adam_range(blk_onestep, blk_target, S0));
+    ctx->adam_done_blk = blk_target;
+  }
   FQL_CHECK_CUDA(cudaStreamWaitEvent(S0, ev_s2, 0));
   if (dp_grads && !dp_bucketed) {
     const int64_t t0 = L.net[FQL_NET_TARGET_CRITIC].begin;
diff --git a/fql_b200/csrc/step.cuh b/fql_b200/csrc/step.cuh
--- a/fql_b200/csrc/step.cuh
+++ b/fql_b200/csrc/step.cuh
@@ -299,6 +299,7 @@
   void* t_start;
 };
 int tc_cluster_forward(const TcClusterFwdSpec& f, int other_clusters, cudaStream_t st);
+int tc_cluster_critic_forward(const TcCritic& t, int net, float* out, int other_clusters, cudaStream_t st);
 struct TcClusterBwdSpec {
   const FqlDims* d;
   const Layout* L;
diff --git a/fql_b200/csrc/tc_prims.cuh b/fql_b200/csrc/tc_prims.cuh
--- a/fql_b200/csrc/tc_prims.cuh
+++ b/fql_b200/csrc/tc_prims.cuh
@@ -68,6 +68,17 @@
       "add.u32 c, c, 1;\n\tsetp.lt.u32 P2, c, 0x4000000;\n\t@P2 bra WC_LOOP;\n\ttrap;\n"
       "WC_DONE:\n\t}\n" ::"r"(smem_u32(bar)), "r"(parity)
       : "memory");
+}
+
+__device__ __forceinline__ uint32_t mapa_shared(uint32_t saddr, uint32_t rank) {
+  uint32_t r;
+  asm volatile("mapa.shared::cluster.u32 %0, %1, %2;" : "=r"(r) : "r"(saddr), "r"(rank));
+  return r;
+}
+__device__ __forceinline__ void st_async_v2(uint32_t cluster_addr, float x, float y, uint32_t cluster_bar) {
+  asm volatile("st.async.shared::cluster.mbarrier::complete_tx::bytes.v2.f32 [%0], {%1, %2}, [%3];" ::"r"(cluster_addr), "f"(x), "f"(y),
+               "r"(cluster_bar)
+               : "memory");
 }
 
 __device__ __forceinline__ void tma_prefetch_desc(const CUtensorMap* m) {
diff --git a/include/fql_b200.h b/include/fql_b200.h
--- a/include/fql_b200.h
+++ b/include/fql_b200.h
@@ -170,6 +170,8 @@
                            int64_t z_rows_e, int64_t z_rows_s, void* stream);
 int fql_test_colsum_bf16(const void* X, int64_t G, int64_t M, int32_t N, float* out, int64_t out_stride_g0, int32_t G0,
                          int64_t out_stride_g1, void* stream);
+int fql_test_critic_cluster_forward(const FqlDims* d, const float* params, const void* shadow, const void* X0b, int32_t M, void* const* Hb,
+                                    float* const* Z, float* const* mu, float* const* rstd, float* out, void* stream);
 
 #ifdef __cplusplus
 }
```

Result: slower. 822,900, median of 6 (-28.1%).
